# a-rtemis99/hpc_suffix_array

Hardware: AMD Instinct MI355X
Metric: suffixes sorted/sec + ms/doubling-round, 1 GiB input at 1/2/4/8 MI355X (higher is better)
Workload: dtype u32

## Files before the change

### hpc_suffix_array_amd/_native.py

```python
from __future__ import annotations

import ctypes
import os
import subprocess

PKG_DIR = os.path.dirname(os.path.abspath(__file__))
LIB_PATH = os.path.join(PKG_DIR, "lib", "libsa_hip.so")
LIB_PATH = os.environ.get("SA_LIB_PATH", LIB_PATH)
CSRC = os.path.join(PKG_DIR, "csrc")

SA_MAX_ROUNDS = 64
KERNEL_KINDS = ["init", "hist_first", "hist_keys", "scan", "scatter_first", "scatter_keys",
                "heads", "heads_scan", "rerank", "seg_count", "seg_scan", "seg_write", "alphabet", "pack",
                "sort_u", "windows", "local_sort", "pivot_keys", "pivot_count", "pivot_write"]
SCHEDULE_PACKED = 0
SCHEDULE_REFERENCE = 1
ROUND1_AUTO = 0
ROUND1_LSD = 1
ROUND1_BUCKETED = 2
SA_K_COUNT = len(KERNEL_KINDS)
FIND_AUTO = 0
FIND_LANE = 1
FIND_WAVE = 2
FIND_LANE_MAX = 3584
FIND_MODES = {"auto": FIND_AUTO, "lane": FIND_LANE, "wave": FIND_WAVE}
BWT_STATS = 258
BWT_TILE = 4096
LOCATE_SA_ORDER = 1
LOCATE_SMALL_CHUNKS = 2
LOCATE_TILE = 2048
LOCATE_ORDERS = {"text": 0, "sa": LOCATE_SA_ORDER}
MEM_INFO = 3
MEM_TOO_MANY = 1
MEM_LANE = 1
MEM_WAVE = 2
MEM_MODES = {"auto": 0, "lane": MEM_LANE, "wave": MEM_WAVE}
LPF_NONE = 0xFFFFFFFF
LZ_TILE = 4096
REP_RIGHT = 0
REP_MAXIMAL = 1
REP_SUPERMAXIMAL = 2
REP_KINDS = {"right": REP_RIGHT, "maximal": REP_MAXIMAL, "supermaximal": REP_SUPERMAXIMAL}
REP_INFO = 2
IBWT_INFO = 3
LF_TILE = 32768
IBWT_S = 64
IBWT_TILE = 16384
FM_INFO = 4
FM_ROWS = (64, 256, 4096)
FM_MAX_SAMPLE = 4096
FM_HEADER = 4096
DOC_NONE = 0xFFFFFFFF
DOC_RANK_ORDER = 1
DOC_TILE = 2048
DOC_GROUP_MAX = 256
DOC_LDS_DOCS = 8192
DOC_ORDERS = {"doc": 0, "rank": DOC_RANK_ORDER}

DROPIN_SYMBOLS = ["create_suffix_array", "destroy_suffix_array", "build_suffix_array",
                  "build_lcp_array", "find_longest_repeated_substring", "is_valid_suffix_array"]
EXT_SYMBOLS = ["sa_context_create", "sa_context_destroy", "sa_context_set_debug", "sa_workspace_bytes", "sa_build_device",
               "sa_build_ex", "sa_check_device", "sa_check", "sa_lcp_device", "sa_lcp", "sa_generate_text_device",
               "sa_alphabet_device", "sa_pack_keys_device", "sa_sort_pairs_device", "sa_scatter_u64_device",
               "sa_gather_u64_device", "sa_running_max_i64_device", "sa_inclusive_sum_i64_device",
               "sa_count_below_u64_device", "sa_select_u8_device",
               "sa_find_device", "sa_find", "sa_find_ex",
               "sa_match_device", "sa_matching_stats_device", "sa_match", "sa_matching_stats",
               "sa_bwt_device", "sa_bwt", "sa_inverse_device", "sa_inverse",
               "sa_locate_device", "sa_locate",
               "sa_mems_device", "sa_mems",
               "sa_lpf_device", "sa_lpf", "sa_lz77_device", "sa_lz77",
               "sa_repeats_device", "sa_repeats",
               "sa_lf_device", "sa_ibwt_device", "sa_lf", "sa_ibwt", "sa_ibwt_ex",
               "sa_fm_index_bytes", "sa_fm_build_device", "sa_fm_count_device", "sa_fm_locate_device",
               "sa_fm_build", "sa_fm_count", "sa_fm_locate",
               "sa_doc_array_device", "sa_doc_of_device", "sa_doc_frequency_device", "sa_doc_list_device",
               "sa_doc_array", "sa_doc_of", "sa_doc_frequency", "sa_doc_list",
               "sa_dist_begin", "sa_dist_cuts", "sa_dist_plan_cuts", "sa_dist_reserve", "sa_dist_release", "sa_dist_round1", "sa_dist_req_count", "sa_dist_req_fill",
               "sa_dist_answer", "sa_dist_refine",
               "sa_last_error", "sa_host_syncs", "sa_device_count", "sa_version", "sa_struct_size"]


class SAError(RuntimeError):
    """A libsa_hip entry point returned an error code."""


DEBUG_FLAGS = {"no_cmp": 0x1, "no_pk8": 0x2, "no_pad": 0x4, "pad_overflow": 0x8, "no_fast32": 0x10,
               "no_pivot": 0x20, "perm_always": 0x40, "no_xq": 0x80, "xq_overflow": 0x100,
               "no_tied": 0x200, "no_key1_round": 0x400, "no_eonly": 0x800,
               "eonly": 0x1000, "fast32_small": 0x2000, "no_round2_fused": 0x4000,
               "ls_one_wg": 0x8000, "no_alpha_sample": 0x10000, "alpha_sample_small": 0x20000}


def debug_bits(names) -> int:
    bits = 0
    for x in names or ():
        if x not in DEBUG_FLAGS:
            raise ValueError(f"unknown debug flag {x!r} (one of {sorted(DEBUG_FLAGS)})")
        bits |= DEBUG_FLAGS[x]
    return bits


class SaOpts(ctypes.Structure):
    _fields_ = [("profile", ctypes.c_int32), ("schedule", ctypes.c_int32), ("init_chars", ctypes.c_int32),
                ("radix", ctypes.c_int32), ("round1", ctypes.c_int32), ("debug", ctypes.c_uint32),
                ("span_extra", ctypes.c_int32), ("tune", ctypes.c_int32)]


class SaStats(ctypes.Structure):
    _fields_ = [
        ("rounds", ctypes.c_int32),
        ("n_kinds", ctypes.c_int32),
        ("total_ms", ctypes.c_double),
        ("h2d_ms", ctypes.c_double),
        ("d2h_ms", ctypes.c_double),
        ("round_ms", ctypes.c_double * SA_MAX_ROUNDS),
        ("distinct", ctypes.c_uint64 * SA_MAX_ROUNDS),
        ("passes", ctypes.c_int32 * SA_MAX_ROUNDS),
        ("sorted_n", ctypes.c_uint64 * SA_MAX_ROUNDS),
        ("prefix_len", ctypes.c_uint64 * SA_MAX_ROUNDS),
        ("schedule", ctypes.c_int32),
        ("init_chars", ctypes.c_int32),
        ("sigma", ctypes.c_int32),
        ("sparse_ranks", ctypes.c_int32),
        ("round1", ctypes.c_int32),
        ("largest_window", ctypes.c_int32),
        ("model_bytes", ctypes.c_uint64),
        ("kern_ms", ctypes.c_double * SA_K_COUNT),
        ("kern_launches", ctypes.c_uint64 * SA_K_COUNT),
        ("kern_bytes", ctypes.c_uint64 * SA_K_COUNT),
        ("round1_segments", ctypes.c_int32),
        ("round1_layout", ctypes.c_int32),
        ("round_bytes", ctypes.c_uint64 * SA_MAX_ROUNDS),
        ("round1_windows", ctypes.c_int32 * 4),
        ("alphabet", ctypes.c_int32),
    ]

    def to_dict(self) -> dict:
        r = self.rounds
        return {
            "rounds": r,
            "total_ms": self.total_ms,
            "h2d_ms": self.h2d_ms,
            "d2h_ms": self.d2h_ms,
            "round_ms": list(self.round_ms[:r]),
            "distinct": [int(x) for x in self.distinct[:r]],
            "passes": list(self.passes[:r]),
            "sorted_n": [int(x) for x in self.sorted_n[:r]],
            "prefix_len": [int(x) for x in self.prefix_len[:r]],
            "schedule": "reference" if self.schedule == SCHEDULE_REFERENCE else "packed",
            "init_chars": self.init_chars,
            "sigma": self.sigma,
            "sparse_ranks": bool(self.sparse_ranks),
            "round1": {ROUND1_LSD: "lsd", ROUND1_BUCKETED: "bucketed", 3: "pivot"}.get(self.round1, "lsd"),
            "largest_window": self.largest_window,
            "round1_segments": {0: "exact", 1: "padded", 2: "padded-overflow", 3: "striped-records",
                                4: "striped-records-overflow"}.get(self.round1_segments, "exact"),
            "round1_layout": {"compact": bool(self.round1_layout & 1), "pk8": bool(self.round1_layout & 2),
                              "xq": bool(self.round1_layout & 4), "eonly": bool(self.round1_layout & 8)},
            "reference_model_bytes": int(self.model_bytes),
            "round_bytes": [int(x) for x in self.round_bytes[:r]],
            "round1_windows": [int(x) for x in self.round1_windows],
            "alphabet": {0: "exact", 1: "sampled", 2: "refuted"}.get(self.alphabet, "exact"),
            "kernels": {k: {"ms": self.kern_ms[i], "launches": int(self.kern_launches[i]),
                            "bytes": int(self.kern_bytes[i])} for i, k in enumerate(KERNEL_KINDS)},
        }


DIST_OK = 0
DIST_UNSUPPORTED = 1
DIST_UNBALANCED = 2


class SaDistInfo(ctypes.Structure):
    _fields_ = [("status", ctypes.c_int32), ("sigma", ctypes.c_int32), ("K", ctypes.c_int32),
                ("bucket_bits", ctypes.c_int32), ("m", ctypes.c_uint64), ("sa_off", ctypes.c_uint64),
                ("m_max", ctypes.c_uint64), ("bucket_lo", ctypes.c_uint32), ("bucket_hi", ctypes.c_uint32),
                ("round1_ok", ctypes.c_int32), ("reserved", ctypes.c_int32), ("heads", ctypes.c_uint64),
                ("unsorted", ctypes.c_uint64), ("groups", ctypes.c_uint64)]


class SuffixArrayStruct(ctypes.Structure):
    _fields_ = [("str", ctypes.c_void_p), ("n", ctypes.c_int),
                ("sa", ctypes.POINTER(ctypes.c_int)), ("lcp", ctypes.POINTER(ctypes.c_int))]


_lib = None


def source_hash() -> str:
    import glob
    import hashlib
    h = hashlib.sha256()
    files = sorted(glob.glob(os.path.join(CSRC, "sa_*")) + [os.path.join(CSRC, "Makefile")]
                   + glob.glob(os.path.join(PKG_DIR, "..", "include", "*.h")))
    for p in files:
        with open(p, "rb") as f:
            h.update(os.path.basename(p).encode() + b"\0" + f.read())
    return h.hexdigest()[:16]


def build_library(force: bool = False) -> str:
    if force or not os.path.exists(LIB_PATH):
        subprocess.run(["make", "-s", "-C", CSRC], check=True)
    return LIB_PATH


def lib() -> ctypes.CDLL:
    global _lib
    if _lib is not None:
        return _lib
    if not os.path.exists(LIB_PATH):
        raise SAError(f"{LIB_PATH} is missing: run `make -C {CSRC}` (or __graft_entry__.build())")
    L = ctypes.CDLL(LIB_PATH)
    vp, u64, i32 = ctypes.c_void_p, ctypes.c_uint64, ctypes.c_int
    L.sa_context_create.argtypes = [i32, u64, ctypes.POINTER(vp)]
    L.sa_context_create.restype = i32
    L.sa_context_destroy.argtypes = [vp]
    L.sa_context_destroy.restype = None
    L.sa_context_set_debug.argtypes = [vp, ctypes.POINTER(SaOpts)]
    L.sa_context_set_debug.restype = i32
    L.sa_workspace_bytes.argtypes = [u64]
    L.sa_workspace_bytes.restype = u64
    L.sa_build_device.argtypes = [vp, vp, u64, vp, vp, ctypes.POINTER(SaOpts), ctypes.POINTER(SaStats)]
    L.sa_build_device.restype = i32
    L.sa_build_ex.argtypes = [vp, u64, vp, i32, ctypes.POINTER(SaOpts), ctypes.POINTER(SaStats)]
    L.sa_build_ex.restype = i32
    L.sa_check_device.argtypes = [vp, vp, u64, vp, vp]
    L.sa_check_device.restype = i32
    L.sa_check.argtypes = [vp, u64, vp, i32]
    L.sa_check.restype = i32
    L.sa_lcp_device.argtypes = [vp, vp, u64, vp, vp, ctypes.POINTER(u64), ctypes.POINTER(u64), vp]
    L.sa_lcp_device.restype = i32
    L.sa_lcp.argtypes = [vp, u64, vp, i32, vp, ctypes.POINTER(u64), ctypes.POINTER(u64)]
    L.sa_lcp.restype = i32
    L.sa_alphabet_device.argtypes = [vp, u64, ctypes.POINTER(ctypes.c_uint32), vp]
    L.sa_alphabet_device.restype = i32
    L.sa_pack_keys_device.argtypes = [vp, vp, u64, u64, u64, ctypes.POINTER(ctypes.c_uint16), u64,
                                      ctypes.c_uint32, vp, vp]
    L.sa_pack_keys_device.restype = i32
    L.sa_sort_pairs_device.argtypes = [vp, vp, vp, u64, ctypes.c_uint32, vp, vp, vp]
    L.sa_sort_pairs_device.restype = i32
    L.sa_scatter_u64_device.argtypes = [vp, u64, vp, ctypes.c_int64, vp, u64, vp]
    L.sa_scatter_u64_device.restype = i32
    L.sa_gather_u64_device.argtypes = [vp, vp, u64, vp, ctypes.c_int64, u64, vp]
    L.sa_gather_u64_device.restype = i32
    L.sa_running_max_i64_device.argtypes = [vp, u64, vp]
    L.sa_running_max_i64_device.restype = i32
    L.sa_inclusive_sum_i64_device.argtypes = [vp, u64, vp]
    L.sa_inclusive_sum_i64_device.restype = i32
    L.sa_count_below_u64_device.argtypes = [vp, u64, vp, u64, i32, vp, vp]
    L.sa_count_below_u64_device.restype = i32
    L.sa_select_u8_device.argtypes = [vp, u64, vp, ctypes.POINTER(u64), vp]
    L.sa_select_u8_device.restype = i32
    L.sa_find_device.argtypes = [vp, u64, vp, vp, u64, vp, u64, vp, vp, ctypes.c_uint32, vp]
    L.sa_find_device.restype = i32
    L.sa_find.argtypes = [vp, u64, vp, i32, vp, vp, u64, vp, vp]
    L.sa_find.restype = i32
    L.sa_find_ex.argtypes = [vp, u64, vp, i32, vp, vp, u64, vp, vp, ctypes.c_uint32]
    L.sa_find_ex.restype = i32
    L.sa_match_device.argtypes = [vp, u64, vp, vp, u64, vp, u64, vp, vp, vp, ctypes.c_uint32, vp]
    L.sa_match_device.restype = i32
    L.sa_matching_stats_device.argtypes = [vp, u64, vp, vp, u64, u64, vp, vp, vp, ctypes.c_uint32, vp]
    L.sa_matching_stats_device.restype = i32
    L.sa_match.argtypes = [vp, u64, vp, i32, vp, vp, u64, vp, vp, vp, ctypes.c_uint32]
    L.sa_match.restype = i32
    L.sa_matching_stats.argtypes = [vp, u64, vp, i32, vp, u64, u64, vp, vp, vp, ctypes.c_uint32]
    L.sa_matching_stats.restype = i32
    L.sa_bwt_device.argtypes = [vp, u64, vp, vp, vp, vp]
    L.sa_bwt_device.restype = i32
    L.sa_bwt.argtypes = [vp, u64, vp, i32, vp, vp]
    L.sa_bwt.restype = i32
    L.sa_inverse_device.argtypes = [vp, u64, vp, vp, vp]
    L.sa_inverse_device.restype = i32
    L.sa_inverse.argtypes = [vp, u64, i32, vp]
    L.sa_inverse.restype = i32
    L.sa_locate_device.argtypes = [vp, u64, vp, vp, vp, u64, u64, ctypes.c_uint32, vp, vp, u64, ctypes.POINTER(u64), vp]
    L.sa_locate_device.restype = i32
    L.sa_locate.argtypes = [vp, u64, i32, vp, vp, u64, u64, ctypes.c_uint32, vp, vp, u64]
    L.sa_locate.restype = i32
    L.sa_mems_device.argtypes = [vp, vp, u64, vp, vp, u64, u64, u64, u64, ctypes.c_uint32, vp, vp, vp, u64,
                                 ctypes.POINTER(u64), vp]
    L.sa_mems_device.restype = i32
    L.sa_mems.argtypes = [vp, u64, vp, i32, vp, u64, u64, u64, u64, ctypes.c_uint32, vp, vp, vp, u64,
                          ctypes.POINTER(u64)]
    L.sa_mems.restype = i32
    L.sa_lpf_device.argtypes = [vp, vp, u64, vp, vp, vp, vp, vp]
    L.sa_lpf_device.restype = i32
    L.sa_lz77_device.argtypes = [vp, u64, vp, vp, vp, vp, vp, u64, ctypes.POINTER(u64), vp]
    L.sa_lz77_device.restype = i32
    L.sa_lpf.argtypes = [vp, u64, vp, i32, vp, vp]
    L.sa_lpf.restype = i32
    L.sa_lz77.argtypes = [vp, u64, vp, i32, vp, vp, vp, u64, ctypes.POINTER(u64)]
    L.sa_lz77.restype = i32
    L.sa_repeats_device.argtypes = [vp, vp, u64, vp, vp, u64, u64, ctypes.c_uint32, vp, vp, vp, u64,
                                    ctypes.POINTER(u64), vp]
    L.sa_repeats_device.restype = i32
    L.sa_repeats.argtypes = [vp, u64, vp, i32, u64, u64, ctypes.c_uint32, vp, vp, vp, u64, ctypes.POINTER(u64)]
    L.sa_repeats.restype = i32
    L.sa_lf_device.argtypes = [vp, vp, u64, u64, vp, vp]
    L.sa_lf_device.restype = i32
    L.sa_ibwt_device.argtypes = [vp, vp, u64, u64, vp, vp, ctypes.POINTER(u64), vp]
    L.sa_ibwt_device.restype = i32
    L.sa_lf.argtypes = [vp, u64, u64, vp, i32]
    L.sa_lf.restype = i32
    L.sa_ibwt.argtypes = [vp, u64, u64, vp, vp, i32]
    L.sa_ibwt.restype = i32
    L.sa_ibwt_ex.argtypes = [vp, u64, u64, vp, vp, i32, ctypes.POINTER(u64)]
    L.sa_ibwt_ex.restype = i32
    u32 = ctypes.c_uint32
    L.sa_fm_index_bytes.argtypes = [u64, u32]
    L.sa_fm_index_bytes.restype = u64
    L.sa_fm_build_device.argtypes = [vp, vp, u64, u64, vp, u32, vp, u64, ctypes.POINTER(u64), vp]
    L.sa_fm_build_device.restype = i32
    L.sa_fm_count_device.argtypes = [vp, u64, vp, u64, vp, u64, vp, vp, vp]
# ... 82 lines not shown
```

### hpc_suffix_array_amd/csrc/sa_bucket.h

```cpp
#pragma once
#include <type_traits>

#include "sa_kernels.h"

namespace sa {

#ifndef SA_BS_BLOCK
#define SA_BS_BLOCK 512
#endif
constexpr int kBsBlock = SA_BS_BLOCK;
#ifndef SA_BS_ITEMS
#define SA_BS_ITEMS 18
#endif
constexpr int kBsItems = SA_BS_ITEMS;
constexpr int kBsCap = kBsBlock * kBsItems;
constexpr uint32_t kWinStride = 1024;
#ifndef SA_BS_WPC
#define SA_BS_WPC 2
#endif
constexpr uint32_t kBsWpc = SA_BS_WPC;
#ifndef SA_BS_GRID
#define SA_BS_GRID (1u << 22)
#endif
constexpr uint32_t kBsGrid = SA_BS_GRID;
constexpr uint64_t kBucketMinN = 1ull << 20;
constexpr uint32_t kLoBits = 8;
constexpr uint32_t kLoRadix = 1u << kLoBits;

__device__ __forceinline__ uint32_t bucket_of(uint64_t key1, uint32_t rb, uint64_t cmul, uint32_t bsh) {
    return (uint32_t)(((key1 >> rb) * cmul) >> bsh);
}

__device__ __forceinline__ uint32_t bucket_dmin(uint32_t b, uint64_t cmul, uint32_t bsh) {
    const uint64_t d0 = ((uint64_t)b << bsh) / cmul;
    return (uint32_t)((((d0 * cmul) >> bsh) == b) ? d0 : d0 + 1);
}

struct SrcBucketKeys {
    const uint64_t* __restrict__ keys;
    const uint32_t* __restrict__ vals;
    uint32_t rb, bsh;
    uint64_t cmul;
    uint32_t bofs;
    __device__ __forceinline__ uint64_t key(uint64_t e) const { return keys[e]; }
    __device__ __forceinline__ uint32_t val(uint64_t e) const { return vals[e]; }
    static constexpr bool kPk8 = false;
    __device__ __forceinline__ uint32_t digit(uint64_t k, uint32_t shift, uint32_t mask) const {
        return ((bucket_of(k, rb, cmul, bsh) - bofs) >> shift) & mask;
    }
};

struct SrcPk8 {
    const uint64_t* __restrict__ items;
    __device__ __forceinline__ uint64_t key(uint64_t e) const { return items[e]; }
    __device__ __forceinline__ uint32_t val(uint64_t) const { return 0u; }
    static constexpr bool kPk8 = true;
};

template <int NB>
__device__ __forceinline__ void lds_bytes(const uint32_t* __restrict__ w32, uint32_t off, uint32_t (&out)[NB / 4]) {
    static_assert(NB % 4 == 0, "whole words");
    const uint32_t base = off >> 2, sh = off & 3u;
    uint32_t w[NB / 4 + 1];
#pragma unroll
    for (int q = 0; q <= NB / 4; ++q) w[q] = w32[base + q];
#pragma unroll
    for (int q = 0; q < NB / 4; ++q) out[q] = __builtin_amdgcn_alignbyte(w[q + 1], w[q], sh);
}
template <int NB>
__device__ __forceinline__ uint32_t byte_at(const uint32_t (&v)[NB / 4], int j) {
    return (v[j >> 2] >> (8 * (j & 3))) & 0xFFu;
}

constexpr uint32_t kCoarseBits = 12;
constexpr uint32_t kCoarse = 1u << kCoarseBits;

constexpr uint32_t kRecStripes = 64;
constexpr uint32_t kXq = 8;
constexpr uint32_t kRecCurStride = 64;
constexpr uint64_t rec_capacity(uint64_t m) { return m + m / 8 + kRecStripes * (2ull * kTile + 1); }
template <bool POW2 = false, bool COARSE = false, int LM = 0, bool IDENT = false, bool DNA = false>
__global__ __launch_bounds__(kBlock) void k_bucket_hist(const uint8_t* __restrict__ text, uint64_t n,
                                                        const uint16_t* __restrict__ code, BucketSpec b,
                                                        uint32_t* __restrict__ ghist, uint64_t p0, uint64_t p1,
                                                        uint32_t blo, uint32_t bhi,
                                                        uint64_t* __restrict__ lkeys = nullptr,
                                                        uint32_t* __restrict__ lpos = nullptr,
                                                        uint32_t* __restrict__ wg = nullptr, uint32_t rcap = 0,
                                                        uint32_t* __restrict__ rovf = nullptr) {
    constexpr bool REC = LM == 2 || LM == 3;
    constexpr int RUN = kTile / kBlock;
    constexpr uint32_t NB = COARSE ? kCoarse : kLoRadix;
    __shared__ uint32_t s_tmp[kWaves];
    __shared__ uint16_t s_rp[REC ? kTile : 1];
    __shared__ uint32_t s_claim;
    __shared__ uint8_t s_map[256];
    __shared__ __attribute__((aligned(16))) uint32_t s_dcw[(kTile + kMaxK) / 4 + 8];
    uint8_t* s_dc = reinterpret_cast<uint8_t*>(s_dcw);
    __shared__ uint32_t s_hlo[NB];
    constexpr bool PKD = DNA && REC;
    __shared__ uint32_t s_pk[PKD ? kBlock + kMaxK / 16 + 2 : 1];
    {
        const uint32_t cv = code[threadIdx.x];
        s_map[threadIdx.x] = (uint8_t)(cv ? cv - 1u : 0u);
    }
    for (uint32_t i = threadIdx.x; i < NB; i += kBlock) s_hlo[i] = 0;
    const uint32_t sig = b.sigma, ps1 = (uint32_t)b.pow_s1;
    const uint32_t shh = b.bsh;
    const uint32_t cshift = b.bb > kCoarseBits ? b.bb - kCoarseBits : 0u;
    const uint32_t bspan = bhi - blo;
    __syncthreads();
    const uint64_t tiles = (p1 - p0 + kTile - 1) / kTile;
    uint32_t kept_lane = 0;
    uint32_t run = LM == 2 ? wg[blockIdx.x] : 0u;
    const uint32_t stripe = blockIdx.x % kRecStripes;
    const uint64_t rbase = (uint64_t)stripe * rcap;
    auto fetch = [&](uint64_t tt2, uint4& v, uint32_t& hv) {
        const uint64_t tb2 = p0 + tt2 * kTile;
        const uint64_t i2 = tb2 + (uint64_t)threadIdx.x * RUN;
        v = (i2 + RUN <= n && (((uintptr_t)(text + i2)) & 15) == 0) ? *reinterpret_cast<const uint4*>(text + i2)
                                                                     : make_uint4(0u, 0u, 0u, 0u);
        const uint64_t h2 = tb2 + kTile + threadIdx.x;
        hv = (threadIdx.x < (uint32_t)kMaxK && h2 < n) ? (uint32_t)text[h2] : 0u;
    };
    uint4 cv = make_uint4(0u, 0u, 0u, 0u);
    uint32_t chv = 0;
    if (blockIdx.x < tiles) fetch(blockIdx.x, cv, chv);
    for (uint64_t tt = blockIdx.x; tt < tiles; tt += gridDim.x) {
        const uint64_t tb = p0 + tt * kTile;
        uint4 nv;
        uint32_t nhv;
        const uint64_t tn = tt + gridDim.x;
        if constexpr (LM != 3) fetch(tn < tiles ? tn : tiles - 1, nv, nhv);
        {
            const uint64_t i = tb + (uint64_t)threadIdx.x * RUN;
            uint32_t w[4];
            if (i + RUN <= n && (((uintptr_t)(text + i)) & 15) == 0) {
                const uint4 v = cv;
                w[0] = v.x;
                w[1] = v.y;
                w[2] = v.z;
                w[3] = v.w;
                if constexpr (DNA) {
#pragma unroll
                    for (int q = 0; q < 4; ++q) w[q] = ((w[q] >> 1) ^ (w[q] >> 2)) & 0x03030303u;
                } else if constexpr (!IDENT) {
#pragma unroll
                    for (int q = 0; q < 4; ++q) {
                        uint32_t o = 0;
#pragma unroll
                        for (int y = 0; y < 4; ++y) o |= (uint32_t)s_map[(w[q] >> (8 * y)) & 0xFFu] << (8 * y);
                        w[q] = o;
                    }
                }
            } else {
#pragma unroll
// ... 114 lines not shown
                    const uint64_t a = s_pk[wi], bw = s_pk[wi + 1], cw = s_pk[wi + 2];
                    uint64_t win = ((a << 32) | bw) << off;
                    if (off) win |= cw >> (32u - off);
                    Dk = (uint32_t)(win >> (64u - 2u * b.s));
                    r = (win >> (64u - 2u * K)) & ((1ull << (2u * b.R)) - 1ull);
                } else {
                    for (uint32_t q = 0; q < b.s; ++q) Dk = POW2 ? ((Dk << lg) | s_dc[l + q]) : Dk * sig + s_dc[l + q];
                    for (uint32_t q = b.s; q < K; ++q) r = POW2 ? ((r << lg) | s_dc[l + q]) : r * sig + s_dc[l + q];
                }
                lkeys[rb + t] = ((uint64_t)Dk << b.rb) | bucket_low(b, r, n - (tb + l));
                lpos[rb + t] = (uint32_t)(tb + l);
            }
            if (LM == 2) run += tot;
        }
        cv = nv;
        chv = nhv;
        __syncthreads();
    }
    if (LM == 1) {
        uint32_t tot;
        block_exclusive_sum(kept_lane, s_tmp, &tot);
        if (threadIdx.x == 0) wg[blockIdx.x] = tot;
    }
    for (uint32_t i = threadIdx.x; i < NB; i += kBlock) {
        if (!s_hlo[i]) continue;
        if constexpr (COARSE)
            atomicAdd(reinterpret_cast<unsigned long long*>(ghist) + i, (unsigned long long)s_hlo[i]);
        else
            atomicAdd(&ghist[i], s_hlo[i]);
    }
}

__global__ __launch_bounds__(kBlock) void k_exscan_u32(const uint32_t* __restrict__ in, uint32_t* __restrict__ out,
                                                       uint32_t cnt) {
    __shared__ uint32_t s_tmp[kWaves];
    uint32_t carry = 0;
    for (uint32_t base = 0; base < cnt; base += kBlock * 16) {
        uint32_t v[16], sum = 0;
#pragma unroll
        for (int k = 0; k < 16; ++k) {
            const uint32_t i = base + threadIdx.x * 16 + k;
            v[k] = i < cnt ? in[i] : 0u;
            sum += v[k];
        }
        uint32_t tot;
        uint32_t off = block_exclusive_sum(sum, s_tmp, &tot) + carry;
#pragma unroll
        for (int k = 0; k < 16; ++k) {
            const uint32_t i = base + threadIdx.x * 16 + k;
            if (i < cnt) out[i] = off;
            off += v[k];
        }
        carry += tot;
    }
}

__global__ __launch_bounds__(kBlock) void k_window_starts_tab(const uint32_t* __restrict__ bstart, uint32_t nb,
                                                              uint64_t n, uint64_t nw, uint32_t* __restrict__ ws,
                                                              uint32_t* __restrict__ wb) {
    for (uint64_t j = (uint64_t)blockIdx.x * kBlock + threadIdx.x; j <= nw; j += (uint64_t)gridDim.x * kBlock) {
        const uint64_t x = j * kWinStride;
        if (x >= n) {
            ws[j] = (uint32_t)n;
            wb[j] = nb;
            continue;
        }
        uint32_t lo = 0, len = nb + 1;
        while (len > 0) {
            const uint32_t half = len >> 1;
            if (bstart[lo + half] < x) {
                lo += half + 1;
                len -= half + 1;
            } else {
                len = half;
            }
        }
        ws[j] = bstart[lo];
        wb[j] = lo;
    }
}

__global__ __launch_bounds__(kBlock) void k_window_starts(const uint64_t* __restrict__ keys, uint64_t n,
                                                          uint64_t nw, uint32_t rb, uint64_t cmul, uint32_t bsh,
                                                          uint32_t* __restrict__ ws) {
    for (uint64_t j = (uint64_t)blockIdx.x * kBlock + threadIdx.x; j <= nw; j += (uint64_t)gridDim.x * kBlock) {
        const uint64_t x = j * kWinStride;
        uint64_t res;
        if (x >= n) {
            res = n;
        } else if (x == 0) {
            res = 0;
        } else {
            const uint32_t bx = bucket_of(keys[x - 1], rb, cmul, bsh);
            if (bucket_of(keys[x], rb, cmul, bsh) != bx) {
                res = x;
            } else {
                uint64_t lo = x, hi, step = 1;
                for (;;) {
                    hi = lo + step;
                    if (hi >= n) {
                        hi = n;
                        break;
                    }
                    if (bucket_of(keys[hi], rb, cmul, bsh) != bx) break;
                    lo = hi;
                    step *= 2;
                }
                while (hi - lo > 1) {
                    const uint64_t mid = lo + (hi - lo) / 2;
                    if (bucket_of(keys[mid], rb, cmul, bsh) != bx) hi = mid;
                    else lo = mid;
                }
                res = hi;
            }
        }
        ws[j] = (uint32_t)res;
    }
}

__global__ __launch_bounds__(kBlock) void k_window_list(const uint32_t* __restrict__ ws, uint64_t nw,
                                                        uint32_t* __restrict__ list, uint32_t* __restrict__ words) {
    __shared__ uint32_t s_n[kWaves], s_base;
    __shared__ uint32_t s_mx[kWaves];
    const uint32_t lane = lane_id(), wave = wave_id();
    const uint64_t per = ((nw + gridDim.x - 1) / gridDim.x + kBlock - 1) / kBlock * kBlock;
    const uint64_t j0 = (uint64_t)blockIdx.x * per, j1 = j0 + per < nw ? j0 + per : nw;
    uint32_t mx = 0, cnt = 0;
    for (uint64_t j = j0 + threadIdx.x; j < j1; j += kBlock) {
        const uint32_t d = ws[j + 1] - ws[j];
        mx = d > mx ? d : mx;
        cnt += d != 0;
    }
    uint32_t tot;
    uint32_t off = block_exclusive_sum(cnt, s_n, &tot);
    if (threadIdx.x == 0) s_base = tot ? atomicAdd(&words[7], tot) : 0u;
    __syncthreads();
    off += s_base;
    for (uint64_t j = j0 + threadIdx.x; j < j1; j += kBlock)
        if (ws[j + 1] != ws[j]) list[off++] = (uint32_t)j;
#pragma unroll
    for (int o = kWave / 2; o > 0; o >>= 1) {
        const uint32_t y = __shfl_xor(mx, o, kWave);
        mx = y > mx ? y : mx;
    }
    if (lane == 0) s_mx[wave] = mx;
    __syncthreads();
    if (threadIdx.x == 0) {
        uint32_t t = 0;
        for (int x = 0; x < kWaves; ++x) t = s_mx[x] > t ? s_mx[x] : t;
        if (t) atomicMax(&words[5], t);
    }
}

template <bool POW2>
__global__ __launch_bounds__(kBlock) void k_bucket_sample(const uint8_t* __restrict__ text, uint64_t n,
                                                          const uint16_t* __restrict__ code, BucketSpec b,
                                                          uint32_t ssh, uint32_t* __restrict__ ghist) {
    __shared__ uint8_t s_map[256];
    __shared__ uint32_t s_h[kLoRadix];
    {
        const uint32_t cv = code[threadIdx.x];
        s_map[threadIdx.x] = (uint8_t)(cv ? cv - 1u : 0u);
    }
    for (uint32_t i = threadIdx.x; i < kLoRadix; i += kBlock) s_h[i] = 0;
    __syncthreads();
    const uint32_t lg = POW2 ? (uint32_t)__builtin_ctz(b.sigma) : 0u;
    const uint32_t bksh = POW2 ? lg * b.s - b.bb : 0u;
    const uint64_t ns = n >> ssh;
    for (uint64_t i = (uint64_t)blockIdx.x * kBlock + threadIdx.x; i < ns; i += (uint64_t)gridDim.x * kBlock) {
        uint32_t hsh = (uint32_t)i * 0x9E3779B1u;
        hsh ^= hsh >> 15;
        hsh *= 0x85EBCA6Bu;
        hsh ^= hsh >> 13;
        const uint64_t p = (i << ssh) + (hsh >> (32 - ssh));
        uint32_t raw[32];
#pragma unroll
        for (uint32_t q = 0; q < 32; ++q)
            raw[q] = (q < b.s && p + q < n) ? (uint32_t)text[p + q] : 256u;
        uint32_t D = 0;
#pragma unroll
        for (uint32_t q = 0; q < 32; ++q) {
            if (q < b.s) {
                const uint32_t c = raw[q] < 256u ? (uint32_t)s_map[raw[q]] : 0u;
                D = POW2 ? ((D << lg) | c) : D * b.sigma + c;
            }
        }
        const uint32_t bk = POW2 ? (D >> bksh) : (uint32_t)(((uint64_t)D * b.cmul) >> b.bsh);
        atomicAdd(&s_h[bk & (kLoRadix - 1)], 1u);
    }
    __syncthreads();
    for (uint32_t i = threadIdx.x; i < kLoRadix; i += kBlock)
        if (s_h[i]) atomicAdd(&ghist[i], s_h[i]);
}

__global__ __launch_bounds__(kLoRadix) void k_pad_starts(const uint32_t* __restrict__ samples, uint32_t ssh,
                                                         uint32_t slack_off, uint32_t limit,
                                                         uint32_t* __restrict__ pstart) {
    __shared__ uint32_t s_tmp[kLoRadix / kWave];
    const uint32_t k = samples[threadIdx.x];
    const float bound = slack_off ? (float)k : (float)k + 4.0f * sqrtf((float)k) + 16.0f;
    uint64_t cap = (uint64_t)bound << ssh;
    cap = slack_off ? cap : cap + (cap >> 5);
    cap = (cap + 63) & ~63ull;
    const uint32_t c32 = (uint32_t)cap;
    const uint32_t inc = wave_inclusive_sum(c32);
    if (lane_id() == kWave - 1) s_tmp[wave_id()] = inc;
    __syncthreads();
    uint32_t off = 0;
    for (uint32_t w = 0; w < wave_id(); ++w) off += s_tmp[w];
    __syncthreads();
    if (threadIdx.x == kLoRadix - 1) s_tmp[0] = off + inc;
    __syncthreads();
    const bool fits = s_tmp[0] <= limit;
    pstart[threadIdx.x] = fits ? off + inc - c32 : 0u;
    if (threadIdx.x == kLoRadix - 1) pstart[kLoRadix] = fits ? off + inc : 0u;
}

#ifndef SA_SUB_BITS
#define SA_SUB_BITS 11
#endif
constexpr int kSubBits = SA_SUB_BITS;
constexpr int kSubBuckets = 1 << kSubBits;
constexpr uint32_t kMaxSub = 64;
constexpr int kRetryWord = 13;

struct BucketRel {
    const uint32_t* __restrict__ wb;
    const uint32_t* __restrict__ bstart;
    const uint32_t* __restrict__ bdmin;
    uint32_t rb;
    uint32_t bits1 = 0;
};

template <int BLOCK, int ITEMS>
__device__ __forceinline__ bool load_window(const uint64_t* __restrict__ w_in, const BucketRel& br, uint32_t j,
                                            uint64_t a, uint32_t m, uint32_t ib, uint64_t (&w)[ITEMS], uint64_t& mn,
                                            uint32_t& bits, uint64_t (*s_red)[BLOCK / kWave],
                                            uint32_t (*s_bk)[32], uint32_t* __restrict__ err, bool* fixed = nullptr) {
    if (fixed) *fixed = false;
    constexpr int WAVES = BLOCK / kWave;
    constexpr int WT = kWave * ITEMS;
    const uint32_t wave = wave_id(), lane = lane_id();
    const uint64_t imask = (ib >= 64) ? ~0ull : ((1ull << ib) - 1ull);
    const uint32_t b0 = br.wb[j], nbk = br.wb[j + 1] - b0;
    uint32_t dmin0 = 0;
    if (nbk == 1) {
        dmin0 = br.bdmin[b0];
    } else if (nbk <= 32) {
        if (threadIdx.x < nbk) {
            s_bk[0][threadIdx.x] = br.bstart[b0 + threadIdx.x];
            s_bk[1][threadIdx.x] = br.bdmin[b0 + threadIdx.x];
        }
        __syncthreads();
    }
    auto dmin_of = [&](uint64_t p) -> uint32_t {
        if (nbk == 1) return dmin0;
        if (nbk <= 32) {
            uint32_t lo = 0;
            for (uint32_t step = 16; step; step >>= 1)
                if (lo + step < nbk && s_bk[0][lo + step] <= p) lo += step;
            return s_bk[1][lo];
        }
        uint32_t lo = b0, len = nbk;
        while (len > 1) {
            const uint32_t half = len >> 1;
            if (br.bstart[lo + half] <= p) {
                lo += half;
                len -= half;
            } else {
                len = half;
            }
        }
        return br.bdmin[lo];
    };
    uint64_t mx = 0;
    mn = ~0ull;
    if (nbk == 1 && br.bits1) {
        const uint32_t l0 = wave * WT + lane;
#pragma unroll
        for (int i = 0; i < ITEMS; ++i) {
            const uint32_t le = l0 + i * kWave;
            w[i] = w_in[a + (le < m ? le : m - 1)];
        }
        bits = br.bits1;
        mn = (uint64_t)dmin0 << br.rb;
        if (fixed) *fixed = true;
        __syncthreads();
        return true;
    }
    if (nbk == 1) {
        const uint32_t l0 = wave * WT + lane;
#pragma unroll
        for (int i = 0; i < ITEMS; ++i) {
            const uint32_t le = l0 + i * kWave;
            const uint64_t x = w_in[a + (le < m ? le : m - 1)];
            w[i] = x;
            mn = x < mn ? x : mn;
            mx = x > mx ? x : mx;
        }
#pragma unroll
        for (int o = kWave / 2; o > 0; o >>= 1) {
            const uint64_t y0 = __shfl_xor(mn, o, kWave), y1 = __shfl_xor(mx, o, kWave);
            mn = y0 < mn ? y0 : mn;
            mx = y1 > mx ? y1 : mx;
        }
        if (lane == 0) {
// ... 122 lines not shown
        if (mh) last_h = (int32_t)(rb0 + 63 - __clzll(mh));
        nh += __popcll(mh);
        nu += __popcll(mu);
        ng += __popcll(muh);
    }
    if (lane == 0) {
        s_red[0][wave] = (uint64_t)(uint32_t)last_h | ((uint64_t)nh << 32);
        s_red[1][wave] = (uint64_t)nu | ((uint64_t)ng << 32);
    }
    __syncthreads();
    int32_t cw = -1;
    uint32_t bu = 0, bg = 0, th = 0, tu = 0, tg = 0;
#pragma unroll
    for (int x = 0; x < WAVES; ++x) {
        const uint64_t v0 = s_red[0][x], v1 = s_red[1][x];
        if (x < (int)wave) {
            if ((int32_t)(uint32_t)v0 >= 0) cw = (int32_t)(uint32_t)v0;
            bu += (uint32_t)v1;
            bg += (uint32_t)(v1 >> 32);
        }
        th += (uint32_t)(v0 >> 32);
        tu += (uint32_t)v1;
        tg += (uint32_t)(v1 >> 32);
    }
    if (threadIdx.x == 0) {
        so.cnt_u[j] = tu;
        so.cnt_g[j] = tg;
        tot_h += th;
        tot_u += tu;
        tot_g += tg;
    }
    const uint64_t imask = (ib >= 64) ? ~0ull : ((1ull << ib) - 1ull);
    const uint64_t lt = lanemask_lt(), lem = lt | (1ull << lane);
    while (urows) {
        const uint32_t i = (uint32_t)__builtin_ctz(urows);
        urows &= urows - 1;
        const uint32_t rb0 = wave * WT + i * kWave;
        uint64_t mh, mu, muh;
        masks(rb0, mh, mu, muh);
        const uint64_t pre = s_pre[wave * ITEMS + i];
        const int32_t ph = (int32_t)(uint32_t)pre;
        const int32_t ch = ph >= 0 ? ph : cw;
        if ((mu >> lane) & 1ull) {
            const uint64_t hl = mh & lem;
            const uint32_t hpos = hl ? rb0 + 63 - (uint32_t)__clzll(hl) : (uint32_t)ch;
            const uint32_t ku = bu + (uint32_t)((pre >> 32) & 0xFFFFu) + (uint32_t)__popcll(mu & lt);
            const uint32_t kg = bg + (uint32_t)(pre >> 48) + (uint32_t)__popcll(muh & lem) - 1u;
            const uint32_t x = (uint32_t)(s_w[rb0 + lane] & imask);
            const uint32_t rv = (uint32_t)(so.rank_off + a + hpos + 1u);
            if (so.tmp_rank) so.tmp_rank[a + ku] = rv;
            else so.rank[x] = rv;
            atomicOr(&so.member[x >> 5], 1u << (x & 31));
            so.tmp_pos[a + ku] = (uint32_t)(a + rb0 + lane);
            so.tmp_idx[a + ku] = x;
            so.tmp_g[a + ku] = kg;
        }
    }
}

__device__ __forceinline__ void flush_totals(uint32_t* __restrict__ words, uint64_t th, uint64_t tu, uint64_t tg) {
    if (threadIdx.x == 0) {
        if (th) atomicAdd(&words[0], (uint32_t)th);
        if (tu) atomicAdd(&words[1], (uint32_t)tu);
        if (tg) atomicAdd(&words[2], (uint32_t)tg);
    }
}

constexpr int kWsPer = 8;
constexpr int kWsBlock = kBlock * kWsPer;

__device__ __forceinline__ void wscan_load(const uint32_t* __restrict__ c, uint64_t nw, uint64_t b0, uint32_t (&x)[kWsPer],
                                           uint32_t& sum) {
    sum = 0;
#pragma unroll
    for (int k = 0; k < kWsPer; ++k) {
        const uint64_t i = b0 + threadIdx.x * kWsPer + k;
        x[k] = i <= nw ? c[i] : 0u;
        sum += x[k];
    }
}

__global__ __launch_bounds__(kBlock) void k_wscan_reduce(const uint32_t* __restrict__ cu, const uint32_t* __restrict__ cg,
                                                         uint64_t nw, uint32_t* __restrict__ part) {
    __shared__ uint32_t s_tmp[kWaves];
    const uint64_t b0 = (uint64_t)blockIdx.x * kWsBlock;
    uint32_t x[kWsPer], su, sg, tu, tg;
    wscan_load(cu, nw, b0, x, su);
    wscan_load(cg, nw, b0, x, sg);
    block_exclusive_sum(su, s_tmp, &tu);
    block_exclusive_sum(sg, s_tmp, &tg);
    if (threadIdx.x == 0) {
        part[2 * blockIdx.x] = tu;
        part[2 * blockIdx.x + 1] = tg;
    }
}

__global__ __launch_bounds__(kBlock) void k_wscan_top(uint32_t* __restrict__ part, uint32_t blocks) {
    __shared__ uint32_t s_tmp[kWaves];
    uint32_t carry_u = 0, carry_g = 0;
    for (uint32_t b0 = 0; b0 < blocks; b0 += kBlock) {
        const uint32_t b = b0 + threadIdx.x;
        const uint32_t u = b < blocks ? part[2 * b] : 0u, g = b < blocks ? part[2 * b + 1] : 0u;
        uint32_t tu, tg;
        const uint32_t eu = block_exclusive_sum(u, s_tmp, &tu) + carry_u;
        const uint32_t eg = block_exclusive_sum(g, s_tmp, &tg) + carry_g;
        if (b < blocks) {
            part[2 * b] = eu;
            part[2 * b + 1] = eg;
        }
        carry_u += tu;
        carry_g += tg;
    }
}

__global__ __launch_bounds__(kBlock) void k_wscan_apply(uint32_t* __restrict__ cu, uint32_t* __restrict__ cg, uint64_t nw,
                                                        const uint32_t* __restrict__ part) {
    __shared__ uint32_t s_tmp[kWaves];
    const uint64_t b0 = (uint64_t)blockIdx.x * kWsBlock;
    for (int a = 0; a < 2; ++a) {
        uint32_t* c = a ? cg : cu;
        uint32_t x[kWsPer], sum;
        wscan_load(c, nw, b0, x, sum);
        uint32_t off = block_exclusive_sum(sum, s_tmp, nullptr) + part[2 * blockIdx.x + a];
#pragma unroll
        for (int k = 0; k < kWsPer; ++k) {
            const uint64_t i = b0 + threadIdx.x * kWsPer + k;
            if (i <= nw) c[i] = off;
            off += x[k];
        }
    }
}

__global__ __launch_bounds__(kBlock) void k_u_gather(const uint32_t* __restrict__ list,
                                                     const uint32_t* __restrict__ words,
                                                     const uint32_t* __restrict__ ws, const uint32_t* __restrict__ ou,
                                                     const uint32_t* __restrict__ og, SegOut so,
                                                     uint32_t* __restrict__ u_pos, uint32_t* __restrict__ u_idx,
                                                     uint32_t* __restrict__ u_g, RankMap rm = RankMap{}) {
    const uint32_t nlist = words[7];
    const uint32_t lane = lane_id();
    for (uint64_t q = (uint64_t)blockIdx.x * kWaves + wave_id(); q < nlist; q += (uint64_t)gridDim.x * kWaves) {
        const uint32_t j = list[q];
        const uint32_t a = ws[j], o = ou[j], c = ou[j + 1] - o, g0 = og[j];
        for (uint32_t k = lane; k < c; k += kWave) {
            const uint32_t x = so.tmp_idx[a + k];
            u_pos[o + k] = so.tmp_pos[a + k];
            u_idx[o + k] = x;
            u_g[o + k] = so.tmp_g[a + k] + g0;
            if (so.tmp_rank) so.rank[rm.slot(x)] = so.tmp_rank[a + k];
        }
    }
}

constexpr int kR2Batch = 16;

__global__ __launch_bounds__(kBlock) void k_round2_windows(const uint32_t* __restrict__ list, const uint32_t* words,
                                                           const uint32_t* __restrict__ ws,
                                                           const uint32_t* __restrict__ cnt_u,
                                                           const uint32_t* __restrict__ tmp_pos,
                                                           const uint32_t* __restrict__ tmp_idx,
                                                           const uint32_t* __restrict__ tmp_g,
                                                           const uint8_t* __restrict__ text, uint64_t n,
                                                           const uint16_t* __restrict__ code, BucketSpec bs, uint64_t m,
                                                           uint32_t* __restrict__ sa, uint32_t* flag) {
    const uint32_t nlist = words[7];
    const uint32_t lane = lane_id();
    const uint32_t K = bs.s + bs.R;
    const CodeMap map{code};
    const uint64_t lt = lanemask_lt(), lem = lt | (1ull << lane);
    for (uint64_t q0 = ((uint64_t)blockIdx.x * kWaves + wave_id()) * kR2Batch; q0 < nlist;
         q0 += (uint64_t)gridDim.x * kWaves * kR2Batch) {
        if (__builtin_amdgcn_readfirstlane((int)__atomic_load_n(flag, __ATOMIC_RELAXED))) return;
        uint32_t a_l = 0, c_l = 0;
        if (lane < (uint32_t)kR2Batch && q0 + lane < nlist) {
            const uint32_t j = list[q0 + lane];
            c_l = cnt_u[j];
            a_l = ws[j];
        }
        if (__ballot(c_l > (uint32_t)kWave)) {
            if (lane == 0) atomicOr(flag, 1u);
            return;
        }
        const uint32_t e_l = wave_inclusive_sum(c_l);
        uint64_t todo = __ballot(c_l != 0);
        uint32_t base = 0;
        while (todo) {
            const uint64_t fit = todo & __ballot(e_l - base <= (uint32_t)kWave);
            todo &= ~fit;
            uint32_t a = 0, off = 0, nbase = base;
            bool act = false;
            for (uint64_t f = fit; f; f &= f - 1) {
                const int w = __builtin_ctzll(f);
                const uint32_t ew = (uint32_t)__shfl((int)e_l, w, kWave), cw = (uint32_t)__shfl((int)c_l, w, kWave);
                const uint32_t aw = (uint32_t)__shfl((int)a_l, w, kWave);
                const uint32_t s0 = ew - cw - base;
                if (lane >= s0 && lane < s0 + cw) {
                    a = aw;
                    off = lane - s0;
                    act = true;
                }
                nbase = ew;
            }
            base = nbase;
            bool bad = act && (uint64_t)a + off >= m;
            act = act && !bad;
            uint32_t pos = 0, x = 0, g = 0;
            if (act) {
                pos = tmp_pos[a + off];
                x = tmp_idx[a + off];
                g = tmp_g[a + off];
            }
            bad = bad || (act && x >= n);
            uint64_t key = 0;
            if (act && !bad && (uint64_t)x + K < n) {
                uint32_t D;
                key = key1_words<true>(text, n, map, bs, (uint64_t)x + K, &D) + 1u;
            }
            const uint64_t ma = __ballot(act);
            const uint32_t gp = (uint32_t)__shfl_up((int)g, 1, kWave);
            const bool head = act && (lane == 0 || off == 0 || g != gp || !((ma >> (lane - 1)) & 1ull));
            const uint64_t mh = __ballot(head);
            const uint64_t hl = mh & lem, ab = (mh | ~ma) & ~lem;
            const uint32_t start = hl ? 63u - (uint32_t)__clzll(hl) : lane;
            const uint32_t end = ab ? (uint32_t)__builtin_ctzll(ab) : (uint32_t)kWave;
            const uint32_t len = end - start;
            bad = bad || (act && len > (uint32_t)kUsLimit);
            uint32_t rank = 0;
#pragma unroll
            for (int t = 0; t < kUsLimit; ++t) {
                const uint32_t src = (start + t) & (kWave - 1);
                const uint64_t kk = __shfl(key, (int)src, kWave);
                if (act && (uint32_t)t < len && src != lane) {
                    rank += kk < key ? 1u : 0u;
                    bad = bad || kk == key;
                }
            }
            const uint64_t p = (uint64_t)(uint32_t)__shfl((int)pos, (int)start, kWave) + rank;
            bad = bad || (act && p >= m);
            if (__ballot(bad)) {
                if (lane == 0) atomicOr(flag, 1u);
                return;
            }
            if (act) sa[p] = x;
        }
    }
}

constexpr int kPcPer = 16;
constexpr int kPcBlock = kBlock * kPcPer;

__device__ __forceinline__ void popc_load(const uint32_t* __restrict__ bits, uint64_t nw, uint64_t b0,
                                          uint32_t (&c)[kPcPer]) {
    if (b0 + kPcPer <= nw) {
#pragma unroll
        for (int q = 0; q < kPcPer / 4; ++q) {
            const uint4 v = reinterpret_cast<const uint4*>(bits + b0)[q];
            c[4 * q] = (uint32_t)__popc(v.x);
            c[4 * q + 1] = (uint32_t)__popc(v.y);
            c[4 * q + 2] = (uint32_t)__popc(v.z);
            c[4 * q + 3] = (uint32_t)__popc(v.w);
        }
    } else {
#pragma unroll
        for (int k = 0; k < kPcPer; ++k) c[k] = b0 + k < nw ? (uint32_t)__popc(bits[b0 + k]) : 0u;
    }
}

__global__ __launch_bounds__(kBlock) void k_popc_reduce(const uint32_t* __restrict__ bits, uint64_t nw,
                                                        uint32_t* __restrict__ part) {
    __shared__ uint32_t s_tmp[kWaves];
    uint32_t c[kPcPer], sum = 0;
    popc_load(bits, nw, (uint64_t)blockIdx.x * kPcBlock + (uint64_t)threadIdx.x * kPcPer, c);
#pragma unroll
    for (int k = 0; k < kPcPer; ++k) sum += c[k];
    uint32_t tot;
    block_exclusive_sum(sum, s_tmp, &tot);
    if (threadIdx.x == 0) part[blockIdx.x] = tot;
}

constexpr int kPcTop = 1024;
__global__ __launch_bounds__(kPcTop) void k_popc_top(uint32_t* __restrict__ part, uint32_t blocks) {
    __shared__ uint32_t s_tmp[kPcTop / kWave];
    const uint32_t per = (blocks + kPcTop - 1) / kPcTop;
    const uint32_t b0 = threadIdx.x * per, b1 = b0 + per < blocks ? b0 + per : blocks;
    uint32_t sum = 0;
#pragma unroll 8
    for (uint32_t b = b0; b < b1; ++b) sum += part[b];
    const uint32_t inc = wave_inclusive_sum(sum);
    if (lane_id() == kWave - 1) s_tmp[wave_id()] = inc;
    __syncthreads();
    uint32_t run = inc - sum;
#pragma unroll
    for (int w = 0; w < kPcTop / kWave; ++w) run += w < (int)wave_id() ? s_tmp[w] : 0u;
#pragma unroll 8
    for (uint32_t b = b0; b < b1; ++b) {
        const uint32_t v = part[b];
        part[b] = run;
        run += v;
    }
}

__global__ __launch_bounds__(kBlock) void k_popc_apply(const uint32_t* __restrict__ bits, uint64_t nw,
                                                       const uint32_t* __restrict__ part,
                                                       uint32_t* __restrict__ prefix) {
    __shared__ uint32_t s_tmp[kWaves];
    const uint64_t b0 = (uint64_t)blockIdx.x * kPcBlock + (uint64_t)threadIdx.x * kPcPer;
    uint32_t c[kPcPer], sum = 0;
// ... 175 lines not shown
                cm = y > cm ? y : cm;
            }
            if (lane == kWave - 1) s_tmp[wave] = inc;
            if (lane == 0) s_red[0][wave] = cm;
            __syncthreads();
            uint32_t off = 0;
#pragma unroll
            for (int x = 0; x < WAVES; ++x) {
                off += (x < (int)wave) ? s_tmp[x] : 0u;
                big = (uint32_t)s_red[0][x] > big ? (uint32_t)s_red[0][x] : big;
            }
            uint32_t b = off + inc - sum;
#pragma unroll
            for (int x = 0; x < WPT; ++x) {
                const uint32_t b0 = b, b1 = b + c[2 * x];
                s_cnt[WPT * dg + x] = b0 | (b1 << 16);
                b = b1 + c[2 * x + 1];
            }
        }
        __syncthreads();
        probe.mark(2);
        if (big > kMaxSub) {
            if (threadIdx.x == 0) {
                if (fixed && retry) retry[atomicAdd(&words[kRetryWord], 1u)] = j;
                else skew[atomicAdd(&words[10], 1u)] = j;
            }
            __syncthreads();
            continue;
        }
#pragma unroll
        for (int i = 0; i < ITEMS; ++i) {
            if (wave * WT + i * kWave + lane < m) {
                const uint32_t sb = (uint32_t)(w[i] >> dsh) & (kSubBuckets - 1);
                const uint32_t old = atomicAdd(&s_cnt[sb >> 1], 1u << (16 * (sb & 1)));
                s_w[(old >> (16 * (sb & 1))) & 0xFFFFu] = w[i];
            }
        }
        __syncthreads();
        probe.mark(3);
        uint32_t nu = 0, ng = 0;
        uint32_t umask = 0;
        const uint32_t sb0 = 2 * WPT * dg;
        const uint32_t low_bits = bits > (uint32_t)kSubBits ? bits - kSubBits : bits;
        const uint32_t low_mask = low_bits >= 32 ? ~0u : ((1u << low_bits) - 1u);
        static_assert(2 * WPT == 4, "four sub-buckets per thread");
        uint32_t order = 0;
        {
            uint32_t o[4];
#pragma unroll
            for (int k = 0; k < 4; ++k) {
                const uint32_t sb = sb0 + k;
                o[k] = ((end_of(sb) - (sb ? end_of(sb - 1) : 0u)) << 2) | (uint32_t)k;
            }
            sort_net32<4>(o);
#pragma unroll
            for (int k = 0; k < 4; ++k) order |= (o[3 - k] & 3u) << (2 * k);
        }
#pragma unroll 1
        for (uint32_t i = 0; i < 4; ++i) {
            const uint32_t sb = sb0 + ((order >> (2 * i)) & 3u);
            const uint32_t lo = sb ? end_of(sb - 1) : 0u, hi = end_of(sb), cnt = hi - lo;
            const bool wide = __ballot(cnt > 8u) != 0ull;
            const bool wide4 = __ballot(cnt > 4u) != 0ull, wide12 = __ballot(cnt > 12u) != 0ull;
            if (cnt == 0) continue;
            const uint32_t nu0 = nu;
            if (!wide4 && low_bits <= 28) sort_sub<4>(s_w, lo, cnt, ib, low_mask, nu, ng);
            else if (!wide && low_bits <= 28) sort_sub<8>(s_w, lo, cnt, ib, low_mask, nu, ng);
            else if (!wide12 && low_bits <= 28) sort_sub<12>(s_w, lo, cnt, ib, low_mask, nu, ng);
            else
            if (cnt <= (uint32_t)kNet && low_bits <= 28) sort_sub<kNet>(s_w, lo, cnt, ib, low_mask, nu, ng);
            else sort_sub_lds(s_w, lo, hi, ib, nu, ng);
            if (nu != nu0) umask |= 1u << (sb - sb0);
        }
        probe.mark(4);
        uint32_t bu, bg, th_w, tu_w, tg_w;
        {
            const uint32_t iug = wave_inclusive_sum(nu | (ng << 16));
            uint32_t* const s_ug = s_tmp2;
            if (lane == kWave - 1) s_ug[wave] = iug;
            __syncthreads();
            uint32_t oug = 0, tug = 0;
#pragma unroll
            for (int x = 0; x < WAVES; ++x) {
                const uint32_t xug = s_ug[x];
                oug += (x < (int)wave) ? xug : 0u;
                tug += xug;
            }
            tu_w = tug & 0xFFFFu;
            tg_w = tug >> 16;
            th_w = m - tu_w + tg_w;
            bu = (oug & 0xFFFFu) + (iug & 0xFFFFu) - nu;
            bg = (oug >> 16) + (iug >> 16) - ng;
        }
        if (so.rank) {
            if (threadIdx.x == 0) {
                so.cnt_u[j] = tu_w;
                so.cnt_g[j] = tg_w;
                th += th_w;
                tu += tu_w;
                tg += tg_w;
            }
            if (umask) {
                const uint64_t imask = (ib >= 64) ? ~0ull : ((1ull << ib) - 1ull);
                uint32_t ku = bu, kg = bg;
                for (uint32_t um = umask; um; um &= um - 1u) {
                    const uint32_t sb = sb0 + (uint32_t)__builtin_ctz(um);
                    const uint32_t lo = sb ? end_of(sb - 1) : 0u, hi = end_of(sb);
                    uint32_t head = lo;
                    uint64_t pr = ~0ull;
                    for (uint32_t k = lo; k < hi; ++k) {
                        const uint64_t x = s_w[k], r = x >> ib;
                        const uint64_t nx = k + 1 < hi ? (s_w[k + 1] >> ib) : ~0ull;
                        const bool eqp = k > lo && pr == r, eqn = k + 1 < hi && nx == r;
                        if (!eqp) head = k;
                        if (!eqp && eqn) ++kg;
                        if (eqp || eqn) {
                            const uint32_t xi = (uint32_t)(x & imask);
                            const uint32_t rv = (uint32_t)(so.rank_off + a + head + 1u);
                            if (so.tmp_rank) so.tmp_rank[a + ku] = rv;
                            else so.rank[xi] = rv;
                            atomicOr(&so.member[xi >> 5], 1u << (xi & 31));
                            so.tmp_pos[a + ku] = (uint32_t)(a + k);
                            so.tmp_idx[a + ku] = xi;
                            so.tmp_g[a + ku] = kg - 1u;
                            ++ku;
                        }
                        pr = r;
                    }
                }
            }
        }
        probe.mark(5);
        store_window<BLOCK, ITEMS>(s_w, a, m, ib, mn, keys_out, sa_out, so.ksh);
        __syncthreads();
        probe.mark(6);
    }
    probe.flush(words);
    flush_totals(words, th, tu, tg);
}

template <int ITEMS>
__device__ __forceinline__ uint32_t slot0() {
    uint32_t t = threadIdx.x;
    asm volatile("" : "+v"(t));
    return (t / kWave) * (kWave * ITEMS) + (t & (kWave - 1));
}

constexpr uint32_t kSlotBits = kBsCap > (1 << 14) ? 15 : 14;
constexpr uint32_t kSlotMask = (1u << kSlotBits) - 1u;
constexpr uint32_t kLowMax = 32 - kSlotBits;
static_assert(kBsCap <= (1 << kSlotBits), "load slots in kSlotBits");
constexpr int kHdrWord = 14;
constexpr int kTicketWord = 15;

__global__ __launch_bounds__(kBlock) void k_window_split(const uint32_t* __restrict__ list,
                                                         const uint32_t* __restrict__ ws, BucketRel br,
                                                         uint32_t* __restrict__ words, uint4* __restrict__ hdr,
                                                         uint32_t* __restrict__ retry, uint32_t fast,
                                                         const uint32_t* __restrict__ pc = nullptr,
                                                         const uint32_t* __restrict__ pn = nullptr, uint32_t nb = 0,
                                                         uint32_t* __restrict__ hx = nullptr, uint32_t crows = 0) {
    const uint32_t nlist = words[7];
    const uint32_t lane = lane_id();
    for (uint64_t q0 = (uint64_t)blockIdx.x * kBlock; q0 < nlist; q0 += (uint64_t)gridDim.x * kBlock) {
        const uint64_t q = q0 + threadIdx.x;
        uint32_t j = 0, b0 = 0;
        bool one = false;
        const bool ok = q < nlist;
        if (ok) {
            j = list[q];
            b0 = br.wb[j];
            one = fast && br.wb[j + 1] - b0 == 1u;
            if (one && hx) {
                uint32_t nr = 0;
                for (uint32_t k = 0; k < kXq; ++k) {
                    const uint32_t c = pn[(uint64_t)k * nb + b0];
                    if (!crows && c && c < kWave) one = false;
                    nr += (c + kWave - 1) / kWave;
                }
                if (crows && nr > crows) one = false;
            }
        }
        const uint64_t m1 = __ballot(ok && one), m2 = __ballot(ok && !one);
        uint32_t base1 = 0, base2 = 0;
        if (lane == 0) {
            if (m1) base1 = atomicAdd(&words[kHdrWord], (uint32_t)__popcll(m1));
            if (m2) base2 = atomicAdd(&words[kRetryWord], (uint32_t)__popcll(m2));
        }
        base1 = (uint32_t)__shfl((int)base1, 0, kWave);
        base2 = (uint32_t)__shfl((int)base2, 0, kWave);
        if (ok && one) {
            const uint32_t a = ws[j];
            const uint32_t qi = base1 + (uint32_t)__popcll(m1 & lanemask_lt());
            hdr[qi] = make_uint4(j, a, ws[j + 1] - a, br.bdmin[b0]);
            if (hx) {
                uint32_t P = 0;
                for (uint32_t k = 0; k < kXq; ++k) {
                    const uint32_t c = pc[(uint64_t)k * nb + b0];
                    hx[(uint64_t)qi * 16 + k] = c - P;
                    if (k) hx[(uint64_t)qi * 16 + kXq - 1 + k] = P;
                    P += pn[(uint64_t)k * nb + b0];
                }
            }
        } else if (ok) {
            retry[base2 + (uint32_t)__popcll(m2 & lanemask_lt())] = j;
        }
    }
}

__global__ __launch_bounds__(kBlock) void k_window_gather(const uint32_t* __restrict__ list,
                                                          const uint32_t* __restrict__ words,
                                                          const uint32_t* __restrict__ ws,
                                                          const uint32_t* __restrict__ wb,
                                                          const uint32_t* __restrict__ pc,
                                                          const uint32_t* __restrict__ pn, uint32_t nb,
                                                          const uint64_t* __restrict__ in,
                                                          uint64_t* __restrict__ out) {
    const uint32_t nlist = words[kRetryWord];
    for (uint32_t qi = blockIdx.x; qi < nlist; qi += gridDim.x) {
        const uint32_t j = list[qi];
        uint64_t dst = ws[j];
        for (uint32_t b = wb[j]; b < wb[j + 1]; ++b) {
            for (uint32_t k = 0; k < kXq; ++k) {
                const uint32_t c = pn[(uint64_t)k * nb + b];
                const uint64_t src = pc[(uint64_t)k * nb + b];
                for (uint32_t t = threadIdx.x; t < c; t += kBlock) out[dst + t] = in[src + t];
                dst += c;
            }
        }
    }
}

template <int N, int LSV = 0>
__device__ __forceinline__ bool sort_sub_words(uint32_t* __restrict__ s_k, const uint32_t* __restrict__ s_x,
                                               uint32_t lo, uint32_t cnt, uint32_t& nu, uint32_t& ng) {
    uint32_t v[N];
#pragma unroll
    for (int t = 0; t < N; ++t) {
        if constexpr (LSV & 1) {
            const uint32_t x = s_k[lo + t];
            v[t] = (uint32_t)t < cnt ? x : ~0u;
        } else {
            v[t] = (uint32_t)t < cnt ? s_k[lo + t] : ~0u;
        }
    }
    sort_net32<N>(v);
    uint32_t eqm = 0;
#pragma unroll
    for (int t = 0; t + 1 < N; ++t) eqm |= ((v[t] ^ v[t + 1]) <= kSlotMask ? 1u : 0u) << t;
    eqm &= (1u << (cnt - 1)) - 1u;
    if constexpr (LSV & 2) {
        if (eqm == 0u) {
            uint32_t xi[N];
#pragma unroll
            for (int t = 0; t < N; ++t) xi[t] = s_x[min(v[t] & kSlotMask, (uint32_t)kBsCap - 1u)];
#pragma unroll
            for (int t = 0; t < N; ++t)
                if ((uint32_t)t < cnt) s_k[lo + t] = xi[t];
            return false;
        }
    }
#pragma unroll
    for (int t = 0; t < N; ++t)
        if ((uint32_t)t < cnt) s_k[lo + t] = v[t];
    nu += (uint32_t)__popc(eqm | (eqm << 1));
    ng += (uint32_t)__popc(eqm & ~(eqm << 1));
    return eqm != 0u;
}

__device__ __forceinline__ void sort_sub_words_lds(uint32_t* __restrict__ s_k, uint32_t lo, uint32_t hi, uint32_t& nu,
                                                   uint32_t& ng) {
    for (uint32_t k = lo + 1; k < hi; ++k) {
        const uint32_t x = s_k[k];
        uint32_t y = k;
        while (y > lo && s_k[y - 1] > x) {
            s_k[y] = s_k[y - 1];
            --y;
        }
        s_k[y] = x;
    }
    uint32_t pr = ~0u, cur = s_k[lo] >> kSlotBits;
    for (uint32_t k = lo; k < hi; ++k) {
        const uint32_t nx = k + 1 < hi ? (s_k[k + 1] >> kSlotBits) : ~0u;
        const bool eqp = k > lo && pr == cur, eqn = k + 1 < hi && nx == cur;
        nu += (eqp || eqn) ? 1u : 0u;
        ng += (!eqp && eqn) ? 1u : 0u;
        pr = cur;
        cur = nx;
    }
}

template <int ITEMS, int I0 = 0, int I1 = ITEMS>
__device__ __forceinline__ void load_items(const uint64_t* __restrict__ w_in, uint64_t a, uint32_t m,
                                           uint64_t (&x)[ITEMS]) {
    const uint32_t l0 = slot0<ITEMS>();
#pragma unroll
    for (int i = I0; i < I1; ++i) {
        const uint32_t le = l0 + i * kWave;
        x[i] = w_in[a + (le < m ? le : m - 1)];
    }
}

struct XqWin {
    const uint32_t* __restrict__ hx = nullptr;
    const uint32_t* __restrict__ rows = nullptr;
};

__device__ __forceinline__ uint32_t xq_offset(const uint32_t* __restrict__ hx, uint32_t le) {
    uint32_t off = hx[0];
#pragma unroll
    for (int k = 1; k < (int)kXq; ++k) off = hx[kXq - 1 + k] <= le ? hx[k] : off;
    return off;
}

template <int ITEMS, int I0 = 0, int I1 = ITEMS>
__device__ __forceinline__ void load_items_cr(const uint64_t* __restrict__ w_in, const uint32_t (&rv)[3],
                                              uint64_t (&x)[ITEMS]) {
    const uint32_t lane = lane_id();
#pragma unroll
    for (int i = I0; i < I1; ++i) {
        const uint32_t base = (uint32_t)__builtin_amdgcn_readlane((int)rv[0], i);
        x[i] = (w_in + base)[lane];
    }
}

template <int ITEMS, int ROWS>
__device__ __forceinline__ void load_rows_xq(const uint32_t* __restrict__ rows, uint32_t (&rv)[3]) {
    const uint32_t lane = lane_id();
    const uint32_t w = (uint32_t)__builtin_amdgcn_readfirstlane((int)(threadIdx.x / kWave));
    const uint32_t r = w * ITEMS + (lane < (uint32_t)ITEMS ? lane : 0u);
#pragma unroll
    for (int t = 0; t < 3; ++t) rv[t] = rows[t * ROWS + r];
}

template <int ITEMS, int I0 = 0, int I1 = ITEMS>
__device__ __forceinline__ void load_items_xq(const uint64_t* __restrict__ w_in, const uint32_t (&rv)[3], uint32_t m,
                                              uint64_t (&x)[ITEMS]) {
    const uint32_t l0 = slot0<ITEMS>();
    const uint32_t lane = lane_id();
    const uint32_t last = m - 1;
#pragma unroll
    for (int i = I0; i < I1; ++i) {
        const uint32_t le = l0 + i * kWave;
        const uint32_t lc = le < m ? le : last;
        const uint32_t da = (uint32_t)__builtin_amdgcn_readlane((int)rv[0], i);
        const uint32_t db = (uint32_t)__builtin_amdgcn_readlane((int)rv[1], i);
        const uint32_t sp = (uint32_t)__builtin_amdgcn_readlane((int)rv[2], i);
        x[i] = w_in[(uint32_t)((lane < sp ? da : db) + lc)];
    }
}

template <bool CR>
__global__ __launch_bounds__(kBlock) void k_window_rows(const uint32_t* __restrict__ words, const uint4* __restrict__ hdr,
                                                        const uint32_t* __restrict__ hx, uint32_t nrows,
                                                        uint32_t* __restrict__ rows) {
    const uint32_t nh = words[kHdrWord];
    const uint32_t lane = lane_id();
    for (uint64_t q = (uint64_t)blockIdx.x * kWaves + wave_id(); q < nh; q += (uint64_t)gridDim.x * kWaves) {
        const uint32_t m = hdr[q].z;
        uint32_t hv[16];
#pragma unroll
        for (int k = 0; k < 16; ++k) hv[k] = hx[q * 16 + k];
        if constexpr (CR) {
            uint32_t st[kXq], cn[kXq], nfull = 0;
#pragma unroll
            for (int k = 0; k < (int)kXq; ++k) {
                const uint32_t p0 = k ? hv[kXq - 1 + k] : 0u, p1 = k + 1 < (int)kXq ? hv[kXq + k] : m;
                st[k] = hv[k] + p0;
                cn[k] = p1 - p0;
                nfull += cn[k] / kWave;
            }
            for (uint32_t r = lane; r < nrows; r += kWave) {
                uint32_t base = st[0], cnt = 0, rf = 0, rp = nfull;
#pragma unroll
                for (int k = 0; k < (int)kXq; ++k) {
                    const uint32_t nf = cn[k] / kWave, rem = cn[k] % kWave;
                    if (r >= rf && r < rf + nf) {
                        base = st[k] + kWave * (r - rf);
                        cnt = kWave;
                    }
                    if (rem && r == rp) {
                        base = st[k] + kWave * nf;
                        cnt = rem;
                    }
                    rf += nf;
                    rp += rem ? 1u : 0u;
                }
                uint32_t* const e = rows + q * 3 * nrows + r;
                e[0] = base;
                e[nrows] = cnt;
            }
            continue;
        }
        for (uint32_t r = lane; r < nrows; r += kWave) {
            const uint32_t lo = std::min(r * kWave, m - 1), hi = std::min(r * kWave + (kWave - 1), m - 1);
            uint32_t split = kWave;
#pragma unroll
            for (int k = kXq - 1; k >= 1; --k) {
                const uint32_t pk = hv[kXq - 1 + k];
                if (pk > lo && pk <= hi) split = pk - r * kWave;
            }
            uint32_t* const e = rows + q * 3 * nrows + r;
            e[0] = xq_offset(hv, lo);
            e[nrows] = xq_offset(hv, hi);
            e[2 * nrows] = split;
        }
    }
}

#ifndef SA_LS_WFULL
#define SA_LS_WFULL 1
#endif
#ifndef SA_LS_CLAIMS
#define SA_LS_CLAIMS 1
#endif
#ifndef SA_LS_HRANK
#define SA_LS_HRANK 1
#endif
#ifndef SA_LS_HRANK_PF
#define SA_LS_HRANK_PF 3
#endif
#if SA_LS_HRANK_PF == 0
#define SA_LS_PF_TABLE {0, 0, 18, 18, 18}
#elif SA_LS_HRANK_PF == 1
#define SA_LS_PF_TABLE {18, 18, 18, 18, 18}
#elif SA_LS_HRANK_PF == 3
#define SA_LS_PF_TABLE {6, 6, 12, 18, 18}
#elif SA_LS_HRANK_PF == 5
#define SA_LS_PF_TABLE {0, 0, 6, 12, 18}
#elif SA_LS_HRANK_PF == 6
#define SA_LS_PF_TABLE {3, 6, 9, 15, 18}
#endif
constexpr int kLsPfHr[5] = SA_LS_PF_TABLE;
constexpr int kLsPfOld[5] = {0, 0, 18, 18, 18};
template <int P>
using pf_point = std::integral_constant<int, P>;
template <int BLOCK, int ITEMS, class Probe = NoProbe, bool XQ = false, int LSV = 0, bool CR = false>
__global__ __launch_bounds__(BLOCK, 4) void k_bucket_sort(const uint64_t* __restrict__ keys_in,
                                                       const uint4* __restrict__ hdr, uint32_t rb, uint32_t bits,
                                                       uint32_t ib, uint32_t* __restrict__ words,
                                                       uint64_t* __restrict__ keys_out, uint32_t* __restrict__ sa_out,
                                                       uint32_t* __restrict__ retry, SegOut so, XqWin xw = XqWin{}) {
    constexpr int WAVES = BLOCK / kWave;
    constexpr int CAP = BLOCK * ITEMS;
    static_assert(CAP <= (1 << kSlotBits), "load slots");
    __shared__ uint32_t s_lds[kSubBuckets / 2 + CAP + ((LSV & 1) ? kNet : 0) + CAP];
    uint32_t* const s_cnt = s_lds;
    uint32_t* const s_k = s_lds + kSubBuckets / 2;
    uint32_t* const s_x = s_k + CAP + ((LSV & 1) ? kNet : 0);
    __shared__ uint32_t s_tmp[WAVES];
    __shared__ uint32_t s_cm[WAVES];
    __shared__ uint32_t s_ug[WAVES];
    __shared__ uint32_t s_q[2];
    __shared__ unsigned long long s_tot[3];
    constexpr int WPT = kSubBuckets / 2 / BLOCK;
    static_assert(WPT * 2 == 4 && WPT * 2 * BLOCK == kSubBuckets, "four sub-buckets per thread");
    constexpr int ROWS = WAVES * ITEMS;

    const uint32_t wave = wave_id(), lane = lane_id();
    const uint32_t dg = threadIdx.x;
    const uint32_t nwin = words[kHdrWord];
    const uint32_t low_bits = bits - kSubBits;
    const uint32_t dsh = ib + low_bits;
    const uint32_t lmask = (1u << low_bits) - 1u;
    const uint64_t imask = (1ull << ib) - 1ull;
    auto end_of = [&](uint32_t sb) -> uint32_t { return ((s_cnt[sb >> 1] >> (16 * (sb & 1))) & 0xFFFFu) >> 2; };
    static_assert(4 * CAP < (1 << 16), "byte counts in 16-bit halves");
    auto cnt_word = [&](uint32_t y) -> uint32_t* {
        return reinterpret_cast<uint32_t*>(reinterpret_cast<char*>(s_cnt) + ((y << 1) & 0xFFCu));
    };
    auto half_inc = [](uint32_t y) -> uint32_t {
        uint32_t r;
        asm("v_lshlrev_b32_e64 %0, %1, 4" : "=v"(r) : "v"(y << 4));
        return r;
    };
    constexpr bool HR = SA_LS_HRANK != 0;
    typedef uint16_t __attribute__((may_alias)) half_t;
    Probe probe;
    if (threadIdx.x == 0) {
        s_q[0] = atomicAdd(&words[kTicketWord], 1u);
        if constexpr (HR) s_q[1] = atomicAdd(&words[kTicketWord], 1u);
        s_tot[0] = s_tot[1] = s_tot[2] = 0;
    }
    if constexpr (HR)
        for (int i = threadIdx.x; i < kSubBuckets / 2; i += BLOCK) s_cnt[i] = 0;
    __syncthreads();
    uint32_t q = (uint32_t)__builtin_amdgcn_readfirstlane((int)s_q[0]);
    if (q >= nwin) return;
    uint4 h = hdr[q];
    uint64_t w[ITEMS];
    uint32_t rv[3] = {0u, 0u, 0u};
    if constexpr (XQ) {
        load_rows_xq<ITEMS, ROWS>(xw.rows + (uint64_t)q * 3 * ROWS, rv);
        if constexpr (CR) load_items_cr<ITEMS>(keys_in, rv, w);
        else load_items_xq<ITEMS>(keys_in, rv, h.z, w);
    } else {
        load_items<ITEMS>(keys_in, h.y, h.z, w);
    }
    uint32_t qn = 0;
    bool more = false;
    uint4 hn = make_uint4(0u, 0u, 1u, 0u);
    uint32_t rwn[3] = {0u, 0u, 0u};
    auto next_window = [&](uint32_t ticket, uint32_t cur, uint32_t& qx, bool& mx, uint4& hx,
                           uint32_t (&rx)[3]) __attribute__((always_inline)) {
        qx = (uint32_t)__builtin_amdgcn_readfirstlane((int)ticket);
        mx = qx < nwin;
        hx = make_uint4(0u, 0u, 1u, 0u);
        if (mx) hx = hdr[qx];
        if constexpr (XQ) load_rows_xq<ITEMS, ROWS>(xw.rows + (uint64_t)(mx ? qx : cur) * 3 * ROWS, rx);
    };
    if constexpr (HR) next_window(s_q[1], q, qn, more, hn, rwn);
    uint32_t par = 0;
    for (;;) {
        probe.mark(-1);
        const uint32_t j = h.x, m = h.z;
        const uint64_t a = h.y;
        const uint64_t mn = (uint64_t)h.w << rb;
        if constexpr (!HR) {
            if (threadIdx.x == 0) s_q[par ^ 1u] = atomicAdd(&words[kTicketWord], 1u);
            for (int i = threadIdx.x; i < kSubBuckets / 2; i += BLOCK) s_cnt[i] = 0;
            __syncthreads();
            next_window(s_q[par ^ 1u], q, qn, more, hn, rwn);
        }
        probe.mark(0);
        const uint32_t l0 = slot0<ITEMS>();
        const bool wfull = SA_LS_WFULL && (wave + 1) * (uint32_t)(kWave * ITEMS) <= m;
        bool sfull = wfull;
        if constexpr (XQ && CR)
            sfull = SA_LS_WFULL && __ballot(lane < (uint32_t)ITEMS && rv[1] == kWave) == (1ull << ITEMS) - 1ull;
        auto slot_ok = [&](int i) -> bool {
            if constexpr (XQ && CR) return lane < (uint32_t)__builtin_amdgcn_readlane((int)rv[1], i);
            else return l0 + i * kWave < m;
        };
        static_assert(ITEMS == 18, "SA_LS_PF_TABLE");
        auto prefetch_at = [&](auto pc, auto rest) __attribute__((always_inline)) {
            constexpr int P = decltype(pc)::value;
            constexpr int A = P ? (HR ? kLsPfHr[P - 1] : kLsPfOld[P - 1]) : 0;
            constexpr int B = decltype(rest)::value ? ITEMS : (HR ? kLsPfHr[P] : kLsPfOld[P]);
            if constexpr (A < B) {
                __builtin_amdgcn_sched_barrier(0);
                if constexpr (XQ && CR) load_items_cr<ITEMS, A, B>(keys_in, rwn, w);
                else if constexpr (XQ) load_items_xq<ITEMS, A, B>(keys_in, rwn, hn.z, w);
                else load_items<ITEMS, A, B>(keys_in, hn.y, hn.z, w);
            }
        };
        constexpr std::false_type part{};
        constexpr std::true_type rest{};
        constexpr int RKW = (ITEMS + 3) / 4;
        uint32_t kk[HR ? ITEMS : 1], rk[HR ? RKW : 1];
        uint32_t tk = 0;
        static_assert(4 * kMaxSub <= 256, "byte ranks in 8 bits");
        if constexpr (HR) {
#pragma unroll
            for (int r = 0; r < RKW; ++r) rk[r] = 0;
            auto count1 = [&](int i, uint32_t le) {
                const uint32_t k = (uint32_t)(w[i] >> ib);
                const uint32_t y = k >> low_bits;
                const uint32_t old = atomicAdd(cnt_word(y), half_inc(y));
                s_x[le] = (uint32_t)(w[i] & imask);
                kk[i] = k;
                rk[i / 4] |= __builtin_amdgcn_ubfe(old, y << 4, 8u) << (8 * (i % 4));
            };
            if (sfull) {
#pragma unroll
                for (int i = 0; i < ITEMS; ++i) count1(i, l0 + i * kWave);
            } else {
#pragma unroll
                for (int i = 0; i < ITEMS; ++i) {
                    kk[i] = 0;
                    if (slot_ok(i)) count1(i, l0 + i * kWave);
                }
            }
            __builtin_amdgcn_sched_barrier(0);
            if (threadIdx.x == 0) tk = atomicAdd(&words[kTicketWord], 1u);
            prefetch_at(pf_point<0>{}, part);
        } else if (sfull) {
#pragma unroll
            for (int i = 0; i < ITEMS; ++i) {
                const uint32_t y = (uint32_t)(w[i] >> dsh);
                atomicAdd(cnt_word(y), half_inc(y));
            }
        } else {
#pragma unroll
            for (int i = 0; i < ITEMS; ++i) {
                if (slot_ok(i)) {
                    const uint32_t y = (uint32_t)(w[i] >> dsh);
                    atomicAdd(cnt_word(y), half_inc(y));
                }
            }
        }
        __syncthreads();
        probe.mark(1);
        uint32_t big = 0;
        uint32_t bw[2 * WPT + 1];
        {
            uint32_t c[2 * WPT], sum = 0, cm = 0;
#pragma unroll
            for (int x = 0; x < WPT; ++x) {
                const uint32_t pw = s_cnt[WPT * dg + x];
                c[2 * x] = pw & 0xFFFFu;
                c[2 * x + 1] = pw >> 16;
            }
#pragma unroll
            for (int x = 0; x < 2 * WPT; ++x) {
                sum += c[x];
                cm = c[x] > cm ? c[x] : cm;
            }
            const uint32_t inc = wave_inclusive_sum(sum);
#pragma unroll
            for (int o = kWave / 2; o > 0; o >>= 1) {
                const uint32_t y = __shfl_xor(cm, o, kWave);
                cm = y > cm ? y : cm;
            }
            if (lane == kWave - 1) s_tmp[wave] = inc;
            if (lane == 0) s_cm[wave] = cm;
            __syncthreads();
            uint32_t off = 0;
#pragma unroll
            for (int x = 0; x < WAVES; ++x) {
                off += (x < (int)wave) ? s_tmp[x] : 0u;
                big = s_cm[x] > big ? s_cm[x] : big;
            }
            uint32_t b = off + inc - sum;
#pragma unroll
            for (int x = 0; x < WPT; ++x) {
                const uint32_t b0 = b, b1 = b + c[2 * x];
                s_cnt[WPT * dg + x] = b0 | (b1 << 16);
                b = b1 + c[2 * x + 1];
                bw[2 * x] = b0 >> 2;
                bw[2 * x + 1] = b1 >> 2;
            }
            bw[2 * WPT] = b >> 2;
            if constexpr (HR)
                if (threadIdx.x == 0) s_q[0] = tk;
        }
        prefetch_at(pf_point<1>{}, part);
        __syncthreads();
        probe.mark(2);
        uint32_t qnn = 0;
        bool moren = false;
        uint4 hnn = make_uint4(0u, 0u, 1u, 0u);
        uint32_t rwnn[3] = {0u, 0u, 0u};
        if ((big >> 2) > kMaxSub) {
            if (threadIdx.x == 0) retry[atomicAdd(&words[kRetryWord], 1u)] = j;
            if constexpr (HR) {
#pragma unroll
                for (int x = 0; x < WPT; ++x) s_cnt[WPT * dg + x] = 0;
            }
            prefetch_at(pf_point<2>{}, rest);
            __syncthreads();
            if constexpr (HR) next_window(s_q[0], q, qnn, moren, hnn, rwnn);
        } else {
            auto place1 = [&](int i, uint32_t le) {
                const uint32_t k = kk[HR ? i : 0];
                const uint32_t st = reinterpret_cast<const half_t*>(s_cnt)[(k >> low_bits) & (uint32_t)(kSubBuckets - 1)];
                const uint32_t at = st + __builtin_amdgcn_ubfe(rk[HR ? i / 4 : 0], 8u * (i % 4), 8u);
                *reinterpret_cast<uint32_t*>(reinterpret_cast<char*>(s_k) + at) = ((k & lmask) << kSlotBits) | le;
            };
            auto scatter1 = [&](int i, uint32_t le) {
                const uint32_t y = (uint32_t)(w[i] >> dsh);
                const uint32_t old = atomicAdd(cnt_word(y), half_inc(y));
                const uint32_t at = __builtin_amdgcn_ubfe(old, y << 4, 16u);
                *reinterpret_cast<uint32_t*>(reinterpret_cast<char*>(s_k) + at) =
                    (((uint32_t)(w[i] >> ib) & lmask) << kSlotBits) | le;
                s_x[le] = (uint32_t)(w[i] & imask);
            };
            (void)place1;
            (void)scatter1;
            if constexpr (HR) {
                if (sfull) {
#pragma unroll
                    for (int i = 0; i < ITEMS; ++i) place1(i, l0 + i * kWave);
                } else {
#pragma unroll
                    for (int i = 0; i < ITEMS; ++i)
                        if (slot_ok(i)) place1(i, l0 + i * kWave);
                }
            } else if (sfull) {
#pragma unroll
                for (int g = 0; g < ITEMS; g += SA_LS_CLAIMS) {
                    uint32_t y[SA_LS_CLAIMS], old[SA_LS_CLAIMS];
#pragma unroll
                    for (int t = 0; t < SA_LS_CLAIMS; ++t) {
                        y[t] = (uint32_t)(w[g + t] >> dsh);
                        old[t] = atomicAdd(cnt_word(y[t]), half_inc(y[t]));
                    }
#pragma unroll
                    for (int t = 0; t < SA_LS_CLAIMS; ++t) {
                        const int i = g + t;
                        const uint32_t le = l0 + i * kWave;
                        const uint32_t at = __builtin_amdgcn_ubfe(old[t], y[t] << 4, 16u);
                        *reinterpret_cast<uint32_t*>(reinterpret_cast<char*>(s_k) + at) =
                            (((uint32_t)(w[i] >> ib) & lmask) << kSlotBits) | le;
                        s_x[le] = (uint32_t)(w[i] & imask);
// ... 19 lines not shown
                    lo = bw[3], hi = bw[4];
                    if (k == 0) lo = bw[0], hi = bw[1];
                    if (k == 1) lo = bw[1], hi = bw[2];
                    if (k == 2) lo = bw[2], hi = bw[3];
                } else {
                    const uint32_t sb = sb0 + k;
                    lo = sb ? end_of(sb - 1) : 0u;
                    hi = end_of(sb);
                }
            };
            uint32_t order = 0;
            {
                uint32_t o[4];
#pragma unroll
                for (int k = 0; k < 4; ++k) {
                    uint32_t lo, hi;
                    sub_range((uint32_t)k, lo, hi);
                    o[k] = ((hi - lo) << 2) | (uint32_t)k;
                }
                sort_net32<4>(o);
#pragma unroll
                for (int k = 0; k < 4; ++k) order |= (o[3 - k] & 3u) << (2 * k);
            }
#pragma unroll 1
            for (uint32_t i = 0; i < 4; ++i) {
                const uint32_t sb = sb0 + ((order >> (2 * i)) & 3u);
                uint32_t lo, hi;
                sub_range(sb - sb0, lo, hi);
                const uint32_t cnt = hi - lo;
                const bool wide4 = __ballot(cnt > 4u) != 0ull, wide8 = __ballot(cnt > 8u) != 0ull,
                           wide12 = __ballot(cnt > 12u) != 0ull;
                if (cnt == 0) continue;
                const uint32_t nu0 = nu;
                constexpr int LW = LSV & 1;
                bool grp;
                if ((LSV & 2) && !so.samples) {
                    if (!wide4) grp = sort_sub_words<4, LSV>(s_k, s_x, lo, cnt, nu, ng);
                    else if (!wide8) grp = sort_sub_words<8, LSV>(s_k, s_x, lo, cnt, nu, ng);
                    else if (!wide12) grp = sort_sub_words<12, LSV>(s_k, s_x, lo, cnt, nu, ng);
                    else if (cnt <= (uint32_t)kNet) grp = sort_sub_words<kNet, LSV>(s_k, s_x, lo, cnt, nu, ng);
                    else {
                        sort_sub_words_lds(s_k, lo, hi, nu, ng);
                        grp = true;
                    }
                } else {
                    if (!wide4) sort_sub_words<4, LW>(s_k, s_x, lo, cnt, nu, ng);
                    else if (!wide8) sort_sub_words<8, LW>(s_k, s_x, lo, cnt, nu, ng);
                    else if (!wide12) sort_sub_words<12, LW>(s_k, s_x, lo, cnt, nu, ng);
                    else if (cnt <= (uint32_t)kNet) sort_sub_words<kNet, LW>(s_k, s_x, lo, cnt, nu, ng);
                    else sort_sub_words_lds(s_k, lo, hi, nu, ng);
                    grp = nu != nu0;
                }
                if (grp) umask |= 1u << (sb - sb0);
                if (so.samples)
                    for_each_sample(a, lo, hi, so.ksh, [&](uint32_t q) {
                        keys_out[(a + q) >> so.ksh] = mn + (((uint64_t)sb << low_bits) | (s_k[q] >> kSlotBits));
                    });
            }
            prefetch_at(pf_point<3>{}, part);
            probe.mark(4);
            uint32_t bu, bg, tu_w, tg_w;
            {
                const uint32_t iug = wave_inclusive_sum(nu | (ng << 16));
                if (lane == kWave - 1) s_ug[wave] = iug;
                __syncthreads();
                uint32_t oug = 0, tug = 0;
#pragma unroll
                for (int x = 0; x < WAVES; ++x) {
                    const uint32_t xug = s_ug[x];
                    oug += (x < (int)wave) ? xug : 0u;
                    tug += xug;
                }
                tu_w = tug & 0xFFFFu;
                tg_w = tug >> 16;
                bu = (oug & 0xFFFFu) + (iug & 0xFFFFu) - nu;
                bg = (oug >> 16) + (iug >> 16) - ng;
            }
            if constexpr (HR) {
#pragma unroll
                for (int x = 0; x < WPT; ++x) s_cnt[WPT * dg + x] = 0;
            }
            const bool idx_back = (LSV & 2) && !so.samples;
            if (so.rank && threadIdx.x == 0) {
                so.cnt_u[j] = tu_w;
                so.cnt_g[j] = tg_w;
                s_tot[0] += m - tu_w + tg_w;
                s_tot[1] += tu_w;
                s_tot[2] += tg_w;
            }
            if (umask && (so.rank || idx_back)) {
                uint32_t ku = bu, kg = bg;
                for (uint32_t um = umask; um; um &= um - 1u) {
                    uint32_t lo, hi;
                    sub_range((uint32_t)__builtin_ctz(um), lo, hi);
                    uint32_t head = lo, pr = ~0u;
                    for (uint32_t k = lo; k < hi; ++k) {
                        const uint32_t v = s_k[k], r = v >> kSlotBits;
                        const uint32_t nx = k + 1 < hi ? (s_k[k + 1] >> kSlotBits) : ~0u;
                        const bool eqp = k > lo && pr == r, eqn = k + 1 < hi && nx == r;
                        const uint32_t xi = s_x[v & kSlotMask];
                        if (idx_back) s_k[k] = xi;
                        if (!eqp) head = k;
                        if (!eqp && eqn) ++kg;
                        if (so.rank && (eqp || eqn)) {
                            const uint32_t rv = (uint32_t)(so.rank_off + a + head + 1u);
                            if (so.tmp_rank) so.tmp_rank[a + ku] = rv;
                            else so.rank[xi] = rv;
                            atomicOr(&so.member[xi >> 5], 1u << (xi & 31));
                            so.tmp_pos[a + ku] = (uint32_t)(a + k);
                            so.tmp_idx[a + ku] = xi;
                            so.tmp_g[a + ku] = kg - 1u;
                            ++ku;
                        }
                        pr = r;
                    }
                }
            }
            prefetch_at(pf_point<4>{}, part);
            probe.mark(5);
            if (idx_back) {
                __syncthreads();
                if (wfull) {
#pragma unroll 2
                    for (int i = 0; i < ITEMS; ++i) {
                        const uint32_t le = l0 + i * kWave;
                        sa_out[a + le] = s_k[le];
                    }
                } else {
#pragma unroll 2
                    for (int i = 0; i < ITEMS; ++i) {
                        const uint32_t le = l0 + i * kWave;
                        if (le < m) sa_out[a + le] = s_k[le];
                    }
                }
            } else if (wfull) {
#pragma unroll 2
                for (int i = 0; i < ITEMS; ++i) {
                    const uint32_t le = l0 + i * kWave;
                    sa_out[a + le] = s_x[s_k[le] & kSlotMask];
                }
            } else {
#pragma unroll 2
                for (int i = 0; i < ITEMS; ++i) {
                    const uint32_t le = l0 + i * kWave;
                    if (le < m) sa_out[a + le] = s_x[s_k[le] & kSlotMask];
                }
            }
            __syncthreads();
            probe.mark(6);
        }
        if (!more) break;
        q = qn;
        h = hn;
        if constexpr (XQ && CR) {
            rv[0] = rwn[0];
            rv[1] = rwn[1];
        }
        if constexpr (HR) {
            qn = qnn;
            more = moren;
            hn = hnn;
#pragma unroll
            for (int t = 0; t < 3; ++t) rwn[t] = rwnn[t];
        }
        par ^= 1u;
    }
    probe.flush(words);
    __syncthreads();
    flush_totals(words, s_tot[0], s_tot[1], s_tot[2]);
}

template <int BLOCK, int ITEMS>
__global__ __launch_bounds__(BLOCK) void k_bucket_sort_lsd(const uint64_t* __restrict__ keys_in, BucketRel br,
                                                           const uint32_t* __restrict__ ws,
                                                           const uint32_t* __restrict__ skew,
                                                           uint32_t* __restrict__ words, uint32_t ib,
                                                           uint64_t* __restrict__ keys_out,
                                                           uint32_t* __restrict__ sa_out, SegOut so) {
    constexpr int WAVES = BLOCK / kWave;
    constexpr int CAP = BLOCK * ITEMS;
    constexpr int WT = kWave * ITEMS;
    static_assert(BLOCK >= kRadix, "one thread per digit");
    static_assert(CAP <= 65535, "16-bit LDS offsets");
    __shared__ uint64_t s_w[CAP];
    __shared__ uint16_t s_wcnt[WAVES][kRadix];
    __shared__ uint16_t s_start[kRadix];
    __shared__ uint32_t s_tmp[kWaves];
    __shared__ uint64_t s_red[2][WAVES];
    __shared__ uint32_t s_bk[2][32];

    const uint32_t wave = wave_id(), lane = lane_id();
    const uint32_t dg = threadIdx.x;
    uint32_t* err = words + 6;
    const uint32_t nskew = words[10];
    static_assert(WAVES * ITEMS * 8 <= WAVES * kRadix * 2, "per-row segment values fit in s_wcnt");
    uint64_t th = 0, tu = 0, tg = 0;
    for (uint32_t q = blockIdx.x; q < nskew; q += gridDim.x) {
        const uint32_t j = skew[q];
        const uint64_t a = ws[j];
        const uint32_t m = (uint32_t)(ws[j + 1] - a);
        uint64_t w[ITEMS];
        uint64_t mn;
        uint32_t bits;
        if (!load_window<BLOCK, ITEMS>(keys_in, br, j, a, m, ib, w, mn, bits, s_red, s_bk, err)) {
            __syncthreads();
            continue;
        }
        const uint32_t passes = (bits + 7) / 8;
        for (uint32_t p = 0; p < passes; ++p) {
            const uint32_t sh = ib + 8 * p;
            for (int i = threadIdx.x; i < WAVES * kRadix; i += BLOCK) (&s_wcnt[0][0])[i] = 0;
            __syncthreads();
            uint32_t r[ITEMS];
            uint16_t* wc = s_wcnt[wave];
#pragma unroll
            for (int i = 0; i < ITEMS; ++i) {
                const uint32_t le = wave * WT + i * kWave + lane;
                const bool ok = le < m;
                const uint32_t d = ok ? (uint32_t)(w[i] >> sh) & 0xFFu : (uint32_t)kRadix;
                uint64_t peers = __ballot(ok);
#pragma unroll
                for (uint32_t bt = 0; bt < 8; ++bt) {
                    const bool bit = (d >> bt) & 1u;
                    const uint64_t bal = __ballot(bit);
                    peers &= bit ? bal : ~bal;
                }
                uint32_t cnt = 0;
                if (ok) cnt = wc[d];
                const uint32_t below = (uint32_t)__popcll(peers & lanemask_lt());
                r[i] = cnt + below;
                if (ok && below == 0) wc[d] = (uint16_t)(cnt + (uint32_t)__popcll(peers));
            }
            __syncthreads();
            uint32_t tot = 0;
            if (dg < (uint32_t)kRadix) {
#pragma unroll
                for (int x = 0; x < WAVES; ++x) {
                    const uint32_t y = s_wcnt[x][dg];
                    s_wcnt[x][dg] = (uint16_t)tot;
                    tot += y;
                }
            }
            {
                const uint32_t x = (dg < (uint32_t)kRadix) ? tot : 0u;
                const uint32_t inc = wave_inclusive_sum(x);
                if (lane == kWave - 1 && wave < (uint32_t)kWaves) s_tmp[wave] = inc;
                __syncthreads();
                uint32_t off = 0;
#pragma unroll
                for (int x2 = 0; x2 < kWaves; ++x2) off += (x2 < (int)wave) ? s_tmp[x2] : 0u;
                if (dg < (uint32_t)kRadix) s_start[dg] = (uint16_t)(off + inc - x);
            }
            __syncthreads();
#pragma unroll
            for (int i = 0; i < ITEMS; ++i) {
                if (wave * WT + i * kWave + lane < m) {
                    const uint32_t d = (uint32_t)(w[i] >> sh) & 0xFFu;
                    s_w[s_start[d] + s_wcnt[wave][d] + r[i]] = w[i];
                }
            }
            __syncthreads();
#pragma unroll
            for (int i = 0; i < ITEMS; ++i) {
                const uint32_t le = wave * WT + i * kWave + lane;
                if (le < m) w[i] = s_w[le];
            }
            __syncthreads();
        }
        if (passes == 0) {
#pragma unroll
            for (int i = 0; i < ITEMS; ++i) {
                const uint32_t le = wave * WT + i * kWave + lane;
                if (le < m) s_w[le] = w[i];
            }
            __syncthreads();
        }
        if (so.rank)
            window_segments<BLOCK, ITEMS>(s_w, reinterpret_cast<uint64_t*>(&s_wcnt[0][0]), s_red, a, m, ib, j, so, th,
                                          tu, tg);
        store_window<BLOCK, ITEMS>(s_w, a, m, ib, mn, keys_out, sa_out, so.ksh);
        __syncthreads();
    }
    flush_totals(words, th, tu, tg);
}

}
```

### hpc_suffix_array_amd/csrc/sa_build.hip

```cpp
#include <hip/hip_runtime.h>

#include <algorithm>
#include <atomic>
#include <chrono>
#include <cstdarg>
#include <cstdio>
#include <cstdlib>
#include <cstring>
#include <mutex>
#include <string>
#include <thread>
#include <vector>

#include "../../include/sa_hip.h"

#ifndef SA_ALPHA_GRID
#define SA_ALPHA_GRID 2048
#endif

#include "sa_bucket.h"
#include "sa_check.h"
#include "sa_kernels.h"
#include "sa_lcp.h"
#include "sa_limits.h"
#include "sa_onesweep.h"
#include "sa_permute.h"
#include "sa_pivot.h"
#include "sa_split.h"
#include "sa_lsd.h"

namespace sa {

static thread_local std::string g_err;

static int set_err(int code, const char* fmt, ...) {
    char buf[512];
    va_list ap;
    va_start(ap, fmt);
    vsnprintf(buf, sizeof buf, fmt, ap);
    va_end(ap);
    g_err = buf;
    return code;
}

#define SA_HIP(call)                                                                         \
    do {                                                                                     \
        hipError_t e_ = (call);                                                              \
        if (e_ != hipSuccess)                                                                \
            return set_err(SA_E_HIP, "%s failed: %s (%s:%d)", #call, hipGetErrorString(e_),  \
                           __FILE__, __LINE__);                                              \
    } while (0)

static std::atomic<uint64_t> g_host_syncs{0};
static hipError_t host_sync(hipStream_t s) {
    g_host_syncs.fetch_add(1, std::memory_order_relaxed);
    return hipStreamSynchronize(s);
}
static hipError_t host_sync_event(hipEvent_t e) {
    g_host_syncs.fetch_add(1, std::memory_order_relaxed);
    return hipEventSynchronize(e);
}
static hipError_t host_memcpy(void* dst, const void* src, size_t bytes, hipMemcpyKind kind) {
    g_host_syncs.fetch_add(1, std::memory_order_relaxed);
    return hipMemcpy(dst, src, bytes, kind);
}

#define SA_TRY(...)                      \
    do {                                 \
        const int rc_ = (__VA_ARGS__);   \
        if (rc_) return rc_;             \
    } while (0)

static bool trace_on() {
    static const bool on = std::getenv("SA_TRACE") != nullptr;
    return on;
}
#define SA_TRACE(...)                                   \
    do {                                                \
        if (trace_on()) {                               \
            std::fprintf(stderr, "[sa] " __VA_ARGS__);  \
            std::fputc('\n', stderr);                   \
        }                                               \
    } while (0)

#ifndef SA_MAX_CHUNKS
#define SA_MAX_CHUNKS 4096
#endif
constexpr uint32_t kMaxChunks = SA_MAX_CHUNKS;
static_assert(kMaxChunks >= 1 && kMaxChunks <= (1u << 20), "chunk scratch sized for at most 2^20 chunks");
constexpr uint64_t kSparseDiv = 8;
constexpr int kEvPool = 256;
constexpr int kRoundEv = SA_MAX_ROUNDS + 1;
constexpr int kSyncEv = kEvPool + kRoundEv;

static uint64_t align_up(uint64_t x, uint64_t a) { return (x + a - 1) / a * a; }

static uint32_t bit_width(uint64_t x) {
    uint32_t w = 0;
    while (x) { ++w; x >>= 1; }
    return w;
}

static Chunking plan_chunks(uint64_t n) {
    Chunking ch;
    ch.n = n;
    const uint64_t tiles = (n + kTile - 1) / kTile;
    uint64_t tpc = (tiles + kMaxChunks - 1) / kMaxChunks;
    if (tpc == 0) tpc = 1;
    ch.tiles_per_chunk = (uint32_t)tpc;
    ch.chunks = (uint32_t)std::max<uint64_t>(1, (tiles + tpc - 1) / tpc);
    return ch;
}

}

namespace sa { struct DistState; }

struct sa_context {
    int device = 0;
    uint64_t cap = 0;
    uint64_t cap_pad = 0;
    uint64_t ucap = 0;
    uint32_t* rank = nullptr;
    uint64_t* keys[2] = {nullptr, nullptr};
    uint32_t* vals_alt = nullptr;
    uint32_t* vals_u = nullptr;
    uint32_t* u_pos[2] = {nullptr, nullptr};
    uint32_t* u_idx[2] = {nullptr, nullptr};
    uint32_t* u_g[2] = {nullptr, nullptr};
    uint32_t* u_gs[2] = {nullptr, nullptr};
    uint64_t gscap = 0;
    uint64_t* keys_u = nullptr;
    uint64_t kucap = 0;
    uint32_t* segx = nullptr;
    uint64_t segx_words = 0;
    uint32_t* os = nullptr;
    uint32_t* lsd = nullptr;
    uint32_t* lsdx = nullptr;
    uint32_t* segw = nullptr;
    uint64_t* states = nullptr;
    uint32_t epoch = 0;
    uint64_t radix_passes = 0;
    int radix = 0;
    int cus = 256;
    uint32_t* member = nullptr;
    uint32_t* hist = nullptr;
    uint32_t* totals = nullptr;
    uint32_t* counts = nullptr;
    uint32_t* words = nullptr;
    uint32_t* alpha = nullptr;
    uint16_t* code = nullptr;
    uint32_t* host_words = nullptr;
    hipEvent_t ev[sa::kEvPool + sa::kRoundEv + 1];
    int ev_ready = 0;
    sa::DistState* dist = nullptr;
    uint32_t dbg = 0;
    int32_t span_extra = 0;
    int32_t tune = 0;
    bool dna = false;
    bool alpha_prove = false;
    bool alpha_refuted = false;
    bool samples_pending = false;
};

namespace sa {

static uint64_t pad_capacity(uint64_t n) { return n + n / 8 + (1ull << 22); }

static uint64_t pad_elems(uint64_t n) {
    const uint64_t m = align_up(std::max<uint64_t>(n, 1), 64);
    return (n >= (1ull << 26) && n <= (1ull << 31)) ? align_up(pad_capacity(n), 64) : m;
}

constexpr uint64_t kMaxRadix = 1024;
static uint64_t tile_states_bytes(uint64_t n) { return ((n + kTile - 1) / kTile + 1) * kMaxRadix * 8; }

static uint64_t ws_bytes(uint64_t n) {
    const uint64_t m = align_up(std::max<uint64_t>(n, 1), 64);
    const uint64_t ku_slack = n >= (1ull << 26) ? n / 16 + 8ull * 1024 * kXqSlack + 64 : 0;
    const uint64_t gs = 2 * (n / 2 + 64) * 4;
    const uint64_t segx = (xq_words(1024) + 1032 + 2ull * kXq * (1ull << 19)) * 4;
    return m * 4 + 2 * m * 8 + m * 4 + (pad_elems(n) - m) * 12 + 7 * m * 4 + (m + ku_slack) * 8 + m / 8 + gs +
           segx + tile_states_bytes(n) + (uint64_t)kRadix * kMaxChunks * 4 + 8192;
}

static void free_ctx_buffers(sa_context* c) {
    hipFree(c->rank);
    hipFree(c->keys[0]);
    hipFree(c->keys[1]);
    hipFree(c->vals_alt);
    hipFree(c->states);
    c->rank = nullptr;
    c->keys[0] = c->keys[1] = nullptr;
    c->vals_alt = nullptr;
    c->states = nullptr;
    c->cap = 0;
    c->cap_pad = 0;
}

static void free_u_buffers(sa_context* c) {
    hipFree(c->vals_u);
    hipFree(c->keys_u);
    hipFree(c->member);
    c->vals_u = nullptr;
    c->keys_u = nullptr;
    c->member = nullptr;
    for (int i = 0; i < 2; ++i) {
        hipFree(c->u_pos[i]);
        hipFree(c->u_idx[i]);
        hipFree(c->u_g[i]);
        hipFree(c->u_gs[i]);
        c->u_pos[i] = c->u_idx[i] = c->u_g[i] = c->u_gs[i] = nullptr;
    }
    c->gscap = 0;
    c->ucap = 0;
    c->kucap = 0;
}

static void set_debug(sa_context* c, const sa_opts* o) {
    c->dbg = o ? o->debug : 0u;
    c->span_extra = o ? o->span_extra : 0;
    c->tune = o ? o->tune : 0;
}

static int ensure_capacity(sa_context* c, uint64_t n) {
    if (n <= c->cap && c->rank) return SA_OK;
    SA_HIP(hipSetDevice(c->device));
    free_ctx_buffers(c);
    const uint64_t m = align_up(std::max<uint64_t>(n, 1), 64);
    const uint64_t mp = pad_elems(n);
    if (hipMalloc(&c->rank, m * 4) != hipSuccess || hipMalloc(&c->keys[0], mp * 8) != hipSuccess ||
        hipMalloc(&c->keys[1], m * 8) != hipSuccess || hipMalloc(&c->vals_alt, mp * 4) != hipSuccess ||
        hipMalloc(&c->states, tile_states_bytes(n)) != hipSuccess ||
        hipMemset(c->states, 0, tile_states_bytes(n)) != hipSuccess) {
        free_ctx_buffers(c);
        (void)hipGetLastError();
        return set_err(SA_E_NOMEM, "device allocation of %.2f GiB workspace failed",
                       (double)ws_bytes(n) / (1ull << 30));
    }
    c->cap = n;
    c->cap_pad = mp;
    SA_TRACE("workspace: rank %p keys0 %p keys1 %p vals_alt %p", (void*)c->rank, (void*)c->keys[0], (void*)c->keys[1],
             (void*)c->vals_alt);
    return SA_OK;
}

static int ensure_u_capacity(sa_context* c, uint64_t n) {
    if (n <= c->ucap && c->vals_u) return SA_OK;
    SA_HIP(hipSetDevice(c->device));
    free_u_buffers(c);
    const uint64_t m = align_up(std::max<uint64_t>(n, 1), 64) * 4;
    const uint64_t ku = align_up(std::max<uint64_t>(n, 1), 64) +
                        (n >= (1ull << 26) ? n / 16 + 8ull * 1024 * kXqSlack + 64 : 0);
    bool ok = hipMalloc(&c->vals_u, m) == hipSuccess && hipMalloc(&c->keys_u, 8 * ku) == hipSuccess &&
              hipMalloc(&c->member, align_up(n, 1024) / 8) == hipSuccess;
    for (int i = 0; i < 2 && ok; ++i)
        ok = hipMalloc(&c->u_pos[i], m) == hipSuccess && hipMalloc(&c->u_idx[i], m) == hipSuccess &&
             hipMalloc(&c->u_g[i], m) == hipSuccess;
    if (!ok) {
        free_u_buffers(c);
        (void)hipGetLastError();
        return set_err(SA_E_NOMEM, "device allocation of the unsorted-set buffers failed");
    }
    c->ucap = n;
    c->kucap = ku;
    SA_TRACE("unsorted-set buffers: vals_u %p keys_u %p", (void*)c->vals_u, (void*)c->keys_u);
    return SA_OK;
}

static int ensure_gs(sa_context* c, uint64_t n) {
    if (n <= c->gscap && c->u_gs[0]) return SA_OK;
    for (int i = 0; i < 2; ++i) {
        hipFree(c->u_gs[i]);
        c->u_gs[i] = nullptr;
    }
    c->gscap = 0;
    const uint64_t w = n / 2 + 64;
    for (int i = 0; i < 2; ++i)
        if (hipMalloc(&c->u_gs[i], w * 4) != hipSuccess) {
            (void)hipGetLastError();
            for (int k = 0; k < 2; ++k) {
                hipFree(c->u_gs[k]);
                c->u_gs[k] = nullptr;
            }
            return set_err(SA_E_NOMEM, "group-start buffers (%llu words)", (unsigned long long)w);
        }
    c->gscap = n;
    return SA_OK;
}

static bool gs_available(sa_context* c, uint64_t n) {
    if (ensure_gs(c, n) == SA_OK) return true;
    (void)hipGetLastError();
    g_err.clear();
    SA_TRACE("group-start buffers unavailable: pivot rounds without tied blocks");
    return false;
}

static uint32_t* gs_buf(const sa_context* c, uint64_t n, int i) { return n <= c->gscap ? c->u_gs[i] : nullptr; }

struct Timer {
    sa_context* c;
    hipStream_t s;
    bool on;
    sa_stats* st;
    int used = 0;
    int kind[kEvPool / 2];
    void begin(int k) {
        if (!on) return;
        if (used >= kEvPool / 2) flush();
        kind[used] = k;
        hipEventRecord(c->ev[2 * used], s);
    }
    void end() {
// ... 820 lines not shown
        Gt = c->host_words[21];
        Dt = c->host_words[22];
        if (T > t1 || Gt > G || Dt > G)
            return set_err(SA_E_INTERNAL, "tied blocks %llu / %llu / %llu out of range", (unsigned long long)T,
                           (unsigned long long)Gt, (unsigned long long)Dt);
    }
    uint32_t Pr = 0;
    uint64_t Dr = 0, mrr = 0, Gr = 0;
    if (mr > 0) {
        const uint32_t bits = bit_width(2 * G - 1) + wr;
        const uint32_t Pn = (bits + 7) / 8;
        uint32_t* const va = tied ? ridx + ra : c->u_g[uo];
        uint32_t* const vb = tied ? ridx + 2 * ra : c->u_idx[uo];
        uint32_t* vfinal = (Pn & 1u) ? va : vb;
        uint32_t* vother = (Pn & 1u) ? vb : va;
        uint64_t* rs = nullptr;
        int rc = radix_sort(c, SrcKeys{kbA, ridx}, 12 * mr, plan_chunks(mr), bits, vfinal, vother, ukb1, kbA, s, tm,
                            st, &rs, &Pr, false, true);
        if (rc) return rc;
        tm.begin(SA_K_SORT_U);
        const dim3 pg((uint32_t)std::min<uint64_t>((mr + kBlock - 1) / kBlock, 8192));
        if (tied)
            hipLaunchKernelGGL(k_pivot_place<true>, pg, dim3(kBlock), 0, s, (const uint64_t*)rs,
                               (const uint32_t*)vfinal, mr, (const uint32_t*)gs, (const uint32_t*)gP, Gu, wr, nullptr,
                               nullptr, m, (const uint32_t*)c->u_pos[ui], c->vals_u);
        else
            hipLaunchKernelGGL(k_pivot_place<false>, pg, dim3(kBlock), 0, s, (const uint64_t*)rs,
                               (const uint32_t*)vfinal, mr, (const uint32_t*)gs, (const uint32_t*)gP, Gu, wr, ukb0,
                               c->vals_u, m, nullptr, nullptr);
        tm.end();
        SA_HIP(hipGetLastError());
        add_bytes(st, SA_K_SORT_U, tied ? 20 * mr : 24 * mr);
        if (tied) {
            rc = segments(c, rs, vfinal, plan_chunks(mr), PosArray{c->vals_u}, false, nullptr, d_sa, uo, s, tm, st,
                          &Dr, &mrr, &Gr, nullptr, 0, RankMap{}, T, (uint32_t)Gt, c->u_gs[uo]);
            if (rc) return rc;
        }
    }
    *P = 1 + Pr;
    if (tied) {
        *gs_written = true;
        *segs_done = true;
        *Du = Dr + Dt;
        *m2 = mrr + T;
        *G2 = Gr + Gt;
    }
    *sorted = ukb0;
    return SA_OK;
}

static int pivot_round1(sa_context* c, uint64_t n, uint32_t bits1, uint32_t* d_sa, hipStream_t s, Timer& tm,
                        sa_stats* st, bool* done, uint64_t* D, uint64_t* m, uint64_t* G, uint32_t* P) {
    *done = false;
    const Chunking ch = plan_chunks(n);
    const uint64_t* keys = c->keys[1];
    uint32_t* const gs = c->u_pos[1];
    uint32_t* const toff = gs + 2;
    uint32_t* const tid = gs + 4;
    uint32_t* const gP = c->vals_alt;
    uint32_t* const cc = c->hist;
    c->host_words[24] = 0;
    c->host_words[25] = (uint32_t)n;
    SA_HIP(hipMemcpyAsync(gs, c->host_words + 24, 8, hipMemcpyHostToDevice, s));
    tm.begin(SA_K_PIVOT_COUNT);
    hipLaunchKernelGGL((k_pivot_pass<0, true>), dim3(ch.chunks), dim3(kBlock), 0, s, keys, nullptr, nullptr, ch,
                       (const uint32_t*)gs, nullptr, 1u, 0u, cc, gP, nullptr, nullptr, nullptr, nullptr, TiedOut{});
    hipLaunchKernelGGL(k_scan_rows, dim3(3), dim3(kBlock), 0, s, cc, ch.chunks, c->totals);
    tm.end();
    SA_HIP(hipGetLastError());
    add_bytes(st, SA_K_PIVOT_COUNT, 8 * n);
    SA_HIP(hipMemcpyAsync(c->host_words + 16, c->totals, 12, hipMemcpyDeviceToHost, s));
    SA_HIP(host_sync(s));
    const uint64_t t0 = c->host_words[16], t1 = c->host_words[17], t2 = c->host_words[18];
    if (t0 + t1 + t2 != n) return set_err(SA_E_INTERNAL, "round-1 pivot classes %llu + %llu + %llu != %llu",
                                          (unsigned long long)t0, (unsigned long long)t1, (unsigned long long)t2,
                                          (unsigned long long)n);
    SA_TRACE("  round 1: pivot split, tied %llu of %llu", (unsigned long long)t1, (unsigned long long)n);
    if (t1 * 2 < n) return SA_OK;
    const uint64_t mr = t0 + t2;
    uint64_t* const rk = c->keys[0];
    uint32_t* const ridx = c->u_idx[1];
    if (!gs_available(c, n)) return SA_OK;
    tm.begin(SA_K_PIVOT_WRITE);
    hipLaunchKernelGGL(k_pivot_gp, dim3(1), dim3(kBlock), 0, s, (const uint32_t*)gs, 1u, (const uint32_t*)cc, ch,
                       (const uint32_t*)c->totals, gP);
    hipLaunchKernelGGL(k_pivot_tied_scan, dim3(1), dim3(kBlock), 0, s, (const uint32_t*)gP, 1u, toff, tid,
                       c->totals + 4);
    const TiedOut to{nullptr, toff, tid, c->rank, d_sa, c->u_pos[0], c->u_idx[0], c->u_g[0], c->u_gs[0]};
    hipLaunchKernelGGL((k_pivot_pass<3, true>), dim3(ch.chunks), dim3(kBlock), 0, s, keys, nullptr, nullptr, ch,
                       (const uint32_t*)gs, nullptr, 1u, 0u, cc, gP, nullptr, nullptr, rk, ridx, to);
    tm.end();
    SA_HIP(hipGetLastError());
    add_bytes(st, SA_K_PIVOT_WRITE, 8 * n + 16 * t1 + 12 * mr);
    SA_HIP(hipMemcpyAsync(c->host_words + 20, c->totals + 4, 12, hipMemcpyDeviceToHost, s));
    SA_HIP(host_sync(s));
    const uint64_t T = c->host_words[20], Gt = c->host_words[21], Dt = c->host_words[22];
    if (T > t1 || Gt > 1 || Dt > 1)
        return set_err(SA_E_INTERNAL, "round-1 tied block %llu / %llu / %llu out of range", (unsigned long long)T,
                       (unsigned long long)Gt, (unsigned long long)Dt);
    uint32_t Pr = 0;
    uint64_t Dr = 0, mrr = 0, Gr = 0;
    if (mr > 0) {
        const uint32_t Pn = (bits1 + 7) / 8;
        uint32_t* const vfinal = (Pn & 1u) ? c->u_g[1] : ridx;
        uint32_t* const vother = (Pn & 1u) ? ridx : c->u_g[1];
        uint64_t* rs = nullptr;
        int rc = radix_sort(c, SrcKeys{rk, ridx}, 12 * mr, plan_chunks(mr), bits1, vfinal, vother, c->keys_u, rk, s,
                            tm, st, &rs, &Pr);
        if (rc) return rc;
        rc = segments(c, rs, vfinal, plan_chunks(mr), PosGap{t0, t1}, false, nullptr, d_sa, 0, s, tm, st, &Dr, &mrr,
                      &Gr, nullptr, 0, RankMap{}, T, (uint32_t)Gt, c->u_gs[0]);
        if (rc) return rc;
    }
    *done = true;
    *D = Dr + Dt;
    *m = mrr + T;
    *G = Gr + Gt;
    *P = 2 + Pr;
    return SA_OK;
}

static int build_packed(sa_context* c, const uint8_t* d_text, uint64_t n, uint32_t* d_sa, hipStream_t s,
                        const sa_opts* opts, sa_stats* st, Timer& tm) {
    int rc = SA_OK;
    rc = ensure_u_capacity(c, n);
    if (rc) return rc;
    tm.round_mark();
    uint32_t* h_alpha = c->host_words + 64;
    uint16_t* h_code = reinterpret_cast<uint16_t*>(c->host_words + 320);
    const uint32_t tail_n = (uint32_t)std::min<uint64_t>(n, (uint64_t)kMaxK);
    uint8_t* h_tail = reinterpret_cast<uint8_t*>(c->host_words + 2048);
    uint32_t sigma = 0, K = 0, Kb = 0;
    BucketPlan bp;
    const int r1 = opts ? opts->round1 : SA_ROUND1_AUTO;
    bool bucketed = false;
    auto plan_round1 = [&](bool sampled, bool* complete) -> int {
        SA_HIP(hipMemsetAsync(c->alpha, 0, 8 * 4, s));
        tm.begin(SA_K_ALPHABET);
        if (sampled) {
            const bool first4k = (c->dbg & SA_DEBUG_ALPHA_SAMPLE_SMALL) != 0;
            const uint64_t nb = alpha_text_blocks(n), ns = alpha_sample_blocks(n, first4k);
            hipLaunchKernelGGL(k_alphabet_sample, dim3((uint32_t)std::min<uint64_t>(ns, 2ull * (uint32_t)c->cus)),
                               dim3(kBlock), 0, s, d_text, n, nb, ns, c->alpha);
            add_bytes(st, SA_K_ALPHABET, alpha_sample_bytes(n, first4k));
        } else {
            const uint32_t grid = (uint32_t)std::min<uint64_t>((n + kBlock * 16 - 1) / (kBlock * 16), SA_ALPHA_GRID);
            hipLaunchKernelGGL(k_alphabet, dim3(grid), dim3(kBlock), 0, s, d_text, n, c->alpha);
            add_bytes(st, SA_K_ALPHABET, n);
        }
        tm.end();
        SA_HIP(hipGetLastError());
        SA_HIP(hipMemcpyAsync(h_alpha, c->alpha, 8 * 4, hipMemcpyDeviceToHost, s));
        SA_HIP(hipMemcpyAsync(h_tail, d_text + (n - tail_n), tail_n, hipMemcpyDeviceToHost, s));
        SA_HIP(host_sync(s));
        *complete = true;
        for (uint32_t t = 0; t < tail_n; ++t) {
            const uint32_t x = h_tail[t];
            if (!((h_alpha[x >> 5] >> (x & 31)) & 1u)) *complete = false;
            h_alpha[x >> 5] |= 1u << (x & 31);
        }
        sigma = 0;
        for (int b = 0; b < 256; ++b) h_code[b] = ((h_alpha[b >> 5] >> (b & 31)) & 1u) ? (uint16_t)(++sigma) : 0;
        SA_HIP(hipMemcpyAsync(c->code, h_code, 256 * 2, hipMemcpyHostToDevice, s));
        c->dna = sigma == 4 && h_code['A'] && h_code['C'] && h_code['G'] && h_code['T'];
        K = choose_chars(sigma, n, opts ? opts->init_chars : 0);
        Kb = (opts && opts->init_chars > 0) || sigma <= 1 ? K : min_chars(sigma, n);
        bucketed = plan_bucketed(sigma, n, Kb, r1, c->radix, &bp, 1, (c->dbg & SA_DEBUG_NO_CMP) ? 0 : 1);
        if (bucketed && bp.bs.cmp && short_suffix_ties(h_tail, n, tail_n, h_code, sigma, bp.bs.s, bp.bs.R))
            bucketed = plan_bucketed(sigma, n, Kb, r1, c->radix, &bp, 1, 0);
        const bool force_eonly = (c->dbg & SA_DEBUG_EONLY) != 0;
        if (bucketed && bp.bs.cmp == 1 && ((sigma & (sigma - 1)) != 0 || force_eonly) &&
            !(c->dbg & SA_DEBUG_NO_EONLY)) {
            const uint32_t hb = bp.bs.bb - kLoBits;
            BucketPlan b2;
            if ((force_eonly || !plan_pk8(bp, hb, c->dbg, true)) && plan_bucketed(sigma, n, Kb, r1, c->radix, &b2, 1, 2) &&
                (force_eonly || plan_pk8(b2, hb, c->dbg, true)) &&
                !short_suffix_ties(h_tail, n, tail_n, h_code, sigma, b2.bs.s, b2.bs.R, b2.K))
                bp = b2;
        }
        return SA_OK;
    };
    bool sampled = !(c->dbg & SA_DEBUG_NO_ALPHA_SAMPLE) &&
                   (n >= kPadMinN || (c->dbg & SA_DEBUG_ALPHA_SAMPLE_SMALL)) && c->radix == 0 && r1 != SA_ROUND1_LSD;
    bool refuted = false;
    uint64_t* keys1 = nullptr;
    uint32_t ksh1 = 0;
    uint32_t P = 0;
    bool fused = false;
    bool r1_pivot = false;
    uint64_t D = 0, m = 0, G = 0;
    uint64_t seg1[3] = {0, 0, 0};
    int r2 = 0;
    for (;;) {
        bool complete = true;
        rc = plan_round1(sampled, &complete);
        if (rc) return rc;
        if (sampled && !(bucketed && complete)) {
            SA_TRACE("packed: sampled alphabet (sigma=%u) not kept: %s", sigma,
                     complete ? "round 1 is not bucketed" : "the tail holds another symbol");
            sampled = false;
            continue;
        }
        c->samples_pending = false;
        if (!bucketed) break;
        bool done = false;
        c->alpha_prove = sampled && sigma < 256;
        c->alpha_refuted = false;
        rc = round1_bucketed(c, d_text, n, d_sa, bp, full_range(bp, n), s, tm, st, &done, &fused, seg1, &ksh1, true,
                             true, &r2);
        c->alpha_prove = false;
        if (rc) return rc;
        if (c->alpha_refuted) {
            SA_TRACE("packed: the first pass met a symbol outside the sampled alphabet, again with the exact one");
            sampled = false;
            refuted = true;
            continue;
        }
        bucketed = done;
        if (done) {
            keys1 = c->keys[0];
            P = 2;
            K = bp.K;
        }
        break;
    }
    if (st) st->alphabet = refuted ? SA_ALPHABET_REFUTED : sampled ? SA_ALPHABET_SAMPLED : SA_ALPHABET_EXACT;
    const uint64_t base = (uint64_t)sigma + 1;
    const Chunking ch = plan_chunks(n);
    if (!bucketed) {
        const uint32_t bits1 = key_bits(base, K);
        SA_TRACE("packed: sigma=%u K=%u bits=%u", sigma, K, bits1);
        uint64_t top = 1;
        for (uint32_t t = 1; t < K; ++t) top *= base;
        if (c->radix == 0) {
            rc = onesweep_prepare(c, s);
            if (rc) return rc;
        }
        tm.begin(SA_K_PACK);
        hipLaunchKernelGGL(k_pack_text, dim3(ch.chunks), dim3(kBlock), 0, s, d_text, n, (const uint16_t*)c->code, ch,
                           base, top, K, c->keys[1], c->hist, c->radix == 0 ? (bits1 + 7) / 8 : 0u, os_ghist(c));
        tm.end();
        SA_HIP(hipGetLastError());
        add_bytes(st, SA_K_PACK, 9 * n);
        if (c->radix == 0 && !(c->dbg & SA_DEBUG_NO_PIVOT) && n >= (1u << 16)) {
            rc = pivot_round1(c, n, bits1, d_sa, s, tm, st, &r1_pivot, &D, &m, &G, &P);
            if (rc) return rc;
        }
        if (!r1_pivot) {
            SrcKeysIota src{c->keys[1]};
            rc = radix_sort(c, src, 8 * n, ch, bits1, d_sa, c->vals_alt, c->keys[0], c->keys[1], s, tm, st, &keys1,
                            &P, true);
            if (rc) return rc;
        }
    }
    if (st) {
        st->init_chars = (int32_t)K;
        st->sigma = (int32_t)sigma;
        st->round1 = bucketed ? SA_ROUND1_BUCKETED : r1_pivot ? SA_ROUND1_PIVOT : SA_ROUND1_LSD;
    }
    int uo = 0;
    bool sparse = false;
    bool gs_ok[2] = {false, false};
    if (r1_pivot) {
        gs_ok[0] = true;
    } else if (bucketed && fused) {
        D = seg1[0];
        m = seg1[1];
        G = seg1[2];
        sparse = true;
    } else {
        rc = segments(c, keys1, d_sa, ch, PosIdentity{}, true, &sparse, nullptr, uo, s, tm, st, &D, &m, &G, nullptr,
                      0, RankMap{}, 0, 0, gs_buf(c, n, uo));
        if (rc) return rc;
        gs_ok[uo] = gs_buf(c, n, uo) != nullptr;
    }
    uint64_t* ukb0 = keys1 == c->keys[0] ? c->keys[1] : c->keys[0];
    uint64_t* ukb1 = c->keys_u;
    const RankLookup rl{c->rank, c->member, keys1, d_text, (const uint16_t*)c->code, n, base, K,
                        bucketed ? 1u : 0u, bp.bs, bucketed ? c->segw + kBstartOff : nullptr, d_sa, ksh1};
    if (st) st->sparse_ranks = sparse ? 1 : 0;
    auto ensure_samples = [&]() -> int {
        if (!c->samples_pending) return SA_OK;
        c->samples_pending = false;
        const uint64_t ns = (n + (1ull << ksh1) - 1) >> ksh1;
        const uint32_t g = (uint32_t)std::max<uint64_t>(1, std::min<uint64_t>((ns + kBlock - 1) / kBlock, 8192));
        tm.begin(SA_K_SORT_U);
        hipLaunchKernelGGL(k_key1_samples, dim3(g), dim3(kBlock), 0, s, d_text, n, (const uint16_t*)c->code, bp.bs,
                           (const uint32_t*)d_sa, ksh1, keys1);
        tm.end();
        SA_HIP(hipGetLastError());
        add_bytes(st, SA_K_SORT_U, 12 * ns);
        return SA_OK;
    };
    if (r2 == 0) tm.round_mark();
    record_round(st, 0.f, D, P, n, K);
    SA_TRACE("  round 1: D=%llu unsorted=%llu groups=%llu", (unsigned long long)D, (unsigned long long)m,
             (unsigned long long)G);
    if (r2 == 2) {
        tm.round_mark();
        D = n;
        record_round(st, 0.f, D, 1, m, 2 * (uint64_t)K);
        SA_TRACE("  round h=%u: sorted %llu from the local sort's staging, D=%llu", K, (unsigned long long)m,
                 (unsigned long long)D);
        m = 0;
        G = 0;
    }
// ... 988 lines not shown
```

### hpc_suffix_array_amd/csrc/sa_round1.h

```cpp
#pragma once

#ifndef SA_HIST_WPC
#define SA_HIST_WPC 64
#endif
#ifndef SA_REC_STRIPED
#define SA_REC_STRIPED 1
#endif
#ifndef SA_BB_EXTRA
#define SA_BB_EXTRA 0
#endif
#ifndef SA_ITEMS_A
#define SA_ITEMS_A 12
#endif
#ifndef SA_TEXT_BLOCK
#define SA_TEXT_BLOCK 512
#endif
#ifndef SA_LIST_BLOCK
#define SA_LIST_BLOCK 1024
#endif


#ifndef SA_SEG_BLOCK
#define SA_SEG_BLOCK 1024
#endif
// ... 16 lines not shown
constexpr uint64_t kPadMinN = 1ull << 26;
#ifndef SA_LS_VARIANT
#define SA_LS_VARIANT 0
#endif
static int ls_variant(const sa_context* c) {
    const uint32_t t = ((uint32_t)c->tune >> 16) & 0xFu;
    return t ? (int)(t - 1u) : SA_LS_VARIANT;
}

static uint32_t text_stripes(const sa_context* c) {
    const uint32_t e = ((uint32_t)c->tune >> 8) & 0xFFu;
    const uint32_t v = e ? e : 8u;
    return v >= 8 ? 8u : v >= 4 ? 4u : v >= 2 ? 2u : 1u;
}

__global__ __launch_bounds__(kLoRadix) void k_sum_rows(const uint32_t* __restrict__ in, uint32_t rows,
                                                       uint32_t* __restrict__ out) {
    uint32_t t = 0;
    for (uint32_t r = 0; r < rows; ++r) t += in[r * kLoRadix + threadIdx.x];
    out[threadIdx.x] = t;
}
constexpr uint64_t kPadMaxN = 1ull << 31;
constexpr int kUsFlagWord = 12;
constexpr int kAlphaBadWord = 8;

static uint32_t key1_bits(const BucketSpec& bs) {
    unsigned __int128 dmax = 1;
    for (uint32_t t = 0; t < bs.s; ++t) dmax *= bs.sigma;
    const unsigned __int128 kmax = ((dmax - 1) << bs.rb) | (((unsigned __int128)1 << bs.rb) - 1);
    uint32_t kw = 0;
    for (unsigned __int128 x = kmax + 1; x; x >>= 1) ++kw;
    return kw;
}
constexpr uint32_t kPadStartOff = kLoRadix + 1024;
constexpr uint32_t kPadDenseOff = kPadStartOff + kLoRadix + 64;

struct BucketPlan {
    BucketSpec bs{};
    uint32_t ib = 0;
    uint32_t K = 0;
};

static bool plan_bucketed(uint32_t sigma, uint64_t n, uint32_t K, int round1, int radix, BucketPlan* p,
                          int world = 1, int cmp = 0) {
    if (round1 == SA_ROUND1_LSD || radix != 0 || sigma < 2 || n < 2) return false;
    if (round1 == SA_ROUND1_AUTO && n < kBucketMinN) return false;
    uint32_t bb = std::max<uint32_t>(16u, bit_width(n - 1) > 13 ? bit_width(n - 1) - 13 : 0u);
    if (world <= 1) bb = std::min<uint32_t>(bb, 18u);
    bb += SA_BB_EXTRA;
    if (bb > 18 + (uint32_t)bit_width((uint64_t)std::max(world, 1) - 1) || bb > 24) return false;
    uint64_t ps = 1;
    uint32_t s = 0;
    while (ps < (1ull << bb)) {
        ps *= sigma;
        ++s;
    }
    while (ps % (1ull << bb) != 0 && ps < (64ull << bb) && s + 1 < K && ps * sigma <= (1ull << 32)) {
        ps *= sigma;
        ++s;
    }
    if (ps > (1ull << 32)) return false;
    if (K <= s || K > (uint32_t)kMaxK) return false;
    const uint32_t ib = bit_width(n - 1);
    const uint32_t bd = bit_width(ps - 1);
    const uint32_t span = bit_width((ps + (1ull << bb) - 1) >> bb) + 1;
    for (uint32_t R = K - s; R >= 1; --R) {
        unsigned __int128 pr = 1;
        for (uint32_t t = 0; t < R; ++t) pr *= sigma;
        unsigned __int128 lowmax = cmp == 2 ? pr - 1 : cmp ? 2 * pr - 1 : s + (pr - 1) * (R + 1) + R;
        uint32_t rb = 0;
        while (lowmax) {
            ++rb;
            lowmax >>= 1;
        }
        if (bd + rb > 64 || rb + span + ib > 64) continue;
        p->bs.pow_s1 = ps / sigma;
        p->bs.powR1 = (uint64_t)(pr / sigma);
        p->bs.cmul = (1ull << 48) / ps;
        p->bs.bb = bb;
        p->bs.bsh = 48u - bb;
        p->bs.sigma = sigma;
        p->bs.s = s;
        p->bs.R = R;
        p->bs.rb = rb;
        p->bs.cmp = (uint32_t)cmp;
        p->ib = ib;
        p->K = s + R;
        return true;
    }
    return false;
}

static bool short_suffix_ties(const uint8_t* tail, uint64_t n, uint32_t t, const uint16_t* code, uint32_t sigma,
                              uint32_t s, uint32_t R, uint32_t last = 0) {
    auto dig = [&](uint8_t x) -> uint32_t { return code[x] ? code[x] - 1u : 0u; };
    const uint32_t K = s + R;
    if (last == 0) last = K - 1;
    uint64_t Ds[kMaxK + 1];
    unsigned __int128 rs[kMaxK + 1];
    uint32_t cnt = 0;
    for (uint32_t L = 1; L <= last && L <= n && L <= t; ++L) {
        const uint8_t* x = tail + (t - L);
        uint64_t D = 0;
        unsigned __int128 r = 0;
        for (uint32_t q = 0; q < s; ++q) D = D * sigma + (q < L ? dig(x[q]) : 0u);
        for (uint32_t q = s; q < K; ++q) r = r * sigma + (q < L ? dig(x[q]) : 0u);
        for (uint32_t o = 0; o < cnt; ++o)
            if (Ds[o] == D && rs[o] == r) return true;
        Ds[cnt] = D;
        rs[cnt] = r;
        ++cnt;
    }
    return false;
}

static bool plan_pk8(const BucketPlan& bp, uint32_t hb, uint32_t dbg, bool np2 = false) {
    const uint32_t sg = bp.bs.sigma;
    if (sg < 2 || (dbg & SA_DEBUG_NO_PK8)) return false;
    if ((sg & (sg - 1)) != 0) {
        if (!np2) return false;
        const uint64_t ps = bp.bs.pow_s1 * sg;
        const uint64_t per = ((ps + (1ull << bp.bs.bb) - 1) >> bp.bs.bb) + 1;
        return hb + bit_width(per - 1) + bp.bs.rb + bp.ib <= 64;
    }
    const uint32_t lg = (uint32_t)__builtin_ctz(sg);
    if (lg * bp.bs.s < bp.bs.bb) return false;
    return hb + (lg * bp.bs.s - bp.bs.bb) + bp.bs.rb + bp.ib <= 64;
}

struct BucketRange {
    uint32_t blo = 0, bhi = 0;
    uint64_t m = 0;
    uint64_t sa_off = 0;
    bool always_u = false;
    uint32_t* rank = nullptr;
    uint32_t* member = nullptr;
    uint32_t* prefix = nullptr;
    uint32_t* tmp_rank = nullptr;
};

static BucketRange full_range(const BucketPlan& bp, uint64_t n) {
    BucketRange r;
    r.blo = 0;
    r.bhi = 1u << bp.bs.bb;
    r.m = n;
    return r;
}

static uint32_t range_hb(uint32_t nb) {
    const uint32_t w = bit_width(nb > 1 ? nb - 1 : 1);
    return std::max<uint32_t>(7u, w > kLoBits ? w - kLoBits : 0u);
}

static int round1_bucketed(sa_context* c, const uint8_t* d_text, uint64_t n, uint32_t* d_sa, const BucketPlan& bp,
                           const BucketRange& br_, hipStream_t s, Timer& tm, sa_stats* st, bool* done, bool* fused,
                           uint64_t seg[3], uint32_t* ksh, bool allow_pad = true, bool allow_xq = true,
                           int* round2 = nullptr) {
    *done = false;
    *fused = false;
    *ksh = 0;
    if (round2) *round2 = 0;
    const uint64_t m = br_.m;
    const uint32_t blo = br_.blo, bhi = br_.bhi;
    if (bhi <= blo || bhi - blo > (1u << 18)) return set_err(SA_E_INTERNAL, "bucket range [%u, %u)", blo, bhi);
    int rc = onesweep_prepare(c, s);
    if (rc) return rc;
    SA_HIP(hipMemsetAsync(c->words, 0, 12, s));
    SA_HIP(hipMemsetAsync(c->words + 5, 0, 28, s));
    const bool listed = m * 10 <= n * 3;
    uint64_t* const lkeys = c->keys_u;
    uint32_t* const lpos = c->vals_u;
    const uint64_t rtiles = (n + kTile - 1) / kTile;
    const uint32_t rgrid = (uint32_t)(std::min<uint64_t>(rtiles, (uint64_t)SA_HIST_WPC * (uint32_t)c->cus) /
                                      kRecStripes * kRecStripes);
    const uint64_t rcap64 = (c->dbg & SA_DEBUG_PAD_OVERFLOW) ? m / kRecStripes / 2 + 1
                                                             : (m + m / 8) / kRecStripes + 2 * (uint64_t)kTile;
    const bool striped = SA_REC_STRIPED && listed && allow_pad && !(c->dbg & SA_DEBUG_NO_PAD) &&
                         rtiles >= 4ull * kRecStripes && rgrid >= kRecStripes && kRecStripes * rcap64 <= c->ucap;
    const uint32_t rcap = (uint32_t)std::min<uint64_t>(rcap64, UINT32_MAX);
    uint32_t* const rcur = c->hist;
    const bool padded = allow_pad && !listed && blo == 0 && bhi == (1u << bp.bs.bb) && n >= kPadMinN &&
                        n <= kPadMaxN && c->cap_pad >= pad_capacity(n) && !(c->dbg & SA_DEBUG_NO_PAD);
    const uint32_t ssh = std::max<uint32_t>(6u, bit_width(n) > 21 ? bit_width(n) - 21 : 0u);
    uint32_t* const pstart = os_base(c) + kPadStartOff;
    uint32_t* const dlo = os_base(c) + kPadDenseOff;
    if (st) st->round1_segments = padded ? 1 : striped ? 3 : 0;
    tm.begin(SA_K_PACK);
    if (padded) {
        const bool pow2 = (bp.bs.sigma & (bp.bs.sigma - 1)) == 0;
        const uint32_t g = (uint32_t)std::max<uint64_t>(1, std::min<uint64_t>(((n >> ssh) + kBlock - 1) / kBlock,
                                                                               4u * (uint32_t)c->cus));
        if (pow2)
            hipLaunchKernelGGL(k_bucket_sample<true>, dim3(g), dim3(kBlock), 0, s, d_text, n,
                               (const uint16_t*)c->code, bp.bs, ssh, os_ghist(c));
        else
            hipLaunchKernelGGL(k_bucket_sample<false>, dim3(g), dim3(kBlock), 0, s, d_text, n,
                               (const uint16_t*)c->code, bp.bs, ssh, os_ghist(c));
        hipLaunchKernelGGL(k_pad_starts, dim3(1), dim3(kLoRadix), 0, s, (const uint32_t*)os_ghist(c), ssh,
                           (c->dbg & SA_DEBUG_PAD_OVERFLOW) ? 1u : 0u, (uint32_t)c->cap_pad, pstart);
    } else {
        const uint64_t tiles = (n + kTile - 1) / kTile;
        const uint32_t g = (uint32_t)std::max<uint64_t>(1, std::min<uint64_t>(tiles, (uint64_t)SA_HIST_WPC * (uint32_t)c->cus));
        const bool pow2 = (bp.bs.sigma & (bp.bs.sigma - 1)) == 0;
        uint32_t* const wgcnt = c->hist;
        uint32_t* const wgoff = c->hist + g;
#define SA_HIST_G(G, P, L, W)                                                                                 \
    hipLaunchKernelGGL((k_bucket_hist<P, false, L>), dim3(G), dim3(kBlock), 0, s, d_text, n,                  \
                       (const uint16_t*)c->code, bp.bs, os_ghist(c), 0ull, n, blo, bhi, lkeys, lpos, W, rcap,  \
                       c->words + 11)
#define SA_HIST_ID_G(G, L, W)                                                                                 \
    hipLaunchKernelGGL((k_bucket_hist<true, false, L, true>), dim3(G), dim3(kBlock), 0, s, d_text, n,         \
                       (const uint16_t*)c->code, bp.bs, os_ghist(c), 0ull, n, blo, bhi, lkeys, lpos, W, rcap,  \
                       c->words + 11)
#define SA_HIST(P, L, W) SA_HIST_G(g, P, L, W)
#define SA_HIST_ID(L, W) SA_HIST_ID_G(g, L, W)
        const bool ident = bp.bs.sigma == 256;
        if (striped) {
            SA_HIP(hipMemsetAsync(rcur, 0, kRecStripes * kRecCurStride * 4, s));
            if (ident) SA_HIST_ID_G(rgrid, 3, rcur);
            else if (pow2 && SA_DNA_SWAR && c->dna)
                hipLaunchKernelGGL((k_bucket_hist<true, false, 3, false, true>), dim3(rgrid), dim3(kBlock), 0, s, d_text,
                                   n, (const uint16_t*)c->code, bp.bs, os_ghist(c), 0ull, n, blo, bhi, lkeys, lpos, rcur,
                                   rcap, c->words + 11);
            else if (pow2) SA_HIST_G(rgrid, true, 3, rcur);
            else SA_HIST_G(rgrid, false, 3, rcur);
            SA_HIP(hipMemcpyAsync(c->host_words + 11, c->words + 11, 4, hipMemcpyDeviceToHost, s));
            SA_HIP(host_sync(s));
            if (c->host_words[11]) {
                SA_TRACE("  bucketed round 1: a record stripe overflowed, again with the counting scan");
                tm.end();
                const int rc = round1_bucketed(c, d_text, n, d_sa, bp, br_, s, tm, st, done, fused, seg, ksh, false,
                                               allow_xq, round2);
                if (st) st->round1_segments = 4;
                return rc;
            }
        } else if (ident && listed) SA_HIST_ID(1, wgcnt);
        else if (pow2 && listed) SA_HIST(true, 1, wgcnt);
        else if (pow2) SA_HIST(true, 0, wgcnt);
        else if (listed) SA_HIST(false, 1, wgcnt);
        else SA_HIST(false, 0, wgcnt);
        if (listed && !striped) {
            hipLaunchKernelGGL(k_exscan_u32, dim3(1), dim3(kBlock), 0, s, (const uint32_t*)wgcnt, wgoff, g);
            if (ident) SA_HIST_ID(2, wgoff);
            else if (pow2) SA_HIST(true, 2, wgoff);
            else SA_HIST(false, 2, wgoff);
        }
#undef SA_HIST
#undef SA_HIST_ID
#undef SA_HIST_G
#undef SA_HIST_ID_G
    }
    tm.end();
    add_bytes(st, SA_K_PACK, padded ? (n >> ssh) * 64 : n + (striped ? 12 * m : listed ? n + 12 * m : 0));
    const uint32_t hb = (blo == 0 && bhi == (1u << bp.bs.bb)) ? bp.bs.bb - kLoBits : range_hb(bhi - blo);
    if (hb < 7 || hb > 10) return set_err(SA_E_INTERNAL, "second bucket pass of %u bits", hb);
    const uint32_t nb_tab = 1u << (hb + kLoBits);
    const bool np2 = (bp.bs.sigma & (bp.bs.sigma - 1)) != 0;
    const bool pk8 = plan_pk8(bp, hb, c->dbg, !br_.always_u);
    uint32_t bits1 = 0;
    if (bp.bs.cmp) {
        const uint64_t ps = bp.bs.pow_s1 * bp.bs.sigma, per = (ps + (1ull << bp.bs.bb) - 1) >> bp.bs.bb;
        const bool exact = (ps & ((1ull << bp.bs.bb) - 1)) == 0;
        bits1 = bit_width(exact ? per - 1 : per) + bp.bs.rb;
        if (c->span_extra > 0) bits1 = std::min<uint32_t>(bits1 + (uint32_t)c->span_extra, 64u - bp.ib);
    }
    const bool fast32 = bits1 > (uint32_t)kSubBits && bits1 - kSubBits <= kLowMax &&
                        (m / (uint64_t)(bhi - blo) >= 4ull * kWinStride || (c->dbg & SA_DEBUG_FAST32_SMALL)) &&
                        !(c->dbg & SA_DEBUG_NO_FAST32);
    static_assert(kXqQueues == kXq && kXqRegionSlack == kXqSlack, "sa_limits.h mirrors sa_split.h");
    const bool xq = SA_SEG_XQ && allow_xq && fast32 && c->cus % (int)kXq == 0 && !(c->dbg & SA_DEBUG_NO_XQ) &&
                    c->kucap >= xq_region_space(m) + kWave && xq_offsets_fit(m);
    if (st) st->round1_layout = (bp.bs.cmp ? 1 : 0) | (pk8 ? 2 : 0) | (xq ? 4 : 0) | (bp.bs.cmp == 2 ? 8 : 0);
    const uint64_t xqw = xq_words(1u << hb);
    uint32_t* xq_dh = nullptr;
    uint32_t* xq_pc = nullptr;
    uint32_t* xq_pn = nullptr;
    if (xq) {
        const uint64_t need = xqw + 1032 + 2ull * kXq * nb_tab;
        if (c->segx_words < need) {
            hipFree(c->segx);
            c->segx = nullptr;
            c->segx_words = 0;
            if (hipMalloc(&c->segx, need * 4) != hipSuccess) {
                (void)hipGetLastError();
                return set_err(SA_E_NOMEM, "second-pass queue workspace (%llu words)", (unsigned long long)need);
            }
            c->segx_words = need;
        }
        xq_dh = c->segx + xqw;
        xq_pc = xq_dh + 1032;
        xq_pn = xq_pc + (uint64_t)kXq * nb_tab;
    }
    uint32_t* const g_lo = os_ghist(c);
    uint32_t* const g_hi = os_ghist(c) + kLoRadix;
    const uint32_t stripes = padded ? text_stripes(c) : 1u;
    uint32_t* const cursor = stripes > 1 ? c->hist : os_ghist(c) + 5 * kRadix;
    uint32_t* const cursor_sum = stripes > 1 ? c->hist + kMaxStripes * kLoRadix : cursor;
    if (stripes > 1) SA_HIP(hipMemsetAsync(cursor, 0, (size_t)stripes * kLoRadix * 4, s));
    if (!padded) {
        tm.begin(SA_K_SCAN);
        hipLaunchKernelGGL(k_digit_base_wide, dim3(1), dim3(1024), 0, s, (const uint32_t*)g_lo, kLoRadix, os_base(c));
        tm.end();
    }
    tm.begin(SA_K_SCATTER_FIRST);
    {
        constexpr int kItemsA = SA_ITEMS_A;
        constexpr int kTextBlock = SA_TEXT_BLOCK;
        const bool pow2 = (bp.bs.sigma & (bp.bs.sigma - 1)) == 0;
        const bool dna = SA_DNA_SWAR && c->dna && bp.bs.s + bp.bs.R + kItemsA - 1 <= 32 && 2 * bp.bs.s <= 32;
        const bool ident = SA_TEXT_IDENT && bp.bs.sigma == 256 && bp.bs.s + bp.bs.R <= 8 && bp.bs.s <= 4;
        uint32_t* const alpha_bad = c->alpha_prove && !listed ? c->words + kAlphaBadWord : nullptr;
        auto text_grid = [&](int block) {
            const uint64_t tile = (uint64_t)block * kItemsA;
            return (uint32_t)std::max<uint64_t>(
                1, std::min<uint64_t>((n + tile - 1) / tile, (uint64_t)c->cus * (kSpBlock / block)));
        };
#define SA_TEXT_PASS(P, PK, BLK, DNA, ID)                                                                     \
    hipLaunchKernelGGL((k_split_text<kItemsA, BLK, P, PK, DNA, ID>), dim3(text_grid(BLK)), dim3(BLK), 0, s, d_text, n, \
                       (const uint16_t*)c->code, bp.bs, (const uint32_t*)(padded ? pstart : os_base(c)),           \
                       os_tickets(c), c->keys[0], c->vals_alt, g_hi, cursor, m, blo, bhi,                          \
                       padded ? (const uint32_t*)pstart + 1 : nullptr, padded ? c->words + 11 : nullptr, hb, bp.ib, \
                       stripes, alpha_bad)
        if (listed) {
            constexpr int kItemsL = SA_ITEMS_B, kListBlock = SA_LIST_BLOCK;
            const uint64_t tl = (uint64_t)kListBlock * kItemsL;
            const uint32_t gl = (uint32_t)std::max<uint64_t>(
                1, std::min<uint64_t>((m + tl - 1) / tl, (uint64_t)c->cus * (kSpBlock / kListBlock)));
            if (pk8)
                hipLaunchKernelGGL((k_split_list<kItemsL, kListBlock, true>), dim3(gl), dim3(kListBlock), 0, s, bp.bs,
                                   (const uint64_t*)lkeys, (const uint32_t*)lpos, m, blo, (const uint32_t*)os_base(c),
                                   os_tickets(c), c->keys[0], c->vals_alt, g_hi, cursor, hb, bp.ib,
                                   striped ? (const uint32_t*)rcur : nullptr, rcap);
            else
                hipLaunchKernelGGL((k_split_list<kItemsL, kListBlock, false>), dim3(gl), dim3(kListBlock), 0, s, bp.bs,
                                   (const uint64_t*)lkeys, (const uint32_t*)lpos, m, blo, (const uint32_t*)os_base(c),
                                   os_tickets(c), c->keys[0], c->vals_alt, g_hi, cursor, 0u, 0u,
                                   striped ? (const uint32_t*)rcur : nullptr, rcap);
        } else if (pk8 && np2) {
#define SA_TEXT_NP2(R32)                                                                                         \
    hipLaunchKernelGGL((k_split_text<kItemsA, kSpBlock, false, true, false, false, R32>), dim3(text_grid(kSpBlock)), \
                       dim3(kSpBlock), 0, s, d_text, n, (const uint16_t*)c->code, bp.bs,                           \
                       (const uint32_t*)(padded ? pstart : os_base(c)), os_tickets(c), c->keys[0], c->vals_alt, g_hi, \
                       cursor, m, blo, bhi, padded ? (const uint32_t*)pstart + 1 : nullptr,                        \
                       padded ? c->words + 11 : nullptr, hb, bp.ib, stripes, alpha_bad)
            if (bp.bs.powR1 * (uint64_t)bp.bs.sigma <= 0xFFFFFFFFull && !(((uint32_t)c->tune >> 28) & 1u))
                SA_TEXT_NP2(true);
            else
                SA_TEXT_NP2(false);
#undef SA_TEXT_NP2
        } else if (pk8 && dna) {
            SA_TEXT_PASS(true, true, kTextBlock, true, false);
        } else if (pk8 && ident) {
            SA_TEXT_PASS(true, true, kTextBlock, false, true);
        } else if (pk8) {
            SA_TEXT_PASS(true, true, kTextBlock, false, false);
        } else if (pow2 && ident) {
            SA_TEXT_PASS(true, false, kTextBlock, false, true);
        } else if (pow2) {
            SA_TEXT_PASS(true, false, kTextBlock, false, false);
        } else if (bp.bs.powR1 * (uint64_t)bp.bs.sigma <= 0xFFFFFFFFull && !(((uint32_t)c->tune >> 28) & 1u)) {
            hipLaunchKernelGGL((k_split_text<kItemsA, kSpBlock, false, false, false, false, true>),
                               dim3(text_grid(kSpBlock)), dim3(kSpBlock), 0, s, d_text, n, (const uint16_t*)c->code,
                               bp.bs, (const uint32_t*)(padded ? pstart : os_base(c)), os_tickets(c), c->keys[0],
                               c->vals_alt, g_hi, cursor, m, blo, bhi, padded ? (const uint32_t*)pstart + 1 : nullptr,
                               padded ? c->words + 11 : nullptr, hb, bp.ib, stripes, alpha_bad);
        } else {
            SA_TEXT_PASS(false, false, kSpBlock, false, false);
        }
#undef SA_TEXT_PASS
    }
    tm.end();
    add_bytes(st, SA_K_SCATTER_FIRST, listed ? (pk8 ? 20 : 24) * m : n + (pk8 ? 8 : 12) * m);
    tm.begin(SA_K_SCAN);
    hipLaunchKernelGGL(k_digit_base_wide, dim3(1), dim3(1024), 0, s, (const uint32_t*)g_hi, 1u << hb,
                       os_base(c) + kLoRadix);
    if (xq)
        hipLaunchKernelGGL(k_xq_dh, dim3(1), dim3(1024), 0, s, (const uint32_t*)g_hi, 1u << hb,
                           (c->dbg & SA_DEBUG_XQ_OVERFLOW) ? 1u : 0u, xq_dh);
    if (padded) {
        if (stripes > 1)
            hipLaunchKernelGGL(k_sum_rows, dim3(1), dim3(kLoRadix), 0, s, (const uint32_t*)cursor, stripes, cursor_sum);
        hipLaunchKernelGGL(k_digit_base_wide, dim3(1), dim3(1024), 0, s, (const uint32_t*)cursor_sum, kLoRadix, dlo);
    }
    tm.end();
    tm.begin(SA_K_SCATTER_KEYS);
    {
        constexpr int kItemsB = SA_ITEMS_B, kItemsPk = SA_ITEMS_PK;
        const SrcBucketKeys sb{c->keys[0], c->vals_alt, bp.bs.rb, bp.bs.bsh, bp.bs.cmul, blo};
        const SrcPk8 sp{c->keys[0]};
        uint32_t* tk = os_tickets(c) + 1;
        const uint32_t* hbase = os_base(c) + kLoRadix;
        SA_HIP(hipMemsetAsync(c->segw, 0, segw_words(1u << hb) * 4, s));
        SegXq sx;
        if (xq) {
            SA_HIP(hipMemsetAsync(c->segx, 0, xqw * 4, s));
            sx.cur = c->segx;
            sx.sbase = reinterpret_cast<uint64_t*>(c->segx + (uint64_t)kXq * kSegs * (1u << hb));
            sx.done = c->segx + 3ull * kXq * kSegs * (1u << hb);
            sx.tickets = sx.done + kXq * kSegs;
            sx.dh = xq_dh;
            sx.err2 = c->words + 9;
            sx.cap = (uint32_t)std::min<uint64_t>(c->kucap, UINT32_MAX);
        }
        constexpr int kSegBlock = SA_SEG_BLOCK;
        const int sblk = hb <= 9 ? kSegBlock : kSpBlock;
        const uint64_t ut = (uint64_t)sblk * (pk8 ? kItemsPk : kItemsB);
        const uint64_t units = (m + ut - 1) / ut + kSegs;
        const uint32_t grid = xq ? (uint32_t)c->cus * (kSpBlock / sblk)
                                 : (uint32_t)std::max<uint64_t>(1, std::min<uint64_t>(units, (uint64_t)c->cus * (kSpBlock / sblk)));
        switch (hb) {
#define SA_SEG_LAUNCH(S, B, SRC, SH, IT)                                                                      \
    if (xq)                                                                                                   \
        hipLaunchKernelGGL((k_split_seg<S, B, IT, (B <= 9 ? kSegBlock : kSpBlock), true>), dim3(grid),        \
                           dim3(B <= 9 ? kSegBlock : kSpBlock), 0, s, SRC, m, SH,                              \
                           (const uint32_t*)(padded ? pstart : os_base(c)), hbase, c->segw, tk, bp.ib, c->keys_u,      \
                           c->words + 4, padded ? (const uint32_t*)cursor : nullptr,                           \
                           padded ? (const uint32_t*)dlo : nullptr, stripes, sx);                              \
    else                                                                                                      \
        hipLaunchKernelGGL((k_split_seg<S, B, IT, (B <= 9 ? kSegBlock : kSpBlock)>), dim3(grid),                \
                           dim3(B <= 9 ? kSegBlock : kSpBlock), 0, s, SRC, m, SH,                              \
                           (const uint32_t*)(padded ? pstart : os_base(c)), hbase, c->segw, tk, bp.ib, c->keys_u,      \
                           c->words + 4, padded ? (const uint32_t*)cursor : nullptr,                           \
                           padded ? (const uint32_t*)dlo : nullptr, stripes)
#define SA_SEG_PASS(B)                                                                                        \
    case B:                                                                                                   \
        if (pk8) SA_SEG_LAUNCH(SrcPk8, B, sp, 64u - B, kItemsPk);                                             \
        else SA_SEG_LAUNCH(SrcBucketKeys, B, sb, kLoBits, kItemsB);                                           \
        break;
            SA_SEG_PASS(7)
            SA_SEG_PASS(8)
            SA_SEG_PASS(9)
            SA_SEG_PASS(10)
#undef SA_SEG_PASS
#undef SA_SEG_LAUNCH
            default: return set_err(SA_E_INTERNAL, "second bucket pass of %u bits", hb);
        }
        const uint32_t gb = (uint32_t)std::min<uint64_t>(((uint64_t)nb_tab + kBlock) / kBlock, 1024);
        uint32_t* bstart = c->segw + kBstartOff;
        uint32_t* bdmin = bstart + kBstartWords;
#define SA_BSTARTS(R)                                                                                         \
    if (xq)                                                                                                   \
        hipLaunchKernelGGL(k_bucket_starts_xq<R>, dim3(R), dim3(kLoRadix), 0, s, hbase, (const uint32_t*)sx.cur, \
                           (const uint32_t*)xq_dh, m, bp.bs.cmul, bp.bs.bsh, bstart, bdmin, xq_pc, xq_pn, blo); \
    else                                                                                                      \
        hipLaunchKernelGGL(k_bucket_starts<R>, dim3(gb), dim3(kBlock), 0, s, (const uint32_t*)(padded ? dlo : os_base(c)), \
                           hbase, (const uint32_t*)c->segw, m, bp.bs.cmul, bp.bs.bsh, bstart, bdmin, blo)
        switch (hb) {
            case 7: SA_BSTARTS(128); break;
            case 8: SA_BSTARTS(256); break;
            case 9: SA_BSTARTS(512); break;
            default: SA_BSTARTS(1024); break;
        }
#undef SA_BSTARTS
    }
    tm.end();
    add_bytes(st, SA_K_SCATTER_KEYS, (pk8 ? 16 : 20) * m);
    SA_HIP(hipGetLastError());
    const uint64_t nw = (m + kWinStride - 1) / kWinStride;
    uint32_t* ws = c->vals_alt;
    uint32_t* list = c->vals_alt + nw + 1;
    tm.begin(SA_K_WINDOWS);
    {
        const uint32_t g1 = (uint32_t)std::min<uint64_t>((nw + kBlock) / kBlock, 8192);
        hipLaunchKernelGGL(k_window_starts_tab, dim3(g1), dim3(kBlock), 0, s, (const uint32_t*)(c->segw + kBstartOff),
                           nb_tab, m, nw, ws, list + 4 * nw + 2);
        const uint32_t g2 = (uint32_t)std::min<uint64_t>((nw + kBlock - 1) / kBlock, 1024);
        hipLaunchKernelGGL(k_window_list, dim3(g2), dim3(kBlock), 0, s, (const uint32_t*)ws, nw, list, c->words);
    }
    tm.end();
    add_bytes(st, SA_K_WINDOWS, 8 * nw);
    SA_HIP(hipGetLastError());
    SA_HIP(hipMemcpyAsync(c->host_words, c->words, 48, hipMemcpyDeviceToHost, s));
    uint32_t* skew = list + nw;
    uint32_t* cnt_u = skew + nw;
    uint32_t* cnt_g = cnt_u + nw + 1;
    uint32_t* const rank_arr = br_.rank ? br_.rank : c->rank;
    uint32_t* const member = br_.member ? br_.member : c->member;
    SA_HIP(hipEventRecord(c->ev[kSyncEv], s));
    SA_HIP(hipMemsetAsync(cnt_u, 0, (2 * nw + 2) * 4, s));
    SA_HIP(hipMemsetAsync(member, 0, (n + 31) / 32 * 4, s));
    SA_HIP(host_sync_event(c->ev[kSyncEv]));
    if (c->alpha_prove && c->host_words[kAlphaBadWord]) {
        c->alpha_refuted = true;
        return SA_OK;
    }
    if (c->host_words[4]) return set_err(SA_E_INTERNAL, "radix look-back did not complete");
    if (padded && c->host_words[11]) {
        SA_TRACE("  bucketed round 1: padded segment overflow, again with exact digit totals");
        const int rc = round1_bucketed(c, d_text, n, d_sa, bp, br_, s, tm, st, done, fused, seg, ksh, false, allow_xq,
                                       round2);
        if (st) st->round1_segments = 2;
        return rc;
    }
    if (xq && c->host_words[9]) {
        SA_TRACE("  bucketed round 1: second-pass queue overflow, again with one region");
        return round1_bucketed(c, d_text, n, d_sa, bp, br_, s, tm, st, done, fused, seg, ksh, allow_pad, false,
                               round2);
    }
    if (st) st->largest_window = (int32_t)std::min<uint32_t>(c->host_words[5], INT32_MAX);
    if (c->host_words[5] > (uint32_t)kBsCap) {
        SA_TRACE("  bucketed round 1: window of %u > %d suffixes, full sort instead", c->host_words[5], kBsCap);
        return SA_OK;
    }
    BucketRel br{cnt_g + nw + 1, c->segw + kBstartOff, c->segw + kBstartOff + kBstartWords, bp.bs.rb};
    br.bits1 = bits1;
    SegOut so{rank_arr, member, br_.sa_off, c->u_pos[1], c->u_idx[1], c->u_g[1], cnt_u, cnt_g, kKeySample};
    so.tmp_rank = br_.prefix ? br_.tmp_rank : nullptr;
    so.samples = (SA_LAZY_SAMPLES && !br_.always_u && !(c->dbg & SA_DEBUG_NO_KEY1_ROUND)) ? 0u : 1u;
    uint32_t* const retry = cnt_g + 2 * nw + 2;
    BucketRel br_measured = br;
    br_measured.bits1 = 0;
    uint4* const hdr = reinterpret_cast<uint4*>(((uintptr_t)(retry + nw + 4) + 15) & ~(uintptr_t)15);
    uint32_t* const hx = xq ? reinterpret_cast<uint32_t*>(hdr + nw + 1) : nullptr;
    constexpr uint32_t kBsRows = (kBsBlock / kWave) * kBsItems;
    uint32_t* const xrows = xq ? hx + 16 * (nw + 1) : nullptr;
    const uint64_t* const wide_in = xq ? c->keys[1] : c->keys_u;
    auto local_sort = [&](const SegOut& o) {
        const uint32_t g = std::max<uint32_t>(1, std::min(c->host_words[7], kBsGrid));
        static_assert(kRetryWord == kUsFlagWord + 1, "one memset clears words[12..15]");
        (void)hipMemsetAsync(c->words + kUsFlagWord, 0, 16, s);
        if (fast32) {
            const uint32_t gs = (uint32_t)std::max<uint64_t>(1, std::min<uint64_t>((nw + kBlock - 1) / kBlock, 1024));
            const bool cr = xq && !(((uint32_t)c->tune >> 29) & 1u);
            const uint32_t ls_grid = (c->dbg & SA_DEBUG_LS_ONE_WG) ? 1u : kBsWpc * (uint32_t)c->cus;
            hipLaunchKernelGGL(k_window_split, dim3(gs), dim3(kBlock), 0, s, (const uint32_t*)list, (const uint32_t*)ws,
                               br, c->words, hdr, retry, 1u, (const uint32_t*)xq_pc, (const uint32_t*)xq_pn, nb_tab, hx,
                               cr ? kBsRows : 0u);
            if (xq) {
                if (cr)
                    hipLaunchKernelGGL(k_window_rows<true>, dim3(2048), dim3(kBlock), 0, s, (const uint32_t*)c->words,
                                       (const uint4*)hdr, (const uint32_t*)hx, kBsRows, xrows);
                else
                    hipLaunchKernelGGL(k_window_rows<false>, dim3(2048), dim3(kBlock), 0, s, (const uint32_t*)c->words,
                                       (const uint4*)hdr, (const uint32_t*)hx, kBsRows, xrows);
                XqWin xw;
                xw.hx = hx;
                xw.rows = xrows;
#define SA_LS_XQ(V, CR)                                                                                          \
    hipLaunchKernelGGL((k_bucket_sort<kBsBlock, kBsItems, NoProbe, true, V, CR>), dim3(ls_grid), dim3(kBsBlock), 0, \
                       s, (const uint64_t*)c->keys_u, (const uint4*)hdr, bp.bs.rb, br.bits1, bp.ib, c->words,      \
                       c->keys[0], d_sa, retry, o, xw)
                switch (ls_variant(c) | (cr ? 4 : 0)) {
                case 1: SA_LS_XQ(1, false); break;
                case 2: SA_LS_XQ(2, false); break;
                case 3: SA_LS_XQ(3, false); break;
                case 4: SA_LS_XQ(0, true); break;
                case 5: SA_LS_XQ(1, true); break;
                case 6: SA_LS_XQ(2, true); break;
                case 7: SA_LS_XQ(3, true); break;
                default: SA_LS_XQ(0, false); break;
                }
#undef SA_LS_XQ
                hipLaunchKernelGGL(k_window_gather, dim3(1024), dim3(kBlock), 0, s, (const uint32_t*)retry,
                                   (const uint32_t*)c->words, (const uint32_t*)ws, (const uint32_t*)br.wb,
                                   (const uint32_t*)xq_pc, (const uint32_t*)xq_pn, nb_tab, (const uint64_t*)c->keys_u,
                                   c->keys[1]);
            } else {
#define SA_LS(V)                                                                                                 \
    hipLaunchKernelGGL((k_bucket_sort<kBsBlock, kBsItems, NoProbe, false, V>), dim3(ls_grid), dim3(kBsBlock), 0, \
                       s, (const uint64_t*)c->keys_u, (const uint4*)hdr, bp.bs.rb, br.bits1, bp.ib, c->words,   \
                       c->keys[0], d_sa, retry, o)
                switch (ls_variant(c)) {
                case 1: SA_LS(1); break;
                case 2: SA_LS(2); break;
                case 3: SA_LS(3); break;
                default: SA_LS(0); break;
                }
#undef SA_LS
            }
        } else {
            hipLaunchKernelGGL((k_bucket_sort_wide<kBsBlock, kBsItems>), dim3(g), dim3(kBsBlock), 0, s,
                               (const uint64_t*)c->keys_u, br, (const uint32_t*)ws, (const uint32_t*)list, c->words,
                               bp.ib, c->keys[0], d_sa, skew, o, br.bits1 ? retry : (uint32_t*)nullptr, 7u);
        }
        if (br.bits1)
            hipLaunchKernelGGL((k_bucket_sort_wide<kBsBlock, kBsItems>), dim3(std::min<uint32_t>(g, 1024)),
                               dim3(kBsBlock), 0, s, wide_in, br_measured, (const uint32_t*)ws,
                               (const uint32_t*)retry, c->words, bp.ib, c->keys[0], d_sa, skew, o, (uint32_t*)nullptr,
                               (uint32_t)kRetryWord);
        const uint32_t gl = std::min<uint32_t>(g, 1024);
        hipLaunchKernelGGL((k_bucket_sort_lsd<kBsBlock, kBsItems>), dim3(gl), dim3(kBsBlock), 0, s,
                           wide_in, br, (const uint32_t*)ws, (const uint32_t*)skew, c->words, bp.ib,
                           c->keys[0], d_sa, o);
    };
    tm.begin(SA_K_LOCAL_SORT);
    local_sort(so);
    tm.end();
    add_bytes(st, SA_K_LOCAL_SORT, 12 * m + (so.samples ? (m >> kKeySample) * 8 : 0));
    SA_HIP(hipGetLastError());
    auto gather_u = [&]() {
        const uint32_t wb = (uint32_t)((nw + 1 + kWsBlock - 1) / kWsBlock);
        uint32_t* part = c->hist;
        hipLaunchKernelGGL(k_wscan_reduce, dim3(wb), dim3(kBlock), 0, s, (const uint32_t*)cnt_u, (const uint32_t*)cnt_g,
                           nw, part);
        hipLaunchKernelGGL(k_wscan_top, dim3(1), dim3(kBlock), 0, s, part, wb);
        hipLaunchKernelGGL(k_wscan_apply, dim3(wb), dim3(kBlock), 0, s, cnt_u, cnt_g, nw, (const uint32_t*)part);
        const uint32_t g = (uint32_t)std::max<uint64_t>(1, std::min<uint64_t>((c->host_words[7] + kWaves - 1) / kWaves, 4096));
        RankMap rm;
        if (br_.prefix) {
            const uint64_t nwb = (n + 31) / 32;
            const uint32_t pb = (uint32_t)((nwb + kPcBlock - 1) / kPcBlock);
            uint32_t* ppart = br_.prefix + nwb + 1;
            hipLaunchKernelGGL(k_popc_reduce, dim3(pb), dim3(kBlock), 0, s, (const uint32_t*)member, nwb, ppart);
            hipLaunchKernelGGL(k_popc_top, dim3(1), dim3(kPcTop), 0, s, ppart, pb);
            hipLaunchKernelGGL(k_popc_apply, dim3(pb), dim3(kBlock), 0, s, (const uint32_t*)member, nwb,
                               (const uint32_t*)ppart, br_.prefix);
            rm = RankMap{member, br_.prefix};
        }
        hipLaunchKernelGGL(k_u_gather, dim3(g), dim3(kBlock), 0, s, (const uint32_t*)list, (const uint32_t*)c->words,
                           (const uint32_t*)ws, (const uint32_t*)cnt_u, (const uint32_t*)cnt_g, so, c->u_pos[0],
                           c->u_idx[0], c->u_g[0], rm);
    };
    const bool try_r2 = round2 && so.rank && !br_.always_u && !so.tmp_rank && br_.sa_off == 0 &&
                        !(c->dbg & (SA_DEBUG_NO_KEY1_ROUND | SA_DEBUG_NO_ROUND2_FUSED)) && key1_bits(bp.bs) <= 64;
    if (try_r2) {
        tm.round_mark();
        tm.begin(SA_K_SORT_U);
        const uint64_t per = (uint64_t)kWaves * kR2Batch;
        const uint32_t g = (uint32_t)std::max<uint64_t>(1, std::min<uint64_t>((c->host_words[7] + per - 1) / per, 65536));
        hipLaunchKernelGGL(k_round2_windows, dim3(g), dim3(kBlock), 0, s, (const uint32_t*)list,
                           (const uint32_t*)c->words, (const uint32_t*)ws, (const uint32_t*)cnt_u,
                           (const uint32_t*)so.tmp_pos, (const uint32_t*)so.tmp_idx, (const uint32_t*)so.tmp_g, d_text, n,
                           (const uint16_t*)c->code, bp.bs, m, d_sa, c->words + kUsFlagWord);
        tm.end();
    } else {
        tm.begin(SA_K_SEG_WRITE);
        gather_u();
        tm.end();
    }
    SA_HIP(hipGetLastError());
    SA_HIP(hipMemcpyAsync(c->host_words, c->words, 64, hipMemcpyDeviceToHost, s));
    SA_HIP(host_sync(s));
    if (st) {
        const uint32_t wv[4] = {c->host_words[7], c->host_words[kHdrWord], c->host_words[kRetryWord], c->host_words[10]};
        for (int t = 0; t < 4; ++t) st->round1_windows[t] = (int32_t)std::min<uint32_t>(wv[t], INT32_MAX);
    }
    if (c->host_words[6]) {
        SA_TRACE("  bucketed round 1: local sort flags %u, full sort instead", c->host_words[6]);
        if (try_r2) tm.round_unmark();
        return SA_OK;
    }
    seg[0] = c->host_words[0];
    seg[1] = c->host_words[1];
    seg[2] = c->host_words[2];
    add_bytes(st, SA_K_LOCAL_SORT, seg[1] * 28);
    const bool sparse = br_.always_u || seg[1] <= n / kSparseDiv;
    if (try_r2) {
        add_bytes(st, SA_K_SORT_U, seg[1] * 28);
        if (!sparse) {
            tm.round_unmark();
        } else if (c->host_words[kUsFlagWord] == 0) {
            SA_TRACE("  bucketed round 1: round 2 finished from the staging (%llu members)",
                     (unsigned long long)seg[1]);
            *round2 = 2;
        } else {
            SA_TRACE("  bucketed round 1: round 2 from the staging gave up, the set compacted");
            *round2 = 1;
            tm.begin(SA_K_SEG_WRITE);
            gather_u();
            tm.end();
            SA_HIP(hipGetLastError());
        }
    }
    if (!try_r2 || *round2 == 1) add_bytes(st, SA_K_SEG_WRITE, 8 * (2 * nw + 2) + seg[1] * 24);
    if (!sparse) {
        SegOut full{};
        full.ksh = 0;
        SA_HIP(hipMemsetAsync(c->words + 10, 0, 4, s));
        tm.begin(SA_K_LOCAL_SORT);
        local_sort(full);
        tm.end();
        add_bytes(st, SA_K_LOCAL_SORT, 20 * m);
        SA_HIP(hipGetLastError());
    } else {
        *ksh = kKeySample;
        *fused = true;
        c->samples_pending = so.samples == 0u;
    }
    SA_TRACE("  bucketed round 1: s=%u R=%u rb=%u cmp=%u pk8=%d windows=%u (skewed %u) largest=%u", bp.bs.s, bp.bs.R,
             bp.bs.rb, bp.bs.cmp, pk8 ? 1 : 0, c->host_words[7], c->host_words[10], c->host_words[5]);
    *done = true;
    return SA_OK;
}
```

### include/sa_hip.h

```cpp
#ifndef SA_HIP_H
#define SA_HIP_H

#include <stdint.h>

#ifdef __cplusplus
extern "C" {
#endif

#define SA_OK 0
#define SA_E_INVALID (-1)
#define SA_E_NOMEM (-2)
#define SA_E_HIP (-3)
#define SA_E_INTERNAL (-4)

#define SA_MAX_ROUNDS 64

enum sa_kernel_kind {
    SA_K_INIT = 0,
    SA_K_HIST_FIRST = 1,
    SA_K_HIST_KEYS = 2,
    SA_K_SCAN = 3,
    SA_K_SCATTER_FIRST = 4,
    SA_K_SCATTER_KEYS = 5,
    SA_K_HEADS = 6,
    SA_K_HEADS_SCAN = 7,
    SA_K_RERANK = 8,
    SA_K_SEG_COUNT = 9,
    SA_K_SEG_SCAN = 10,
    SA_K_SEG_WRITE = 11,
    SA_K_ALPHABET = 12,
    SA_K_PACK = 13,
    SA_K_SORT_U = 14,
    SA_K_WINDOWS = 15,
    SA_K_LOCAL_SORT = 16,
    SA_K_PIVOT_KEYS = 17,
    SA_K_PIVOT_COUNT = 18,
    SA_K_PIVOT_WRITE = 19,
    SA_K_COUNT = 20
};

#define SA_ROUND1_AUTO 0
#define SA_ROUND1_LSD 1
#define SA_ROUND1_BUCKETED 2
#define SA_ROUND1_PIVOT 3

#define SA_SCHEDULE_PACKED 0
#define SA_SCHEDULE_REFERENCE 1

#define SA_DEBUG_NO_CMP 0x1u
#define SA_DEBUG_NO_PK8 0x2u
#define SA_DEBUG_NO_PAD 0x4u
#define SA_DEBUG_PAD_OVERFLOW 0x8u
#define SA_DEBUG_NO_FAST32 0x10u
#define SA_DEBUG_NO_PIVOT 0x20u
#define SA_DEBUG_PERM_ALWAYS 0x40u
#define SA_DEBUG_NO_XQ 0x80u
#define SA_DEBUG_XQ_OVERFLOW 0x100u
#define SA_DEBUG_NO_KEY1_ROUND 0x400u
#define SA_DEBUG_NO_TIED 0x200u
#define SA_DEBUG_NO_EONLY 0x800u
#define SA_DEBUG_EONLY 0x1000u
#define SA_DEBUG_FAST32_SMALL 0x2000u
#define SA_DEBUG_NO_ROUND2_FUSED 0x4000u
#define SA_DEBUG_LS_ONE_WG 0x8000u
#define SA_DEBUG_NO_ALPHA_SAMPLE 0x10000u
#define SA_DEBUG_ALPHA_SAMPLE_SMALL 0x20000u

#define SA_ALPHABET_EXACT 0
#define SA_ALPHABET_SAMPLED 1
#define SA_ALPHABET_REFUTED 2

typedef struct {
    int32_t profile;
    int32_t schedule;
    int32_t init_chars;
    int32_t radix;
    int32_t round1;
    uint32_t debug;
    int32_t span_extra;
    int32_t tune;
} sa_opts;

typedef struct {
    int32_t rounds;
    int32_t n_kinds;
    double total_ms;
    double h2d_ms, d2h_ms;
    double round_ms[SA_MAX_ROUNDS];
    uint64_t distinct[SA_MAX_ROUNDS];
    int32_t passes[SA_MAX_ROUNDS];
    uint64_t sorted_n[SA_MAX_ROUNDS];
    uint64_t prefix_len[SA_MAX_ROUNDS];
    int32_t schedule;
    int32_t init_chars;
    int32_t sigma;
    int32_t sparse_ranks;
    int32_t round1;
    int32_t largest_window;
    uint64_t model_bytes;
    double kern_ms[SA_K_COUNT];
    uint64_t kern_launches[SA_K_COUNT];
    uint64_t kern_bytes[SA_K_COUNT];
    int32_t round1_segments;
    int32_t round1_layout;
    uint64_t round_bytes[SA_MAX_ROUNDS];
    int32_t round1_windows[4];
    int32_t alphabet;
} sa_stats;

typedef struct sa_context sa_context;

int sa_context_create(int device, uint64_t max_n, sa_context** out);
int sa_context_set_debug(sa_context* ctx, const sa_opts* opts);
void sa_context_destroy(sa_context* ctx);
uint64_t sa_workspace_bytes(uint64_t max_n);

int sa_build_device(sa_context* ctx, const uint8_t* d_text, uint64_t n, uint32_t* d_sa,
                    void* stream, const sa_opts* opts, sa_stats* stats);

int sa_build_ex(const uint8_t* text, uint64_t n, void* sa_out, int sa_width,
                const sa_opts* opts, sa_stats* stats);

int sa_check_device(sa_context* ctx, const uint8_t* d_text, uint64_t n, const uint32_t* d_sa,
                    void* stream);
int sa_check(const uint8_t* text, uint64_t n, const void* sa, int sa_width);

int sa_lcp_device(sa_context* ctx, const uint8_t* d_text, uint64_t n, const uint32_t* d_sa, uint32_t* d_lcp,
                  uint64_t* lrs_len, uint64_t* lrs_pos, void* stream);
int sa_lcp(const uint8_t* text, uint64_t n, const void* sa, int sa_width, void* lcp_out, uint64_t* lrs_len,
           uint64_t* lrs_pos);


#define SA_FIND_LANE 1u
#define SA_FIND_WAVE 2u
#define SA_FIND_LANE_MAX 3584

int sa_find_device(const uint8_t* d_text, uint64_t n, const uint32_t* d_sa,
                   const uint8_t* d_pat, uint64_t pat_bytes, const uint64_t* d_pat_off ,
                   uint64_t nq, uint32_t* d_lo, uint32_t* d_hi, uint32_t flags, void* stream);
int sa_find(const uint8_t* text, uint64_t n, const void* sa, int sa_width,
            const uint8_t* pat, const uint64_t* pat_off, uint64_t nq,
            uint64_t* lo_out, uint64_t* hi_out);
int sa_find_ex(const uint8_t* text, uint64_t n, const void* sa, int sa_width,
               const uint8_t* pat, const uint64_t* pat_off, uint64_t nq,
               uint64_t* lo_out, uint64_t* hi_out, uint32_t flags);

int sa_match_device(const uint8_t* d_text, uint64_t n, const uint32_t* d_sa,
                    const uint8_t* d_pat, uint64_t pat_bytes, const uint64_t* d_pat_off ,
                    uint64_t nq, uint32_t* d_len, uint32_t* d_lo, uint32_t* d_hi, uint32_t flags, void* stream);
int sa_matching_stats_device(const uint8_t* d_text, uint64_t n, const uint32_t* d_sa,
                             const uint8_t* d_query, uint64_t m, uint64_t max_len ,
                             uint32_t* d_len, uint32_t* d_lo, uint32_t* d_hi ,
                             uint32_t flags, void* stream);
int sa_match(const uint8_t* text, uint64_t n, const void* sa, int sa_width,
             const uint8_t* pat, const uint64_t* pat_off, uint64_t nq,
             uint64_t* len_out, uint64_t* lo_out, uint64_t* hi_out, uint32_t flags);
int sa_matching_stats(const uint8_t* text, uint64_t n, const void* sa, int sa_width,
                      const uint8_t* query, uint64_t m, uint64_t max_len,
                      uint64_t* len_out, uint64_t* lo_out, uint64_t* hi_out, uint32_t flags);

#define SA_BWT_STATS 258

int sa_bwt_device(const uint8_t* d_text, uint64_t n, const uint32_t* d_sa, uint8_t* d_bwt,
                  uint64_t* d_stats , void* stream);
int sa_bwt(const uint8_t* text, uint64_t n, const void* sa, int sa_width, uint8_t* bwt_out,
           uint64_t* stats_out );

int sa_inverse_device(sa_context* ctx, uint64_t n, const uint32_t* d_sa, uint32_t* d_isa, void* stream);
int sa_inverse(const void* sa, uint64_t n, int sa_width, void* isa_out );

#define SA_IBWT_INFO 3

int sa_lf_device(sa_context* ctx, const uint8_t* d_bwt, uint64_t n, uint64_t primary, uint32_t* d_lf, void* stream);
int sa_ibwt_device(sa_context* ctx, const uint8_t* d_bwt, uint64_t n, uint64_t primary, uint8_t* d_text,
                   uint32_t* d_sa , uint64_t* info , void* stream);
int sa_lf(const uint8_t* bwt, uint64_t n, uint64_t primary, void* lf_out, int width);
int sa_ibwt(const uint8_t* bwt, uint64_t n, uint64_t primary, uint8_t* text_out, void* sa_out ,
            int sa_width);
int sa_ibwt_ex(const uint8_t* bwt, uint64_t n, uint64_t primary, uint8_t* text_out, void* sa_out ,
               int sa_width, uint64_t* info );

#define SA_FM_INFO 4
#define SA_FM_MAX_SAMPLE 4096

uint64_t sa_fm_index_bytes(uint64_t n, uint32_t sa_sample);

int sa_fm_build_device(sa_context* ctx, const uint8_t* d_bwt, uint64_t n, uint64_t primary,
                       const uint32_t* d_sa , uint32_t sa_sample, void* d_index,
                       uint64_t index_bytes, uint64_t* info , void* stream);
int sa_fm_count_device(const void* d_index, uint64_t index_bytes, const uint8_t* d_pat, uint64_t pat_bytes,
                       const uint64_t* d_pat_off, uint64_t nq, uint32_t* d_lo, uint32_t* d_hi, void* stream);
int sa_fm_locate_device(sa_context* ctx, const void* d_index, uint64_t index_bytes, const uint32_t* d_lo,
                        const uint32_t* d_hi, uint64_t nq, uint64_t max_hits, uint32_t flags,
                        uint64_t* d_off , uint32_t* d_pos , uint64_t pos_cap,
                        uint64_t* total, void* stream);
int sa_fm_build(const uint8_t* bwt, uint64_t n, uint64_t primary, const void* sa ,
                int sa_width, uint32_t sa_sample, void* index_out, uint64_t index_bytes,
                uint64_t* info );
int sa_fm_count(const void* index, uint64_t index_bytes, const uint8_t* pat, const uint64_t* pat_off, uint64_t nq,
                uint64_t* lo_out, uint64_t* hi_out);
int sa_fm_locate(const void* index, uint64_t index_bytes, const uint64_t* lo, const uint64_t* hi, uint64_t nq,
                 uint64_t max_hits, uint32_t flags, uint64_t* off_out , void* pos_out, int pos_width,
                 uint64_t pos_cap);

#define SA_LOCATE_SA_ORDER 1u
#define SA_LOCATE_SMALL_CHUNKS 2u
#define SA_LOCATE_TILE 2048

int sa_locate_device(sa_context* ctx, uint64_t n, const uint32_t* d_sa, const uint32_t* d_lo, const uint32_t* d_hi,
                     uint64_t nq, uint64_t max_hits, uint32_t flags, uint64_t* d_off ,
                     uint32_t* d_pos , uint64_t pos_cap, uint64_t* total, void* stream);
int sa_locate(const void* sa, uint64_t n, int sa_width, const uint64_t* lo, const uint64_t* hi, uint64_t nq,
              uint64_t max_hits, uint32_t flags, uint64_t* off_out , void* pos_out, uint64_t pos_cap);

#define SA_DOC_NONE 0xFFFFFFFFu
#define SA_DOC_RANK_ORDER 1u
#define SA_DOC_TILE 2048
#define SA_DOC_GROUP_MAX 256
#define SA_DOC_LDS_DOCS 8192

int sa_doc_array_device(sa_context* ctx, uint64_t n, const uint32_t* d_sa, const uint64_t* d_doc_off, uint64_t D,
                        uint32_t* d_da , uint32_t* d_prev , void* stream);
int sa_doc_of_device(const uint64_t* d_doc_off, uint64_t D, uint64_t n, const uint32_t* d_pos, uint64_t count,
                     uint32_t* d_doc , uint32_t* d_rel , void* stream);
int sa_doc_frequency_device(uint64_t n, const uint32_t* d_prev, const uint32_t* d_lo, const uint32_t* d_hi, uint64_t nq,
                            uint32_t* d_df, void* stream);
int sa_doc_list_device(sa_context* ctx, uint64_t n, const uint32_t* d_da, const uint32_t* d_prev, const uint32_t* d_lo,
                       const uint32_t* d_hi, uint64_t nq, uint64_t max_docs, uint32_t flags, uint64_t* d_off ,
                       uint32_t* d_docs , uint64_t docs_cap, uint64_t* total, void* stream);
int sa_doc_array(const void* sa, uint64_t n, int sa_width, const uint64_t* doc_off , uint64_t D,
                 void* da_out , void* prev_out );
int sa_doc_of(const uint64_t* doc_off , uint64_t D, uint64_t n, const void* pos, uint64_t count, int width,
              void* doc_out , void* rel_out );
int sa_doc_frequency(const void* prev, uint64_t n, int width, const uint64_t* lo, const uint64_t* hi, uint64_t nq,
                     uint64_t* df_out);
int sa_doc_list(const void* da, const void* prev, uint64_t n, int width, const uint64_t* lo, const uint64_t* hi,
                uint64_t nq, uint64_t max_docs, uint32_t flags, uint64_t* off_out , void* docs_out,
                uint64_t docs_cap);

#define SA_MEM_INFO 3
#define SA_MEM_TOO_MANY 1
#define SA_MEM_LANE 1u
#define SA_MEM_WAVE 2u

int sa_mems_device(sa_context* ctx, const uint8_t* d_text, uint64_t n, const uint32_t* d_sa, const uint8_t* d_query,
                   uint64_t m, uint64_t min_len, uint64_t max_occ, uint64_t max_candidates, uint32_t flags,
                   uint64_t* d_off , uint32_t* d_tpos, uint32_t* d_len, uint64_t out_cap,
                   uint64_t info[SA_MEM_INFO], void* stream);
int sa_mems(const uint8_t* text, uint64_t n, const void* sa, int sa_width, const uint8_t* query, uint64_t m,
            uint64_t min_len, uint64_t max_occ, uint64_t max_candidates, uint32_t flags,
            uint64_t* off_out , void* tpos_out, void* len_out , uint64_t out_cap,
            uint64_t info[SA_MEM_INFO]);

#define SA_LPF_NONE 0xFFFFFFFFu

int sa_lpf_device(sa_context* ctx, const uint8_t* d_text, uint64_t n, const uint32_t* d_sa,
                  const uint32_t* d_lcp , uint32_t* d_lpf, uint32_t* d_src, void* stream);
int sa_lz77_device(sa_context* ctx, uint64_t n, const uint32_t* d_lpf, const uint32_t* d_src, uint32_t* d_pos,
                   uint32_t* d_len, uint32_t* d_fsrc, uint64_t out_cap, uint64_t* z, void* stream);
// ... 89 lines not shown
```

Measured before the change: 109.9 billion.

## Speculatively launch round-1 local sort before host check, gate on device flags

Round-1 local sort is now enqueued before the host reads back the status words. A device-side gate in the window-split kernel aborts when overflow or refutation flags are set, which removes a host round-trip stall between the window build and the local sort. Scratch buffers (words, hist, segw, member, counters) are cleared early with one fused clear kernel launched during alphabet sampling, replacing several separate memsets. It also lowers the round-2 batch from 16 to 4 and adds an optional compile-time path that computes XQ rows in-kernel, off by default. Risks are wasted work when the gate stops, and subtle ordering bugs with cleared-ahead state.

```diff
diff --git a/hpc_suffix_array_amd/_native.py b/hpc_suffix_array_amd/_native.py
--- a/hpc_suffix_array_amd/_native.py
+++ b/hpc_suffix_array_amd/_native.py
@@ -133,6 +133,7 @@
         ("round1_layout", ctypes.c_int32),
         ("round_bytes", ctypes.c_uint64 * SA_MAX_ROUNDS),
         ("round1_windows", ctypes.c_int32 * 4),
+        ("round1_gate", ctypes.c_int32),
         ("alphabet", ctypes.c_int32),
     ]
 
@@ -161,6 +162,7 @@
             "reference_model_bytes": int(self.model_bytes),
             "round_bytes": [int(x) for x in self.round_bytes[:r]],
             "round1_windows": [int(x) for x in self.round1_windows],
+            "round1_gate": {0: "not_speculated", 1: "ran", 2: "stopped"}.get(self.round1_gate, "not_speculated"),
             "alphabet": {0: "exact", 1: "sampled", 2: "refuted"}.get(self.alphabet, "exact"),
             "kernels": {k: {"ms": self.kern_ms[i], "launches": int(self.kern_launches[i]),
                             "bytes": int(self.kern_bytes[i])} for i, k in enumerate(KERNEL_KINDS)},
diff --git a/hpc_suffix_array_amd/csrc/sa_bucket.h b/hpc_suffix_array_amd/csrc/sa_bucket.h
--- a/hpc_suffix_array_amd/csrc/sa_bucket.h
+++ b/hpc_suffix_array_amd/csrc/sa_bucket.h
@@ -2,6 +2,7 @@
 #include <type_traits>
 
 #include "sa_kernels.h"
+#include "sa_rows.h"
 
 namespace sa {
 
@@ -422,6 +423,35 @@
     }
 }
 
+constexpr int kClearMax = 8;
+struct ClearRanges {
+    uint32_t* p[kClearMax];
+    uint64_t words[kClearMax];
+    int n = 0;
+    void add(uint32_t* q, uint64_t w) {
+        if (w && n < kClearMax) {
+            p[n] = q;
+            words[n++] = w;
+        }
+    }
+};
+
+__global__ __launch_bounds__(kBlock) void k_clear_ranges(ClearRanges r) {
+    const uint64_t gid = (uint64_t)blockIdx.x * kBlock + threadIdx.x, gsz = (uint64_t)gridDim.x * kBlock;
+    for (int i = 0; i < r.n; ++i) {
+        uint32_t* const p = r.p[i];
+        const uint64_t w = r.words[i];
+        const uint64_t mis = ((16u - (uint32_t)((uintptr_t)p & 15u)) & 15u) / 4u;
+        const uint64_t head = mis < w ? mis : w;
+        const uint64_t nq = (w - head) / 4;
+        uint4* const q = reinterpret_cast<uint4*>(p + head);
+        for (uint64_t j = gid; j < nq; j += gsz) q[j] = make_uint4(0u, 0u, 0u, 0u);
+        const uint64_t done = head + 4 * nq;
+        if (gid < head) p[gid] = 0u;
+        if (gid < w - done) p[done + gid] = 0u;
+    }
+}
+
 template <bool POW2>
 __global__ __launch_bounds__(kBlock) void k_bucket_sample(const uint8_t* __restrict__ text, uint64_t n,
                                                           const uint16_t* __restrict__ code, BucketSpec b,
@@ -850,7 +880,11 @@
     }
 }
 
-constexpr int kR2Batch = 16;
+#ifndef SA_R2_BATCH
+#define SA_R2_BATCH 4
+#endif
+constexpr int kR2Batch = SA_R2_BATCH;
+static_assert(kR2Batch >= 1 && kR2Batch <= kWave, "one listed window per lane");
 
 __global__ __launch_bounds__(kBlock) void k_round2_windows(const uint32_t* __restrict__ list, const uint32_t* words,
                                                            const uint32_t* __restrict__ ws,
@@ -1332,6 +1366,8 @@
 static_assert(kBsCap <= (1 << kSlotBits), "load slots in kSlotBits");
 constexpr int kHdrWord = 14;
 constexpr int kTicketWord = 15;
+constexpr uint32_t kGateOn = 1u, kGateAlpha = 2u, kGateXq = 4u, kGatePad = 8u;
+constexpr uint32_t kGateStopped = 1u << 31;
 
 __global__ __launch_bounds__(kBlock) void k_window_split(const uint32_t* __restrict__ list,
                                                          const uint32_t* __restrict__ ws, BucketRel br,
@@ -1339,7 +1375,16 @@
                                                          uint32_t* __restrict__ retry, uint32_t fast,
                                                          const uint32_t* __restrict__ pc = nullptr,
                                                          const uint32_t* __restrict__ pn = nullptr, uint32_t nb = 0,
-                                                         uint32_t* __restrict__ hx = nullptr, uint32_t crows = 0) {
+                                                         uint32_t* __restrict__ hx = nullptr, uint32_t crows = 0,
+                                                         uint32_t gate = 0) {
+    if (gate & kGateOn) {
+        const bool stop = words[4] != 0u || words[5] > (uint32_t)kBsCap || ((gate & kGateAlpha) && words[8] != 0u) ||
+                          ((gate & kGateXq) && words[9] != 0u) || ((gate & kGatePad) && words[11] != 0u);
+        if (stop) {
+            if (blockIdx.x == 0 && threadIdx.x == 0) atomicOr(&words[6], kGateStopped);
+            return;
+        }
+    }
     const uint32_t nlist = words[7];
     const uint32_t lane = lane_id();
     for (uint64_t q0 = (uint64_t)blockIdx.x * kBlock; q0 < nlist; q0 += (uint64_t)gridDim.x * kBlock) {
@@ -1513,6 +1558,28 @@
     for (int t = 0; t < 3; ++t) rv[t] = rows[t * ROWS + r];
 }
 
+#ifndef SA_LS_ROWCALC
+#define SA_LS_ROWCALC 0
+#endif
+__device__ __forceinline__ void load_hdr_cr(const uint32_t* __restrict__ hx, uint32_t m, uint32_t (&raw)[3]) {
+    raw[0] = hx[lane_id() & (2 * kRowChunks - 1)];
+    raw[1] = m;
+}
+
+template <int ITEMS>
+__device__ __forceinline__ void calc_rows_cr(const uint32_t (&raw)[3], uint32_t (&rv)[3]) {
+    uint32_t hv[2 * kRowChunks];
+#pragma unroll
+    for (int k = 0; k < (int)(2 * kRowChunks); ++k) hv[k] = (uint32_t)__builtin_amdgcn_readlane((int)raw[0], k);
+    uint32_t st[kRowChunks], cn[kRowChunks];
+    chunk_spans(hv, (uint32_t)__builtin_amdgcn_readfirstlane((int)raw[1]), st, cn);
+    const uint32_t lane = lane_id();
+    const uint32_t w = (uint32_t)__builtin_amdgcn_readfirstlane((int)(threadIdx.x / kWave));
+    const RowWords x = chunk_row(st, cn, w * ITEMS + (lane < (uint32_t)ITEMS ? lane : 0u));
+    rv[0] = x.base;
+    rv[1] = x.count;
+}
+
 template <int ITEMS, int I0 = 0, int I1 = ITEMS>
 __device__ __forceinline__ void load_items_xq(const uint64_t* __restrict__ w_in, const uint32_t (&rv)[3], uint32_t m,
                                               uint64_t (&x)[ITEMS]) {
@@ -1542,33 +1609,14 @@
 #pragma unroll
         for (int k = 0; k < 16; ++k) hv[k] = hx[q * 16 + k];
         if constexpr (CR) {
-            uint32_t st[kXq], cn[kXq], nfull = 0;
-#pragma unroll
-            for (int k = 0; k < (int)kXq; ++k) {
-                const uint32_t p0 = k ? hv[kXq - 1 + k] : 0u, p1 = k + 1 < (int)kXq ? hv[kXq + k] : m;
-                st[k] = hv[k] + p0;
-                cn[k] = p1 - p0;
-                nfull += cn[k] / kWave;
-            }
+            static_assert(kRowChunks == kXq && kRowLanes == (uint32_t)kWave, "sa_rows.h mirrors the XQ layout");
+            uint32_t st[kXq], cn[kXq];
+            chunk_spans(hv, m, st, cn);
             for (uint32_t r = lane; r < nrows; r += kWave) {
-                uint32_t base = st[0], cnt = 0, rf = 0, rp = nfull;
-#pragma unroll
-                for (int k = 0; k < (int)kXq; ++k) {
-                    const uint32_t nf = cn[k] / kWave, rem = cn[k] % kWave;
-                    if (r >= rf && r < rf + nf) {
-                        base = st[k] + kWave * (r - rf);
-                        cnt = kWave;
-                    }
-                    if (rem && r == rp) {
-                        base = st[k] + kWave * nf;
-                        cnt = rem;
-                    }
-                    rf += nf;
-                    rp += rem ? 1u : 0u;
-                }
+                const RowWords x = chunk_row(st, cn, r);
                 uint32_t* const e = rows + q * 3 * nrows + r;
-                e[0] = base;
-                e[nrows] = cnt;
+                e[0] = x.base;
+                e[nrows] = x.count;
             }
             continue;
         }
@@ -1671,7 +1719,11 @@
     uint64_t w[ITEMS];
     uint32_t rv[3] = {0u, 0u, 0u};
     if constexpr (XQ) {
-        load_rows_xq<ITEMS, ROWS>(xw.rows + (uint64_t)q * 3 * ROWS, rv);
+        if constexpr (CR && SA_LS_ROWCALC) {
+            uint32_t raw[3];
+            load_hdr_cr(xw.hx + (uint64_t)q * 16, h.z, raw);
+            calc_rows_cr<ITEMS>(raw, rv);
+        } else load_rows_xq<ITEMS, ROWS>(xw.rows + (uint64_t)q * 3 * ROWS, rv);
         if constexpr (CR) load_items_cr<ITEMS>(keys_in, rv, w);
         else load_items_xq<ITEMS>(keys_in, rv, h.z, w);
     } else {
@@ -1687,9 +1739,14 @@
         mx = qx < nwin;
         hx = make_uint4(0u, 0u, 1u, 0u);
         if (mx) hx = hdr[qx];
-        if constexpr (XQ) load_rows_xq<ITEMS, ROWS>(xw.rows + (uint64_t)(mx ? qx : cur) * 3 * ROWS, rx);
+        if constexpr (XQ && CR && SA_LS_ROWCALC) {
+            load_hdr_cr(xw.hx + (uint64_t)(mx ? qx : cur) * 16, mx ? hx.z : h.z, rx);
+        } else if constexpr (XQ) {
+            load_rows_xq<ITEMS, ROWS>(xw.rows + (uint64_t)(mx ? qx : cur) * 3 * ROWS, rx);
+        }
     };
     if constexpr (HR) next_window(s_q[1], q, qn, more, hn, rwn);
+    uint32_t rc[3] = {0u, 0u, 0u};
     uint32_t par = 0;
     for (;;) {
         probe.mark(-1);
@@ -1719,7 +1776,9 @@
             constexpr int B = decltype(rest)::value ? ITEMS : (HR ? kLsPfHr[P] : kLsPfOld[P]);
             if constexpr (A < B) {
                 __builtin_amdgcn_sched_barrier(0);
-                if constexpr (XQ && CR) load_items_cr<ITEMS, A, B>(keys_in, rwn, w);
+                if constexpr (XQ && CR && SA_LS_ROWCALC && A == 0) calc_rows_cr<ITEMS>(rwn, rc);
+                if constexpr (XQ && CR && SA_LS_ROWCALC) load_items_cr<ITEMS, A, B>(keys_in, rc, w);
+                else if constexpr (XQ && CR) load_items_cr<ITEMS, A, B>(keys_in, rwn, w);
                 else if constexpr (XQ) load_items_xq<ITEMS, A, B>(keys_in, rwn, hn.z, w);
                 else load_items<ITEMS, A, B>(keys_in, hn.y, hn.z, w);
             }
@@ -2045,7 +2104,10 @@
         if (!more) break;
         q = qn;
         h = hn;
-        if constexpr (XQ && CR) {
+        if constexpr (XQ && CR && SA_LS_ROWCALC) {
+            rv[0] = rc[0];
+            rv[1] = rc[1];
+        } else if constexpr (XQ && CR) {
             rv[0] = rwn[0];
             rv[1] = rwn[1];
         }
diff --git a/hpc_suffix_array_amd/csrc/sa_build.hip b/hpc_suffix_array_amd/csrc/sa_build.hip
--- a/hpc_suffix_array_amd/csrc/sa_build.hip
+++ b/hpc_suffix_array_amd/csrc/sa_build.hip
@@ -160,6 +160,7 @@
     bool dna = false;
     bool alpha_prove = false;
     bool alpha_refuted = false;
+    uint32_t cleared_ahead = 0;
     bool samples_pending = false;
 };
 
@@ -1286,6 +1287,11 @@
         SA_HIP(hipGetLastError());
         SA_HIP(hipMemcpyAsync(h_alpha, c->alpha, 8 * 4, hipMemcpyDeviceToHost, s));
         SA_HIP(hipMemcpyAsync(h_tail, d_text + (n - tail_n), tail_n, hipMemcpyDeviceToHost, s));
+        c->cleared_ahead = 0;
+        if (sampled) {
+            const int rca = round1_clear_ahead(c, n, s);
+            if (rca) return rca;
+        }
         SA_HIP(host_sync(s));
         *complete = true;
         for (uint32_t t = 0; t < tail_n; ++t) {
diff --git a/hpc_suffix_array_amd/csrc/sa_round1.h b/hpc_suffix_array_amd/csrc/sa_round1.h
--- a/hpc_suffix_array_amd/csrc/sa_round1.h
+++ b/hpc_suffix_array_amd/csrc/sa_round1.h
@@ -192,6 +192,47 @@
     return std::max<uint32_t>(7u, w > kLoBits ? w - kLoBits : 0u);
 }
 
+#ifndef SA_R1_SPECULATE
+#define SA_R1_SPECULATE 1
+#endif
+#ifndef SA_R1_CLEAR_AHEAD
+#define SA_R1_CLEAR_AHEAD 1
+#endif
+constexpr uint32_t kAheadBase = 1u;
+constexpr uint32_t kAheadSegx = 2u;
+
+static int round1_clear_words(sa_context* c, hipStream_t s) {
+    const int rc = onesweep_prepare(c, s);
+    if (rc) return rc;
+    SA_HIP(hipMemsetAsync(c->words, 0, 12, s));
+    SA_HIP(hipMemsetAsync(c->words + 5, 0, 44, s));
+    return SA_OK;
+}
+
+static int round1_clear_ahead(sa_context* c, uint64_t n, hipStream_t s) {
+    c->cleared_ahead = 0;
+    if (!SA_R1_CLEAR_AHEAD) return SA_OK;
+    ClearRanges r;
+    r.add(c->os, 2 * kMaxPasses * kRadix + kMaxPasses);
+    r.add(c->words, 3);
+    r.add(c->words + 5, 11);
+    const uint32_t stripes = text_stripes(c);
+    if (stripes > 1) r.add(c->hist, (uint64_t)stripes * kLoRadix);
+    r.add(c->segw, segw_words(1024));
+    const uint64_t nw = (n + kWinStride - 1) / kWinStride;
+    r.add(c->vals_alt + 3 * nw + 1, 2 * nw + 2);
+    r.add(c->member, (n + 31) / 32);
+    c->cleared_ahead = kAheadBase;
+    if (c->segx && c->segx_words >= xq_words(1024)) {
+        r.add(c->segx, xq_words(1024));
+        c->cleared_ahead |= kAheadSegx;
+    }
+    static_assert(kClearMax >= 8, "the ranges above");
+    hipLaunchKernelGGL(k_clear_ranges, dim3(8u * (uint32_t)c->cus), dim3(kBlock), 0, s, r);
+    SA_HIP(hipGetLastError());
+    return SA_OK;
+}
+
 static int round1_bucketed(sa_context* c, const uint8_t* d_text, uint64_t n, uint32_t* d_sa, const BucketPlan& bp,
                            const BucketRange& br_, hipStream_t s, Timer& tm, sa_stats* st, bool* done, bool* fused,
                            uint64_t seg[3], uint32_t* ksh, bool allow_pad = true, bool allow_xq = true,
@@ -203,10 +244,12 @@
     const uint64_t m = br_.m;
     const uint32_t blo = br_.blo, bhi = br_.bhi;
     if (bhi <= blo || bhi - blo > (1u << 18)) return set_err(SA_E_INTERNAL, "bucket range [%u, %u)", blo, bhi);
-    int rc = onesweep_prepare(c, s);
-    if (rc) return rc;
-    SA_HIP(hipMemsetAsync(c->words, 0, 12, s));
-    SA_HIP(hipMemsetAsync(c->words + 5, 0, 28, s));
+    uint32_t ahead = (br_.member || blo != 0 || m != n) ? 0u : c->cleared_ahead;
+    c->cleared_ahead = 0;
+    if (!(ahead & kAheadBase)) {
+        const int rc = round1_clear_words(c, s);
+        if (rc) return rc;
+    }
     const bool listed = m * 10 <= n * 3;
     uint64_t* const lkeys = c->keys_u;
     uint32_t* const lpos = c->vals_u;
@@ -321,6 +364,7 @@
             hipFree(c->segx);
             c->segx = nullptr;
             c->segx_words = 0;
+            ahead &= ~kAheadSegx;
             if (hipMalloc(&c->segx, need * 4) != hipSuccess) {
                 (void)hipGetLastError();
                 return set_err(SA_E_NOMEM, "second-pass queue workspace (%llu words)", (unsigned long long)need);
@@ -336,7 +380,7 @@
     const uint32_t stripes = padded ? text_stripes(c) : 1u;
     uint32_t* const cursor = stripes > 1 ? c->hist : os_ghist(c) + 5 * kRadix;
     uint32_t* const cursor_sum = stripes > 1 ? c->hist + kMaxStripes * kLoRadix : cursor;
-    if (stripes > 1) SA_HIP(hipMemsetAsync(cursor, 0, (size_t)stripes * kLoRadix * 4, s));
+    if (stripes > 1 && !(ahead & kAheadBase)) SA_HIP(hipMemsetAsync(cursor, 0, (size_t)stripes * kLoRadix * 4, s));
     if (!padded) {
         tm.begin(SA_K_SCAN);
         hipLaunchKernelGGL(k_digit_base_wide, dim3(1), dim3(1024), 0, s, (const uint32_t*)g_lo, kLoRadix, os_base(c));
@@ -430,10 +474,10 @@
         const SrcPk8 sp{c->keys[0]};
         uint32_t* tk = os_tickets(c) + 1;
         const uint32_t* hbase = os_base(c) + kLoRadix;
-        SA_HIP(hipMemsetAsync(c->segw, 0, segw_words(1u << hb) * 4, s));
+        if (!(ahead & kAheadBase)) SA_HIP(hipMemsetAsync(c->segw, 0, segw_words(1u << hb) * 4, s));
         SegXq sx;
         if (xq) {
-            SA_HIP(hipMemsetAsync(c->segx, 0, xqw * 4, s));
+            if (!(ahead & kAheadSegx)) SA_HIP(hipMemsetAsync(c->segx, 0, xqw * 4, s));
             sx.cur = c->segx;
             sx.sbase = reinterpret_cast<uint64_t*>(c->segx + (uint64_t)kXq * kSegs * (1u << hb));
             sx.done = c->segx + 3ull * kXq * kSegs * (1u << hb);
@@ -510,38 +554,11 @@
     tm.end();
     add_bytes(st, SA_K_WINDOWS, 8 * nw);
     SA_HIP(hipGetLastError());
-    SA_HIP(hipMemcpyAsync(c->host_words, c->words, 48, hipMemcpyDeviceToHost, s));
     uint32_t* skew = list + nw;
     uint32_t* cnt_u = skew + nw;
     uint32_t* cnt_g = cnt_u + nw + 1;
     uint32_t* const rank_arr = br_.rank ? br_.rank : c->rank;
     uint32_t* const member = br_.member ? br_.member : c->member;
-    SA_HIP(hipEventRecord(c->ev[kSyncEv], s));
-    SA_HIP(hipMemsetAsync(cnt_u, 0, (2 * nw + 2) * 4, s));
-    SA_HIP(hipMemsetAsync(member, 0, (n + 31) / 32 * 4, s));
-    SA_HIP(host_sync_event(c->ev[kSyncEv]));
-    if (c->alpha_prove && c->host_words[kAlphaBadWord]) {
-        c->alpha_refuted = true;
-        return SA_OK;
-    }
-    if (c->host_words[4]) return set_err(SA_E_INTERNAL, "radix look-back did not complete");
-    if (padded && c->host_words[11]) {
-        SA_TRACE("  bucketed round 1: padded segment overflow, again with exact digit totals");
-        const int rc = round1_bucketed(c, d_text, n, d_sa, bp, br_, s, tm, st, done, fused, seg, ksh, false, allow_xq,
-                                       round2);
-        if (st) st->round1_segments = 2;
-        return rc;
-    }
-    if (xq && c->host_words[9]) {
-        SA_TRACE("  bucketed round 1: second-pass queue overflow, again with one region");
-        return round1_bucketed(c, d_text, n, d_sa, bp, br_, s, tm, st, done, fused, seg, ksh, allow_pad, false,
-                               round2);
-    }
-    if (st) st->largest_window = (int32_t)std::min<uint32_t>(c->host_words[5], INT32_MAX);
-    if (c->host_words[5] > (uint32_t)kBsCap) {
-        SA_TRACE("  bucketed round 1: window of %u > %d suffixes, full sort instead", c->host_words[5], kBsCap);
-        return SA_OK;
-    }
     BucketRel br{cnt_g + nw + 1, c->segw + kBstartOff, c->segw + kBstartOff + kBstartWords, bp.bs.rb};
     br.bits1 = bits1;
     SegOut so{rank_arr, member, br_.sa_off, c->u_pos[1], c->u_idx[1], c->u_g[1], cnt_u, cnt_g, kKeySample};
@@ -555,22 +572,24 @@
     constexpr uint32_t kBsRows = (kBsBlock / kWave) * kBsItems;
     uint32_t* const xrows = xq ? hx + 16 * (nw + 1) : nullptr;
     const uint64_t* const wide_in = xq ? c->keys[1] : c->keys_u;
-    auto local_sort = [&](const SegOut& o) {
-        const uint32_t g = std::max<uint32_t>(1, std::min(c->host_words[7], kBsGrid));
-        static_assert(kRetryWord == kUsFlagWord + 1, "one memset clears words[12..15]");
-        (void)hipMemsetAsync(c->words + kUsFlagWord, 0, 16, s);
+    bool ls_fresh = true;
+    auto local_sort = [&](const SegOut& o, uint32_t nwin, uint32_t gate) {
+        const uint32_t g = std::max<uint32_t>(1, std::min(nwin, kBsGrid));
+        static_assert(kRetryWord == kUsFlagWord + 1 && kTicketWord == 15, "one memset clears words[12..15]");
+        if (!ls_fresh) (void)hipMemsetAsync(c->words + kUsFlagWord, 0, 16, s);
+        ls_fresh = false;
         if (fast32) {
             const uint32_t gs = (uint32_t)std::max<uint64_t>(1, std::min<uint64_t>((nw + kBlock - 1) / kBlock, 1024));
             const bool cr = xq && !(((uint32_t)c->tune >> 29) & 1u);
             const uint32_t ls_grid = (c->dbg & SA_DEBUG_LS_ONE_WG) ? 1u : kBsWpc * (uint32_t)c->cus;
             hipLaunchKernelGGL(k_window_split, dim3(gs), dim3(kBlock), 0, s, (const uint32_t*)list, (const uint32_t*)ws,
                                br, c->words, hdr, retry, 1u, (const uint32_t*)xq_pc, (const uint32_t*)xq_pn, nb_tab, hx,
-                               cr ? kBsRows : 0u);
+                               cr ? kBsRows : 0u, gate);
             if (xq) {
-                if (cr)
+                if (cr && !SA_LS_ROWCALC)
                     hipLaunchKernelGGL(k_window_rows<true>, dim3(2048), dim3(kBlock), 0, s, (const uint32_t*)c->words,
                                        (const uint4*)hdr, (const uint32_t*)hx, kBsRows, xrows);
-                else
+                else if (!cr)
                     hipLaunchKernelGGL(k_window_rows<false>, dim3(2048), dim3(kBlock), 0, s, (const uint32_t*)c->words,
                                        (const uint4*)hdr, (const uint32_t*)hx, kBsRows, xrows);
                 XqWin xw;
@@ -623,9 +642,55 @@
                            wide_in, br, (const uint32_t*)ws, (const uint32_t*)skew, c->words, bp.ib,
                            c->keys[0], d_sa, o);
     };
-    tm.begin(SA_K_LOCAL_SORT);
-    local_sort(so);
-    tm.end();
+    const bool spec = SA_R1_SPECULATE && fast32;
+    const uint32_t gate = kGateOn | (c->alpha_prove ? kGateAlpha : 0u) | (xq ? kGateXq : 0u) | (padded ? kGatePad : 0u);
+    SA_HIP(hipMemcpyAsync(c->host_words, c->words, 48, hipMemcpyDeviceToHost, s));
+    SA_HIP(hipEventRecord(c->ev[kSyncEv], s));
+    if (!((ahead & kAheadBase) && pk8 && !listed)) SA_HIP(hipMemsetAsync(cnt_u, 0, (2 * nw + 2) * 4, s));
+    if (!((ahead & kAheadBase) && member == c->member)) SA_HIP(hipMemsetAsync(member, 0, (n + 31) / 32 * 4, s));
+    if (spec) {
+        tm.begin(SA_K_LOCAL_SORT);
+        local_sort(so, (uint32_t)std::min<uint64_t>(nw, UINT32_MAX), gate);
+        tm.end();
+    }
+    SA_HIP(host_sync_event(c->ev[kSyncEv]));
+    auto gate_stopped = [&]() {
+        if (spec && st) st->round1_gate = SA_GATE_STOPPED;
+    };
+    if (c->alpha_prove && c->host_words[kAlphaBadWord]) {
+        c->alpha_refuted = true;
+        gate_stopped();
+        return SA_OK;
+    }
+    if (c->host_words[4]) {
+        gate_stopped();
+        return set_err(SA_E_INTERNAL, "radix look-back did not complete");
+    }
+    if (padded && c->host_words[11]) {
+        gate_stopped();
+        SA_TRACE("  bucketed round 1: padded segment overflow, again with exact digit totals");
+        const int rc = round1_bucketed(c, d_text, n, d_sa, bp, br_, s, tm, st, done, fused, seg, ksh, false, allow_xq,
+                                       round2);
+        if (st) st->round1_segments = 2;
+        return rc;
+    }
+    if (xq && c->host_words[9]) {
+        gate_stopped();
+        SA_TRACE("  bucketed round 1: second-pass queue overflow, again with one region");
+        return round1_bucketed(c, d_text, n, d_sa, bp, br_, s, tm, st, done, fused, seg, ksh, allow_pad, false,
+                               round2);
+    }
+    if (st) st->largest_window = (int32_t)std::min<uint32_t>(c->host_words[5], INT32_MAX);
+    if (c->host_words[5] > (uint32_t)kBsCap) {
+        SA_TRACE("  bucketed round 1: window of %u > %d suffixes, full sort instead", c->host_words[5], kBsCap);
+        gate_stopped();
+        return SA_OK;
+    }
+    if (!spec) {
+        tm.begin(SA_K_LOCAL_SORT);
+        local_sort(so, c->host_words[7], 0u);
+        tm.end();
+    }
     add_bytes(st, SA_K_LOCAL_SORT, 12 * m + (so.samples ? (m >> kKeySample) * 8 : 0));
     SA_HIP(hipGetLastError());
     auto gather_u = [&]() {
@@ -675,6 +740,8 @@
         const uint32_t wv[4] = {c->host_words[7], c->host_words[kHdrWord], c->host_words[kRetryWord], c->host_words[10]};
         for (int t = 0; t < 4; ++t) st->round1_windows[t] = (int32_t)std::min<uint32_t>(wv[t], INT32_MAX);
     }
+    if (spec && st && st->round1_gate != SA_GATE_STOPPED)
+        st->round1_gate = (c->host_words[6] & kGateStopped) ? SA_GATE_STOPPED : SA_GATE_RAN;
     if (c->host_words[6]) {
         SA_TRACE("  bucketed round 1: local sort flags %u, full sort instead", c->host_words[6]);
         if (try_r2) tm.round_unmark();
@@ -708,7 +775,7 @@
         full.ksh = 0;
         SA_HIP(hipMemsetAsync(c->words + 10, 0, 4, s));
         tm.begin(SA_K_LOCAL_SORT);
-        local_sort(full);
+        local_sort(full, c->host_words[7], 0u);
         tm.end();
         add_bytes(st, SA_K_LOCAL_SORT, 20 * m);
         SA_HIP(hipGetLastError());
diff --git a/hpc_suffix_array_amd/csrc/sa_rows.h b/hpc_suffix_array_amd/csrc/sa_rows.h
--- /dev/null
+++ b/hpc_suffix_array_amd/csrc/sa_rows.h
@@ -0,0 +1,55 @@
+#pragma once
+#include <stdint.h>
+
+#if defined(__HIPCC__) || defined(__HIP__)
+#define SA_ROWS_HD __host__ __device__ __forceinline__
+#define SA_ROWS_UNROLL _Pragma("unroll")
+#else
+#define SA_ROWS_HD inline
+#define SA_ROWS_UNROLL
+#endif
+
+namespace sa {
+
+constexpr uint32_t kRowChunks = 8;
+constexpr uint32_t kRowLanes = 64;
+
+struct RowWords {
+    uint32_t base;
+    uint32_t count;
+};
+
+SA_ROWS_HD RowWords chunk_row(const uint32_t (&st)[kRowChunks], const uint32_t (&cn)[kRowChunks], uint32_t r) {
+    uint32_t nfull = 0;
+    SA_ROWS_UNROLL
+    for (uint32_t k = 0; k < kRowChunks; ++k) nfull += cn[k] / kRowLanes;
+    RowWords w{st[0], 0u};
+    uint32_t rf = 0, rp = nfull;
+    SA_ROWS_UNROLL
+    for (uint32_t k = 0; k < kRowChunks; ++k) {
+        const uint32_t nf = cn[k] / kRowLanes, rem = cn[k] % kRowLanes;
+        if (r - rf < nf) {
+            w.base = st[k] + kRowLanes * (r - rf);
+            w.count = kRowLanes;
+        }
+        if (rem && r == rp) {
+            w.base = st[k] + kRowLanes * nf;
+            w.count = rem;
+        }
+        rf += nf;
+        rp += rem ? 1u : 0u;
+    }
+    return w;
+}
+
+SA_ROWS_HD void chunk_spans(const uint32_t (&hx)[2 * kRowChunks], uint32_t m, uint32_t (&st)[kRowChunks],
+                            uint32_t (&cn)[kRowChunks]) {
+    SA_ROWS_UNROLL
+    for (uint32_t k = 0; k < kRowChunks; ++k) {
+        const uint32_t p0 = k ? hx[kRowChunks - 1 + k] : 0u, p1 = k + 1 < kRowChunks ? hx[kRowChunks + k] : m;
+        st[k] = hx[k] + p0;
+        cn[k] = p1 - p0;
+    }
+}
+
+}
diff --git a/include/sa_hip.h b/include/sa_hip.h
--- a/include/sa_hip.h
+++ b/include/sa_hip.h
@@ -80,6 +80,10 @@
     int32_t span_extra;
     int32_t tune;
 } sa_opts;
+
+#define SA_GATE_NOT_SPECULATED 0
+#define SA_GATE_RAN 1
+#define SA_GATE_STOPPED 2
 
 typedef struct {
     int32_t rounds;
@@ -105,6 +109,7 @@
     int32_t round1_layout;
     uint64_t round_bytes[SA_MAX_ROUNDS];
     int32_t round1_windows[4];
+    int32_t round1_gate;
     int32_t alphabet;
 } sa_stats;
 
```

After: 109.6 billion. No clear change (-0.3%).
